# castacks/mvs_gi

Measured on AMD Instinct MI355X. Metric: stereo frames/sec/GPU (G16V, 3-cam, D=16) + inv-dist L1 vs reference, higher is better.
Workload: dtype f16x3 (split-fp16 MFMA operands: 11 + 11 significant bits, f32 accumulate/activations)

## Files before the change

include/mvsgi.h:

```cpp
#ifndef MVSGI_H
#define MVSGI_H

#include <stddef.h>
#include <stdint.h>

#ifdef __cplusplus
extern "C" {
#endif

#define MVSGI_ABI_VERSION 8

typedef void* mvsgi_stream_t;

#define MVSGI_CONV_AUTO   0
#define MVSGI_CONV_DIRECT 1
#define MVSGI_CONV_MFMA   2
#define MVSGI_CONV_BF16X3 3
#define MVSGI_CONV_BF16X3_C16 4
#define MVSGI_CONV_BF16X3_V32 5
#define MVSGI_CONV_BF16X3_D32 6

#define MVSGI_CONV_F16 0x100

#define MVSGI_SPLIT_F16 1

int         mvsgi_abi_version(void);
const char* mvsgi_last_error(void);

#define MVSGI_SAT_SWEEP 1u
#define MVSGI_SAT_SPLIT 2u
#define MVSGI_SAT_WINO  4u
int mvsgi_saturation_flags(int clear, unsigned* flags);
int mvsgi_saturation_words(unsigned* words8);

int mvsgi_sweep_max_cams(void);
int mvsgi_sweep_std_f32(const float* feats, const float* grids, const void* grid_masks,
                        int grid_mask_is_f32, const float* masks, float* vol,
                        int B, int N, int C, int Hi, int Wi, int Hm, int Wm,
                        int D, int Ho, int Wo, mvsgi_stream_t stream);

int mvsgi_sweep_cat_f32(const float* feats, const float* grids, float* vol,
                        int B, int N, int C, int Hi, int Wi,
                        int D, int Ho, int Wo, mvsgi_stream_t stream);

int mvsgi_sweep_std_nhwc_f32(const float* feats, const float* grids, const void* grid_masks,
                             int grid_mask_is_f32, const float* masks, float* vol,
                             int B, int N, int C, int Hi, int Wi, int Hm, int Wm,
                             int D, int Ho, int Wo, mvsgi_stream_t stream);
int mvsgi_sweep_cat_nhwc_f32(const float* feats, const float* grids, float* vol,
                             int B, int N, int C, int Hi, int Wi,
                             int D, int Ho, int Wo, mvsgi_stream_t stream);

int mvsgi_sweep_validity_u8(const float* grids, const void* grid_masks, int grid_mask_is_f32,
                            const float* masks, unsigned char* vmask,
                            int B, int N, int Hm, int Wm, int D, int Ho, int Wo, mvsgi_stream_t stream);
int mvsgi_sweep_std_nhwc_valid_f32(const float* feats, const float* grids, const unsigned char* vmask,
                                   float* vol, int B, int N, int C, int Hi, int Wi,
                                   int D, int Ho, int Wo, mvsgi_stream_t stream);
int mvsgi_sweep_std_nhwc_valid_rig_f32(const float* feats, const float* grids, const unsigned char* vmask,
                                       float* vol, int B, int N, int C, int Hi, int Wi, int D, int Ho, int Wo,
                                       mvsgi_stream_t stream);

size_t mvsgi_conv3d_packed_weight_floats(int Cout, int Cin);
int mvsgi_conv3d_pack_weights_f32(const float* w_oidhw, float* w_packed, int Cout, int Cin,
                                  mvsgi_stream_t stream);
size_t mvsgi_conv3d_packed_weight_bytes_bf16x3(int Cout, int Cin);
int mvsgi_conv3d_pack_weights_bf16x3(const float* w_oidhw, void* w_packed, int Cout, int Cin,
                                     mvsgi_stream_t stream);
int mvsgi_conv3d_pack_weights_split(const float* w_oidhw, void* w_packed, int Cout, int Cin, int layout, mvsgi_stream_t stream);
int mvsgi_conv3d_f32(const float* x, const float* w_oidhw, const float* w_packed,
                     const float* scale, const float* shift, const float* res, float* y,
                     int B, int Cin, int Din, int Hin, int Win, int Cout,
                     int stride, float neg_slope, int impl, mvsgi_stream_t stream);
const char* mvsgi_conv3d_variant_f32(int B, int Cin, int Din, int Hin, int Win, int Cout,
                                     int stride, int impl);

int mvsgi_conv3d_up2_f32(const float* x, const void* w_packed, int w_layout ,
                         const float* scale, const float* shift, const float* res, float* y,
                         int B, int Cin, int Dl, int Hl, int Wl, int Cout, float neg_slope, mvsgi_stream_t stream);
const char* mvsgi_conv3d_up2_variant_f32(int B, int Cin, int Dl, int Hl, int Wl, int Cout, int w_layout);
int mvsgi_conv3d_v32_applies(int B, int Cin, int Din, int Hin, int Win, int Cout, int stride);
int mvsgi_conv3d_d32_applies(int B, int Cin, int Din, int Hin, int Win, int Cout, int stride);
int mvsgi_conv3d_up2_d32_applies(int B, int Cin, int Dl, int Hl, int Wl, int Cout);
size_t mvsgi_conv3d_packed_weight_bytes_bf16x3_v32(int Cout, int Cin);
int mvsgi_conv3d_pack_weights_bf16x3_v32(const float* w_oidhw, void* w_packed, int Cout, int Cin, mvsgi_stream_t stream);
size_t mvsgi_conv3d_packed_weight_bytes_bf16x3_c16(int Cin);
int mvsgi_conv3d_pack_weights_bf16x3_c16(const float* w_oidhw, void* w_packed, int Cin, mvsgi_stream_t stream);

size_t mvsgi_conv2d_packed_weight_floats(int Cout, int Cin);
int mvsgi_conv2d_pack_weights_f32(const float* w_oihw, float* w_packed, int Cout, int Cin,
                                  mvsgi_stream_t stream);
size_t mvsgi_conv2d_stem_packed_weight_bytes(void);
int mvsgi_conv2d_stem_pack_weights(const float* w_oihw, void* w_packed, mvsgi_stream_t stream);
size_t mvsgi_conv2d_packed_weight_bytes_bf16x3(int Cout, int Cin);
int mvsgi_conv2d_pack_weights_bf16x3(const float* w_oihw, void* w_packed, int Cout, int Cin,
                                     mvsgi_stream_t stream);
int mvsgi_conv2d_f32(const float* x, const float* w_oihw, const void* w_packed,
                     const float* scale, const float* shift, const float* res, float* y,
                     int B, int Cin, int Hin, int Win, int Cout, int ksize, int stride,
                     float neg_slope, int impl, int in_nchw, mvsgi_stream_t stream);
const char* mvsgi_conv2d_variant_f32(int Cin, int Cout, int ksize, int stride, int impl, int in_nchw);

int mvsgi_resize_trilinear_f32(const float* x, float* y, int B, int C,
                               int Di, int Hi, int Wi, int Do, int Ho, int Wo,
                               mvsgi_stream_t stream);

int mvsgi_softargmin_f32(const float* costs, const float* inv_idx, float* inv_dist,
                         float* norm_costs, int B, int D, int H, int W, int scale,
                         mvsgi_stream_t stream);

int mvsgi_softargmin_div_f32(const float* costs, const float* inv_idx, float* inv_dist,
                             float* norm_costs, int B, int D, int H, int W, int scale,
                             float post_div, mvsgi_stream_t stream);

#define MVSGI_SA_AUTO  0
#define MVSGI_SA_PIXEL 1
#define MVSGI_SA_BAND  2
int mvsgi_softargmin_scaled_f32(const float* costs, const float* inv_idx, float* inv_dist,
                                float* norm_costs, int B, int D, int H, int W, double scale,
                                int OH, int OW, float post_div, int variant, mvsgi_stream_t stream);

int mvsgi_ncv_to_nvc_f32(const float* x, float* y, int B, int C, long long V, mvsgi_stream_t stream);
int mvsgi_nvc_to_ncv_f32(const float* x, float* y, int B, int C, long long V, mvsgi_stream_t stream);

int mvsgi_resblock2d_f32(const float* x, const void* w_packed1, const float* scale1, const float* shift1,
                         const void* w_packed2, const float* scale2, const float* shift2, float* y,
                         int N, int H, int W, float neg_slope, mvsgi_stream_t stream);

size_t mvsgi_split2d_bytes(int N, int H, int W);
int mvsgi_f32_to_split2d(const float* x, void* y_split, int N, int H, int W, mvsgi_stream_t stream);
int mvsgi_split2d_to_f32(const void* x_split, float* y, int N, int H, int W, mvsgi_stream_t stream);
size_t mvsgi_resblock2d_split_packed_weight_bytes(void);
int mvsgi_resblock2d_split_pack_weights(const float* w_oihw, const float* scale, void* w_packed, mvsgi_stream_t stream);
int mvsgi_resblock2d_split(const void* x_split, const void* w_packed1, const float* shift1,
                           const void* w_packed2, const float* shift2, void* y, int y_is_split,
                           int N, int H, int W, float neg_slope, mvsgi_stream_t stream);
int mvsgi_conv2d_s2_split(const void* x_split, const void* w_packed, const float* shift, void* y_split,
                          int N, int H, int W, float neg_slope, mvsgi_stream_t stream);
int mvsgi_conv2d_f32_out_split2d(const float* x, const float* w_oihw, const void* w_packed,
                                 const float* scale, const float* shift, const float* res, void* y_split,
                                 int B, int Cin, int Hin, int Win, int Cout, int ksize, int stride,
                                 float neg_slope, int impl, int in_nchw, mvsgi_stream_t stream);

int mvsgi_rays_panorama_f32(const float* dist, float* rays, int N, int H, int W,
                            float lat0, float lat1, float lon0, float lon1, mvsgi_stream_t stream);
int mvsgi_transform_points_f32(const float* T , const float* points, float* out,
                               int B, long long M, mvsgi_stream_t stream);
int mvsgi_grid_double_sphere_f32(const float* points, float* grid, unsigned char* mask, int B, long long M,
                                 float xi, float alpha, float fx, float fy, float cx, float cy,
                                 int calib_h, int calib_w, float w2, mvsgi_stream_t stream);
int mvsgi_grid_equirect_f32(const float* points, float* grid, int B, long long M, mvsgi_stream_t stream);
int mvsgi_rays_equirect_surrogate_f32(float* rays, int H, int W, mvsgi_stream_t stream);

int mvsgi_resample_bilinear_u8_f32(const unsigned char* imgs, const float* grid, const unsigned char* valid, float* out,
                                   long long M, int T, int Hr, int Wr, int H, int W, float invalid_value, mvsgi_stream_t stream);
int mvsgi_resample_bilinear_f32(const float* imgs, const float* grid, const unsigned char* valid, float* out, long long M, int T,
                                int C, int Hr, int Wr, int H, int W, float invalid_value, mvsgi_stream_t stream);
int mvsgi_resample_validity_u8(const float* grid, const unsigned char* ds_mask, unsigned char* valid, long long n,
                               mvsgi_stream_t stream);
int mvsgi_resample_u8_table_f32(float* table256);

int mvsgi_reproject_f32(const float* inv, const float* rays, const void* imgs, int img_kind, const float* T_host,
                        const float* cams_host, float* xyz, float* warped, unsigned char* valid, float* grid,
                        long long B, int N, int C, int Hr, int Wr, int H, int W, float bf, float invalid_value,
                        mvsgi_stream_t stream);

int mvsgi_deform_conv2d_pack_weights_f32(const float* w_oihw, float* w_packed, int Cout, int Cin, int Kh, int Kw,
                                         mvsgi_stream_t stream);
int mvsgi_deform_conv2d_f32(const float* x, const float* offset, int offset_per_image, const float* w_packed,
                            const float* scale, const float* shift, const float* res, float* y,
                            int N, int Cin, int H, int W, int Cout, int Kh, int Kw, int stride_h, int stride_w,
                            int pad_h, int pad_w, int dil_h, int dil_w, float neg_slope, mvsgi_stream_t stream);

int mvsgi_sweep_std_nhwc_valid_split(const float* feats, const float* grids, const unsigned char* vmask,
                                     void* vol_split, int B, int N, int C, int Hi, int Wi, int D, int Ho, int Wo,
                                     int rig_batch, mvsgi_stream_t stream);

int mvsgi_conv3d_f32_out_split(const float* x, const float* w_packed_b3, const float* scale, const float* shift,
                               const float* res, void* y_split, int B, int Cin, int Din, int Hin, int Win, int Cout,
                               int stride, float neg_slope, mvsgi_stream_t stream);
int mvsgi_conv3d_rs16_split(const void* x_split, const void* w_packed_rs, const float* scale, const float* shift, float* y,
                            int B, int D, int H, int W, float neg_slope, mvsgi_stream_t stream);
int mvsgi_conv3d_rs16_split_out_split(const void* x_split, const void* w_packed_rs, const float* scale, const float* shift,
                                      void* y_split, int B, int D, int H, int W, float neg_slope, mvsgi_stream_t stream);
size_t mvsgi_conv3d_s2rs_packed_weight_bytes(void);
int mvsgi_conv3d_s2rs_pack_weights(const float* w_oidhw, const float* scale, void* w_packed, mvsgi_stream_t stream);
int mvsgi_conv3d_s2rs(const void* x_split, const void* w_packed, const float* shift, void* y_split,
                      int B, int D, int H, int W, float neg_slope, mvsgi_stream_t stream);
size_t mvsgi_conv3d_rs_packed_weight_bytes(int Cout, int Cin);
int mvsgi_conv3d_rs_pack_weights(const float* w_oidhw, void* w_packed, int Cout, int Cin, mvsgi_stream_t stream);
size_t mvsgi_act_split_bytes(int B, int C, int D, int H, int W);
int mvsgi_act_f32_to_split(const float* x, void* y_split, int B, int C, int D, int H, int W, mvsgi_stream_t stream);
int mvsgi_act_split_to_f32(const void* x_split, float* y, int B, int C, int D, int H, int W, mvsgi_stream_t stream);
int mvsgi_conv3d_rs_split(const void* x_split, const void* w_packed_rs, const float* scale, const float* shift,
                          const void* res_split, void* y, int y_is_f32, int B, int Cin, int D, int H, int W, int Cout,
                          float neg_slope, mvsgi_stream_t stream);

int mvsgi_conv3d_up2_f32_out_split(const float* x, const void* w_packed, int w_layout, const float* scale, const float* shift,
                                   const float* res, void* y_split, int B, int Cin, int Dl, int Hl, int Wl, int Cout,
                                   float neg_slope, mvsgi_stream_t stream);
int mvsgi_conv3d_up2_poly_split(const void* x_split, const void* plan_dev, const float* scale, const float* shift, void* y_split,
                                int B, int D, int H, int W, float neg_slope, mvsgi_stream_t stream);
size_t mvsgi_conv3d_head_split_packed_weight_bytes(int Cin);
int mvsgi_conv3d_head_split_pack_weights(const float* w_oidhw, void* w_packed, int Cin, mvsgi_stream_t stream);
int mvsgi_conv3d_head_split(const void* x_split, const void* w_packed, float scale, float shift, float* y, int B, int Cin,
                            int D, int H, int W, float neg_slope, mvsgi_stream_t stream);
int mvsgi_conv3d_head_split_pack_weights_f16(const float* w_oidhw, void* w_packed, int Cin, mvsgi_stream_t stream);
int mvsgi_conv3d_head_split_f16(const void* x_split, const void* w_packed, float scale, float shift, float* y, int B, int Cin,
                            int D, int H, int W, float neg_slope, mvsgi_stream_t stream);
size_t mvsgi_conv3d_up2_poly_plan_bytes(int D, int H, int W);
int mvsgi_conv3d_up2_poly_plan(const float* w_oidhw_host, void* plan_host, int D, int H, int W);
int mvsgi_conv3d_up2_poly_f32(const void* x_split, const void* plan_dev, const float* scale, const float* shift, float* y,
                              int B, int D, int H, int W, float neg_slope, mvsgi_stream_t stream);

int mvsgi_act_f32_to_split_fmt(const float* x, void* y_split, int B, int C, int D, int H, int W, int fmt, mvsgi_stream_t stream);
int mvsgi_act_split_to_f32_fmt(const void* x_split, float* y, int B, int C, int D, int H, int W, int fmt, mvsgi_stream_t stream);
int mvsgi_sweep_std_nhwc_valid_split_fmt(const float* feats, const float* grids, const unsigned char* vmask, void* vol_split,
                                         int B, int N, int C, int Hi, int Wi, int D, int Ho, int Wo, int rig_batch, int fmt,
                                         mvsgi_stream_t stream);
int mvsgi_conv3d_f32_out_split_fmt(const float* x, const float* w_packed_b3, const float* scale, const float* shift,
                                   const float* res, void* y_split, int B, int Cin, int Din, int Hin, int Win, int Cout,
                                   int stride, float neg_slope, int fmt, mvsgi_stream_t stream);
int mvsgi_conv3d_rs_pack_weights_fmt(const float* w_oidhw, void* w_packed, int Cout, int Cin, int fmt, mvsgi_stream_t stream);
int mvsgi_conv3d_rs_split_fmt(const void* x_split, const void* w_packed_rs, const float* scale, const float* shift,
                              const void* res_split, void* y, int y_is_f32, int B, int Cin, int D, int H, int W, int Cout,
                              float neg_slope, int fmt, mvsgi_stream_t stream);
int mvsgi_conv3d_rs16_split_fmt(const void* x_split, const void* w_packed_rs, const float* scale, const float* shift, void* y,
                                int y_is_split, int B, int D, int H, int W, float neg_slope, int fmt, mvsgi_stream_t stream);
int mvsgi_conv3d_s2rs_pack_weights_fmt(const float* w_oidhw, const float* scale, void* w_packed, int fmt, mvsgi_stream_t stream);
int mvsgi_conv3d_s2rs_fmt(const void* x_split, const void* w_packed, const float* shift, void* y_split, int B, int D, int H, int W,
                          float neg_slope, float unscale, int fmt, mvsgi_stream_t stream);
int mvsgi_conv3d_s2rs_out_fmt(const void* x_split, const void* w_packed, const float* shift, void* y_split, int B, int D, int H, int W,
                              float neg_slope, float unscale, int fmt, int y_f32p, mvsgi_stream_t stream);
int mvsgi_conv3d_up2_poly_plan_fmt(const float* w_oidhw_host, void* plan_host, int D, int H, int W, int fmt);
int mvsgi_conv3d_up2_poly_fmt(const void* x_split, const void* plan_dev, const float* scale, const float* shift, void* y,
                              int y_is_split, int B, int D, int H, int W, float neg_slope, int fmt, mvsgi_stream_t stream);
int mvsgi_conv3d_up2_poly_wino_pays(int B, int D, int H, int W);

size_t mvsgi_conv3d_wino32_packed_weight_bytes(void);
int mvsgi_conv3d_wino32_applies(int Cin, int Cout, int D, int H, int W, int stride, float neg_slope);
int mvsgi_conv3d_wino32_pack_weights(const float* w_oidhw, void* w_packed, float* unscale, mvsgi_stream_t stream);
int mvsgi_conv3d_wino32_f16(const void* x_split, const void* w_packed, const float* scale, const float* shift, const void* res_split,
                            void* y, int y_is_f32, int act_f32p, int B, int D, int H, int W, float neg_slope, mvsgi_stream_t stream);

size_t mvsgi_instance_norm_ws_bytes(int B, int S, int C);
int mvsgi_instance_norm_f32(const float* x, const float* res, const float* gamma, const float* beta, float* y, float* ws,
                            int B, int S, int C, float eps, float neg_slope, mvsgi_stream_t stream);

#ifdef __cplusplus
}
#endif
#endif
```

mvs_gi_amd/_lib.py:

```python
from __future__ import annotations

import ctypes
import os
from ctypes import c_char_p, c_double, c_float, c_int, c_longlong, c_size_t, c_void_p

_HERE = os.path.dirname(os.path.abspath(__file__))
LIB_PATH = os.environ.get("MVSGI_LIB", os.path.join(_HERE, "libmvsgi_hip.so"))

ABI_VERSION = 8


class MvsgiLibraryMissing(RuntimeError):
    pass


_P = c_void_p
SIGNATURES = {
    "mvsgi_abi_version": (c_int, []),
    "mvsgi_last_error": (c_char_p, []),
    "mvsgi_saturation_flags": (c_int, [c_int, _P]),
    "mvsgi_saturation_words": (c_int, [_P]),
    "mvsgi_sweep_max_cams": (c_int, []),
    "mvsgi_sweep_std_f32": (c_int, [_P, _P, _P, c_int, _P, _P] + [c_int] * 10 + [_P]),
    "mvsgi_sweep_cat_f32": (c_int, [_P, _P, _P] + [c_int] * 8 + [_P]),
    "mvsgi_sweep_std_nhwc_f32": (c_int, [_P, _P, _P, c_int, _P, _P] + [c_int] * 10 + [_P]),
    "mvsgi_sweep_cat_nhwc_f32": (c_int, [_P, _P, _P] + [c_int] * 8 + [_P]),
    "mvsgi_sweep_validity_u8": (c_int, [_P, _P, c_int, _P, _P] + [c_int] * 7 + [_P]),
    "mvsgi_sweep_std_nhwc_valid_f32": (c_int, [_P, _P, _P, _P] + [c_int] * 8 + [_P]),
    "mvsgi_sweep_std_nhwc_valid_split": (c_int, [_P, _P, _P, _P] + [c_int] * 9 + [_P]),
    "mvsgi_sweep_std_nhwc_valid_rig_f32": (c_int, [_P, _P, _P, _P] + [c_int] * 8 + [_P]),
    "mvsgi_conv3d_packed_weight_floats": (c_size_t, [c_int, c_int]),
    "mvsgi_conv3d_pack_weights_f32": (c_int, [_P, _P, c_int, c_int, _P]),
    "mvsgi_conv3d_packed_weight_bytes_bf16x3": (c_size_t, [c_int, c_int]),
    "mvsgi_conv3d_pack_weights_bf16x3": (c_int, [_P, _P, c_int, c_int, _P]),
    "mvsgi_conv3d_pack_weights_split": (c_int, [_P, _P, c_int, c_int, c_int, _P]),
    "mvsgi_conv3d_f32": (c_int, [_P] * 7 + [c_int] * 7 + [c_float, c_int, _P]),
    "mvsgi_conv3d_variant_f32": (c_char_p, [c_int] * 8),
    "mvsgi_conv3d_up2_f32": (c_int, [_P, _P, c_int] + [_P] * 4 + [c_int] * 6 + [c_float, _P]),
    "mvsgi_conv3d_up2_variant_f32": (c_char_p, [c_int] * 7),
    "mvsgi_conv3d_v32_applies": (c_int, [c_int] * 7),
    "mvsgi_conv3d_d32_applies": (c_int, [c_int] * 7),
    "mvsgi_conv3d_up2_d32_applies": (c_int, [c_int] * 6),
    "mvsgi_conv3d_packed_weight_bytes_bf16x3_v32": (c_size_t, [c_int, c_int]),
    "mvsgi_conv3d_pack_weights_bf16x3_v32": (c_int, [_P, _P, c_int, c_int, _P]),
    "mvsgi_conv3d_packed_weight_bytes_bf16x3_c16": (c_size_t, [c_int]),
    "mvsgi_conv3d_pack_weights_bf16x3_c16": (c_int, [_P, _P, c_int, _P]),
    "mvsgi_conv2d_stem_packed_weight_bytes": (c_size_t, []),
    "mvsgi_conv2d_stem_pack_weights": (c_int, [_P, _P, _P]),
    "mvsgi_conv2d_packed_weight_floats": (c_size_t, [c_int, c_int]),
    "mvsgi_conv2d_pack_weights_f32": (c_int, [_P, _P, c_int, c_int, _P]),
    "mvsgi_conv2d_packed_weight_bytes_bf16x3": (c_size_t, [c_int, c_int]),
    "mvsgi_conv2d_pack_weights_bf16x3": (c_int, [_P, _P, c_int, c_int, _P]),
    "mvsgi_conv2d_f32": (c_int, [_P] * 7 + [c_int] * 7 + [c_float, c_int, c_int, _P]),
    "mvsgi_conv2d_variant_f32": (c_char_p, [c_int] * 6),
    "mvsgi_resblock2d_f32": (c_int, [_P] * 8 + [c_int] * 3 + [c_float, _P]),
    "mvsgi_split2d_bytes": (c_size_t, [c_int] * 3),
    "mvsgi_f32_to_split2d": (c_int, [_P, _P] + [c_int] * 3 + [_P]),
    "mvsgi_split2d_to_f32": (c_int, [_P, _P] + [c_int] * 3 + [_P]),
    "mvsgi_resblock2d_split_packed_weight_bytes": (c_size_t, []),
    "mvsgi_resblock2d_split_pack_weights": (c_int, [_P, _P, _P, _P]),
    "mvsgi_resblock2d_split": (c_int, [_P] * 6 + [c_int] * 4 + [c_float, _P]),
    "mvsgi_conv2d_s2_split": (c_int, [_P] * 4 + [c_int] * 3 + [c_float, _P]),
    "mvsgi_conv2d_f32_out_split2d": (c_int, [_P] * 7 + [c_int] * 7 + [c_float, c_int, c_int, _P]),
    "mvsgi_resize_trilinear_f32": (c_int, [_P, _P] + [c_int] * 8 + [_P]),
    "mvsgi_softargmin_f32": (c_int, [_P, _P, _P, _P] + [c_int] * 5 + [_P]),
    "mvsgi_softargmin_div_f32": (c_int, [_P, _P, _P, _P] + [c_int] * 5 + [c_float, _P]),
    "mvsgi_softargmin_scaled_f32": (c_int, [_P, _P, _P, _P] + [c_int] * 4 + [c_double, c_int, c_int, c_float, c_int, _P]),
    "mvsgi_rays_panorama_f32": (c_int, [_P, _P, c_int, c_int, c_int] + [c_float] * 4 + [_P]),
    "mvsgi_transform_points_f32": (c_int, [_P, _P, _P, c_int, c_longlong, _P]),
    "mvsgi_grid_double_sphere_f32": (c_int, [_P, _P, _P, c_int, c_longlong] + [c_float] * 6 + [c_int, c_int, c_float, _P]),
    "mvsgi_grid_equirect_f32": (c_int, [_P, _P, c_int, c_longlong, _P]),
    "mvsgi_rays_equirect_surrogate_f32": (c_int, [_P, c_int, c_int, _P]),
    "mvsgi_resample_bilinear_u8_f32": (c_int, [_P, _P, _P, _P, c_longlong] + [c_int] * 5 + [c_float, _P]),
    "mvsgi_resample_bilinear_f32": (c_int, [_P, _P, _P, _P, c_longlong] + [c_int] * 6 + [c_float, _P]),
    "mvsgi_resample_validity_u8": (c_int, [_P, _P, _P, c_longlong, _P]),
    "mvsgi_resample_u8_table_f32": (c_int, [_P]),
    "mvsgi_reproject_f32": (c_int, [_P, _P, _P, c_int] + [_P] * 6 + [c_longlong] + [c_int] * 6 + [c_float, c_float, _P]),
    "mvsgi_deform_conv2d_pack_weights_f32": (c_int, [_P, _P] + [c_int] * 4 + [_P]),
    "mvsgi_deform_conv2d_f32": (c_int, [_P, _P, c_int] + [_P] * 5 + [c_int] * 13 + [c_float, _P]),
    "mvsgi_act_split_bytes": (c_size_t, [c_int] * 5),
    "mvsgi_act_f32_to_split": (c_int, [_P, _P] + [c_int] * 5 + [_P]),
    "mvsgi_act_split_to_f32": (c_int, [_P, _P] + [c_int] * 5 + [_P]),
    "mvsgi_conv3d_f32_out_split": (c_int, [_P] * 6 + [c_int] * 7 + [c_float, _P]),
    "mvsgi_conv3d_rs16_split": (c_int, [_P] * 5 + [c_int] * 4 + [c_float, _P]),
    "mvsgi_conv3d_rs16_split_out_split": (c_int, [_P] * 5 + [c_int] * 4 + [c_float, _P]),
    "mvsgi_conv3d_s2rs_packed_weight_bytes": (c_size_t, []),
    "mvsgi_conv3d_s2rs_pack_weights": (c_int, [_P, _P, _P, _P]),
    "mvsgi_conv3d_s2rs": (c_int, [_P] * 4 + [c_int] * 4 + [c_float, _P]),
    "mvsgi_conv3d_rs_packed_weight_bytes": (c_size_t, [c_int, c_int]),
    "mvsgi_conv3d_rs_pack_weights": (c_int, [_P, _P, c_int, c_int, _P]),
    "mvsgi_conv3d_rs_split": (c_int, [_P] * 6 + [c_int] * 7 + [c_float, _P]),
    "mvsgi_conv3d_up2_f32_out_split": (c_int, [_P, _P, c_int] + [_P] * 4 + [c_int] * 6 + [c_float, _P]),
    "mvsgi_conv3d_up2_poly_split": (c_int, [_P] * 5 + [c_int] * 4 + [c_float, _P]),
    "mvsgi_conv3d_head_split_packed_weight_bytes": (c_size_t, [c_int]),
    "mvsgi_conv3d_head_split_pack_weights": (c_int, [_P, _P, c_int, _P]),
    "mvsgi_conv3d_head_split": (c_int, [_P, _P, c_float, c_float, _P] + [c_int] * 5 + [c_float, _P]),
    "mvsgi_conv3d_head_split_pack_weights_f16": (c_int, [_P, _P, c_int, _P]),
    "mvsgi_conv3d_head_split_f16": (c_int, [_P, _P, c_float, c_float, _P] + [c_int] * 5 + [c_float, _P]),
    "mvsgi_conv3d_up2_poly_plan_bytes": (c_size_t, [c_int] * 3),
    "mvsgi_conv3d_up2_poly_plan": (c_int, [_P, _P] + [c_int] * 3),
    "mvsgi_conv3d_up2_poly_f32": (c_int, [_P] * 5 + [c_int] * 4 + [c_float, _P]),
    "mvsgi_act_f32_to_split_fmt": (c_int, [_P, _P] + [c_int] * 6 + [_P]),
    "mvsgi_act_split_to_f32_fmt": (c_int, [_P, _P] + [c_int] * 6 + [_P]),
    "mvsgi_sweep_std_nhwc_valid_split_fmt": (c_int, [_P, _P, _P, _P] + [c_int] * 10 + [_P]),
    "mvsgi_conv3d_f32_out_split_fmt": (c_int, [_P] * 6 + [c_int] * 7 + [c_float, c_int, _P]),
    "mvsgi_conv3d_rs_pack_weights_fmt": (c_int, [_P, _P, c_int, c_int, c_int, _P]),
    "mvsgi_conv3d_rs_split_fmt": (c_int, [_P] * 6 + [c_int] * 7 + [c_float, c_int, _P]),
    "mvsgi_conv3d_rs16_split_fmt": (c_int, [_P] * 5 + [c_int] * 5 + [c_float, c_int, _P]),
    "mvsgi_conv3d_s2rs_pack_weights_fmt": (c_int, [_P, _P, _P, c_int, _P]),
    "mvsgi_conv3d_s2rs_fmt": (c_int, [_P] * 4 + [c_int] * 4 + [c_float, c_float, c_int, _P]),
    "mvsgi_conv3d_s2rs_out_fmt": (c_int, [_P] * 4 + [c_int] * 4 + [c_float, c_float, c_int, c_int, _P]),
    "mvsgi_conv3d_up2_poly_plan_fmt": (c_int, [_P, _P] + [c_int] * 4),
    "mvsgi_conv3d_wino32_packed_weight_bytes": (c_size_t, []),
    "mvsgi_conv3d_wino32_applies": (c_int, [c_int] * 6 + [c_float]),
    "mvsgi_conv3d_wino32_pack_weights": (c_int, [_P] * 4),
    "mvsgi_conv3d_wino32_f16": (c_int, [_P] * 6 + [c_int] * 6 + [c_float, _P]),
    "mvsgi_conv3d_up2_poly_fmt": (c_int, [_P] * 5 + [c_int] * 5 + [c_float, c_int, _P]),
    "mvsgi_conv3d_up2_poly_wino_pays": (c_int, [c_int] * 4),
    "mvsgi_ncv_to_nvc_f32": (c_int, [_P, _P, c_int, c_int, c_longlong, _P]),
    "mvsgi_nvc_to_ncv_f32": (c_int, [_P, _P, c_int, c_int, c_longlong, _P]),
    "mvsgi_instance_norm_ws_bytes": (c_size_t, [c_int] * 3),
    "mvsgi_instance_norm_f32": (c_int, [_P] * 6 + [c_int] * 3 + [c_float, c_float, _P]),
}

_lib = None


def load() -> ctypes.CDLL:
    global _lib
    if _lib is not None:
        return _lib
    if not os.path.isfile(LIB_PATH):
        raise MvsgiLibraryMissing(
            f"{LIB_PATH} not found: build the HIP library first (__graft_entry__.build()). "
            "mvs_gi_amd has no CPU fallback.")
    import torch
    lib = ctypes.CDLL(LIB_PATH)
    try:
        lib.mvsgi_abi_version.restype = c_int
        lib.mvsgi_abi_version.argtypes = []
        got = lib.mvsgi_abi_version()
    except AttributeError as e:
        raise MvsgiLibraryMissing(f"{LIB_PATH}: not a libmvsgi_hip ({e}); rebuild it (__graft_entry__.build())") from None
    if got != ABI_VERSION:
        raise MvsgiLibraryMissing(f"{LIB_PATH}: ABI version {got}, expected {ABI_VERSION}; rebuild it (__graft_entry__.build())")
    for name, (res, args) in SIGNATURES.items():
        try:
            fn = getattr(lib, name)
        except AttributeError:
            raise MvsgiLibraryMissing(f"{LIB_PATH}: symbol {name} missing although the ABI version matches; rebuild it "
                                      "(__graft_entry__.build())") from None
        fn.restype = res
        fn.argtypes = args
    lib.mvsgi_saturation_flags(0, None)
    _lib = lib
    return lib


def check(status: int, what: str) -> None:
    if status != 0:
        msg = load().mvsgi_last_error()
        raise RuntimeError(f"{what}: {msg.decode() if msg else 'unknown error'}")
```

mvs_gi_amd/csrc/common.hpp:

```cpp
#pragma once
#include <hip/hip_runtime.h>

#include <cstdarg>
#include <cstdio>
#include <cstdlib>
#include <cstring>
#include <string>

#include "../../include/mvsgi.h"

namespace mvsgi {

std::string& last_error_ref();

inline int fail(const char* fmt, ...) {
    char buf[512];
    va_list ap;
    va_start(ap, fmt);
    vsnprintf(buf, sizeof(buf), fmt, ap);
    va_end(ap);
    last_error_ref() = buf;
    return 1;
}

inline int check_launch(const char* what) {
    hipError_t e = hipGetLastError();
    if (e != hipSuccess) return fail("%s: launch failed: %s", what, hipGetErrorString(e));
    return 0;
}

#define MVSGI_REQUIRE(cond, ...)                      \
    do {                                              \
        if (!(cond)) return ::mvsgi::fail(__VA_ARGS__); \
    } while (0)

constexpr int kSatWords = 8;
unsigned* sat_words();
#define MVSGI_SAT_WORDS(VAR)                                                            \
    unsigned* VAR = ::mvsgi::sat_words();                                               \
    MVSGI_REQUIRE(VAR != nullptr, "cannot allocate the range report's pinned host words")

inline hipStream_t as_stream(mvsgi_stream_t s) { return reinterpret_cast<hipStream_t>(s); }

inline long long cdiv(long long a, long long b) { return (a + b - 1) / b; }

constexpr int kMaxCams = 8;

constexpr int kMaxDevices = 32;
struct PersistentGeom {
    int wgs_per_cu;
    int cus;
};
template <class K>
inline int persistent_geometry(K kern, int threads, size_t lds_bytes, int max_wgs_per_cu,
                               PersistentGeom (&cache)[kMaxDevices], const char* what, PersistentGeom& out) {
    int dev = 0;
    hipError_t e = hipGetDevice(&dev);
    if (e != hipSuccess) return fail("%s: hipGetDevice: %s", what, hipGetErrorString(e));
    if (dev < 0 || dev >= kMaxDevices) return fail("%s: device ordinal %d not supported (max %d)", what, dev, kMaxDevices);
    PersistentGeom g = cache[dev];
    if (!g.wgs_per_cu) {
        e = hipFuncSetAttribute(reinterpret_cast<const void*>(kern), hipFuncAttributeMaxDynamicSharedMemorySize,
                                (int)lds_bytes);
        if (e != hipSuccess) return fail("%s: hipFuncSetAttribute: %s", what, hipGetErrorString(e));
        int occ = 0;
        e = hipOccupancyMaxActiveBlocksPerMultiprocessor(&occ, kern, threads, lds_bytes);
        if (e != hipSuccess || occ < 1) occ = 1;
        int cus = 0;
        e = hipDeviceGetAttribute(&cus, hipDeviceAttributeMultiprocessorCount, dev);
        if (e != hipSuccess || cus < 1) return fail("%s: cannot read the device's CU count", what);
        g.wgs_per_cu = occ > max_wgs_per_cu ? max_wgs_per_cu : occ;
        g.cus = cus;
        cache[dev] = g;
    }
    out = g;
    return 0;
}

inline int device_cus() {
    static int cache[kMaxDevices] = {};
    int dev = 0;
    if (hipGetDevice(&dev) != hipSuccess || dev < 0 || dev >= kMaxDevices) return 256;
    if (!cache[dev]) {
        int cus = 0;
        if (hipDeviceGetAttribute(&cus, hipDeviceAttributeMultiprocessorCount, dev) != hipSuccess || cus < 1) cus = 256;
        cache[dev] = cus;
    }
    return cache[dev];
}

constexpr size_t kRs32PackedBytes = (size_t)2 * 2 * 14 * 2 * 64 * 16;
void rs32_pack_weights_host(const float* w_oidhw_32x32x27, void* packed, bool f16);
int rs32_up2_launch(const void* x_split, const void* w_sets, const float* scale32, const float* shift32, void* y, int y_is_split,
                    int B, int D, int H, int W, float neg_slope, bool f16, hipStream_t st);

constexpr size_t kWinoUp2RoleBytes = (size_t)4 * 4 * 3 * 2 * 2 * 64 * 16;
void wino_up2_pack_role(const float* w32_oidhw, unsigned short* wp, float* unscale32);
bool wino_up2_applies(int D, int H, int W);
int wino_up2_launch(const void* x_split, const void* w_roles, const float* unw, const float* scale16, const float* shift16, void* y_split,
                    int B, int D, int H, int W, float neg_slope, hipStream_t st);

}
```

mvs_gi_amd/csrc/conv3d_headsplit.hip:

```cpp
#include "common.hpp"

namespace {

typedef float f32x4 __attribute__((ext_vector_type(4)));
typedef unsigned u32x4 __attribute__((ext_vector_type(4)));
typedef __bf16 bf16x8 __attribute__((ext_vector_type(8)));
typedef _Float16 f16x8 __attribute__((ext_vector_type(8)));
typedef unsigned short u16x8 __attribute__((ext_vector_type(8)));

struct HeadArgs {
    const unsigned char* x;
    const bf16x8* wp;
    float* y;
    float scale, shift;
    float neg_slope;
    int B, Cin, D, H, W;
    int tiles_h, tiles_w;
};

__device__ __forceinline__ int hs_xcd_remap(int bid, int n) {
    const int q = n >> 3, r = n & 7, x = bid & 7, i = bid >> 3;
    return (x < r ? x * (q + 1) : r * (q + 1) + (x - r) * q) + i;
}

__global__ void head_split_pack_kernel(const float* __restrict__ w, bf16x8* __restrict__ wp, int Cin, bool f16) {
    const int idx = blockIdx.x * 256 + threadIdx.x;
    const int total = (Cin / 16) * 2 * 64;
    if (idx >= total) return;
    const int lane = idx & 63, tt = (idx >> 6) & 1, cs = idx >> 7;
    const int kg = lane >> 4, tap = tt * 16 + (lane & 15);
    u16x8 a1, a2;
    for (int j = 0; j < 8; ++j) {
        const float v = tap < 27 ? w[(cs * 16 + 8 * (kg & 1) + j) * 27 + tap] : 0.f;
        unsigned short h, l;
        if (f16) {
            const _Float16 hh = (_Float16)v;
            h = __builtin_bit_cast(unsigned short, hh);
            l = __builtin_bit_cast(unsigned short, (_Float16)(v - (float)hh));
        } else {
            const __bf16 hh = (__bf16)v;
            h = __builtin_bit_cast(unsigned short, hh);
            l = __builtin_bit_cast(unsigned short, (__bf16)(v - (float)hh));
        }
        a1[j] = h;
        a2[j] = kg < 2 ? l : (unsigned short)0;
    }
    wp[((cs * 2 + tt) * 2) * 64 + lane] = __builtin_bit_cast(bf16x8, a1);
    wp[((cs * 2 + tt) * 2 + 1) * 64 + lane] = __builtin_bit_cast(bf16x8, a2);
}

template <bool F16>
__global__ __launch_bounds__(256) void conv3d_head_split_kernel(HeadArgs a, int dchunk, int nd) {
    constexpr int TH = 8, TW = 32, ITH = TH + 2, ITW = TW + 2, PV = ITH * ITW;
    constexpr int NT = (PV + 15) / 16;
    constexpr int TPW = (NT + 3) / 4;
    constexpr int PSTR = 360;
    static_assert(NT * 16 <= PSTR, "P row too short");
    extern __shared__ __attribute__((aligned(16))) float hs_pbuf[];
    const int tid = threadIdx.x, lane = tid & 63;
    const int wave = __builtin_amdgcn_readfirstlane(tid >> 6);
    const int col = lane & 15, kg = lane >> 4;
    int t = hs_xcd_remap((int)blockIdx.x, (int)gridDim.x);
    const int tw_i = t % a.tiles_w;
    t /= a.tiles_w;
    const int th_i = t % a.tiles_h;
    t /= a.tiles_h;
    const int dc = t % nd;
    const int b = t / nd;
    const int oh0 = th_i * TH, ow0 = tw_i * TW;
    const int od_begin = dc * dchunk;
    const int od_end = od_begin + dchunk < a.D ? od_begin + dchunk : a.D;
    const int p0 = od_begin > 0 ? od_begin - 1 : 0;
    const int p1 = od_end < a.D - 1 ? od_end : a.D - 1;
    const int nchunks = a.Cin / 16;
    const int U = (p1 - p0 + 1) * nchunks;
    const int Hp = a.H + 2, Wp = a.W + 2, rec = a.Cin * 4;
    const long long plane_bytes = (long long)Hp * Wp * rec;

    unsigned goff[TPW];
#pragma unroll
    for (int k = 0; k < TPW; ++k) {
        const int T = wave + 4 * k, v = T * 16 + col;
        const int ih = v / ITW, iw = v - ih * ITW;
        const bool ok = T < NT && v < PV && oh0 + ih < Hp && ow0 + iw < Wp;
        goff[k] = ok ? (unsigned)(((oh0 + ih) * Wp + ow0 + iw) * rec + kg * 16) : 0xffffff00u;
    }
    const unsigned char* xb = a.x + (long long)b * (a.D + 2) * plane_bytes;
    bf16x8 wa[2][2];
    u32x4 xr[TPW];
#define HS_FETCH(P, CS)                                                                                             \
    {                                                                                                               \
        const __amdgpu_buffer_rsrc_t d_ = __builtin_amdgcn_make_buffer_rsrc(                                        \
            const_cast<unsigned char*>(xb) + (long long)((P) + 1) * plane_bytes, 0, (int)plane_bytes, 0x00020000); \
        _Pragma("unroll") for (int k = 0; k < TPW; ++k)                                                             \
            xr[k] = __builtin_amdgcn_raw_buffer_load_b128(d_, goff[k] + (unsigned)((CS) * 64), 0, 0);               \
        _Pragma("unroll") for (int tt = 0; tt < 2; ++tt) {                                                          \
            wa[tt][0] = a.wp[(((CS) * 2 + tt) * 2) * 64 + lane];                                                    \
            wa[tt][1] = a.wp[(((CS) * 2 + tt) * 2 + 1) * 64 + lane];                                                \
        }                                                                                                           \
    }
    HS_FETCH(p0, 0)

    const int h_ = tid / TW, w_ = tid % TW;
    const int oh = oh0 + h_, ow = ow0 + w_;
    const bool inside = oh < a.H && ow < a.W;
    float run[3] = {0.f, 0.f, 0.f};
    f32x4 acc[TPW][2];
#pragma unroll
    for (int k = 0; k < TPW; ++k) acc[k][0] = acc[k][1] = f32x4{0.f, 0.f, 0.f, 0.f};

    int p = p0, cs = 0;
    float pend = 0.f;
    long long pend_vox = -1;
    for (int u = 0; u < U; ++u) {
        int ncs = cs + 1, np = p;
        if (ncs == nchunks) { ncs = 0; np = p + 1; }
        bf16x8 cx[TPW], cw[2][2];
#pragma unroll
        for (int k = 0; k < TPW; ++k) cx[k] = __builtin_bit_cast(bf16x8, xr[k]);
#pragma unroll
        for (int tt = 0; tt < 2; ++tt) { cw[tt][0] = wa[tt][0]; cw[tt][1] = wa[tt][1]; }
        if (pend_vox >= 0) {
            a.y[pend_vox] = pend;
            pend_vox = -1;
        }
        {
            const int fp = u + 1 < U ? np : p, fcs = u + 1 < U ? ncs : cs;
            HS_FETCH(fp, fcs)
        }
#pragma unroll
        for (int k = 0; k < TPW; ++k) {
            if (wave + 4 * k < NT) {
#pragma unroll
                for (int tt = 0; tt < 2; ++tt) {
                    if constexpr (F16) {
                        acc[k][tt] = __builtin_amdgcn_mfma_f32_16x16x32_f16(__builtin_bit_cast(f16x8, cw[tt][1]), __builtin_bit_cast(f16x8, cx[k]), acc[k][tt], 0, 0, 0);
                        acc[k][tt] = __builtin_amdgcn_mfma_f32_16x16x32_f16(__builtin_bit_cast(f16x8, cw[tt][0]), __builtin_bit_cast(f16x8, cx[k]), acc[k][tt], 0, 0, 0);
                    } else {
                        acc[k][tt] = __builtin_amdgcn_mfma_f32_16x16x32_bf16(cw[tt][1], cx[k], acc[k][tt], 0, 0, 0);
                        acc[k][tt] = __builtin_amdgcn_mfma_f32_16x16x32_bf16(cw[tt][0], cx[k], acc[k][tt], 0, 0, 0);
                    }
                }
            }
        }
        if (ncs == 0) {
#pragma unroll
            for (int k = 0; k < TPW; ++k) {
                if (wave + 4 * k < NT) {
                    const int v = (wave + 4 * k) * 16 + col;
#pragma unroll
                    for (int tt = 0; tt < 2; ++tt)
#pragma unroll
                        for (int r = 0; r < 4; ++r) {
                            const int row = tt * 16 + 4 * kg + r;
                            if (row < 27) hs_pbuf[row * PSTR + v] = acc[k][tt][r];
                        }
                    acc[k][0] = acc[k][1] = f32x4{0.f, 0.f, 0.f, 0.f};
                }
            }
            __syncthreads();
#pragma unroll
            for (int k2 = 0; k2 < 9; ++k2) {
                const int vv = (h_ + k2 / 3) * ITW + (w_ + k2 % 3);
                run[0] += hs_pbuf[(18 + k2) * PSTR + vv];
                run[1] += hs_pbuf[(9 + k2) * PSTR + vv];
                run[2] += hs_pbuf[k2 * PSTR + vv];
            }
            const int od = p - 1;
            if (od >= od_begin && inside) {
                const long long vox = (((long long)b * a.D + od) * a.H + oh) * a.W + ow;
                const float r = run[0] * a.scale + a.shift;
                pend = r > 0.f ? r : r * a.neg_slope;
                pend_vox = vox;
            }
            run[0] = run[1];
            run[1] = run[2];
            run[2] = 0.f;
            __syncthreads();
        }
        p = np;
        cs = ncs;
    }
    if (pend_vox >= 0) a.y[pend_vox] = pend;
    if (p1 < od_end && inside) {
        const long long vox = (((long long)b * a.D + p1) * a.H + oh) * a.W + ow;
        const float r = run[0] * a.scale + a.shift;
        a.y[vox] = r > 0.f ? r : r * a.neg_slope;
    }
#undef HS_FETCH
}

}

extern "C" size_t mvsgi_conv3d_head_split_packed_weight_bytes(int Cin) {
    return Cin > 0 && Cin % 16 == 0 ? (size_t)(Cin / 16) * 2 * 2 * 64 * 16 : 0;
}

namespace {
int head_pack(const float* w_oidhw, void* w_packed, int Cin, bool f16, mvsgi_stream_t stream, const char* who) {
    MVSGI_REQUIRE(w_oidhw && w_packed, "%s: null pointer", who);
    MVSGI_REQUIRE(Cin > 0 && Cin % 16 == 0, "%s: Cin=%d must be a positive multiple of 16", who, Cin);
    const int total = (Cin / 16) * 2 * 64;
    hipLaunchKernelGGL(head_split_pack_kernel, dim3((unsigned)mvsgi::cdiv(total, 256)), dim3(256), 0, mvsgi::as_stream(stream), w_oidhw,
                       static_cast<bf16x8*>(w_packed), Cin, f16);
    return mvsgi::check_launch(who);
}

int head_launch(const void* x_split, const void* w_packed, float scale, float shift, float* y, int B, int Cin, int D, int H, int W,
                float neg_slope, bool f16, mvsgi_stream_t stream, const char* who) {
    MVSGI_REQUIRE(x_split && w_packed && y, "%s: null pointer", who);
    MVSGI_REQUIRE(B > 0 && D > 0 && H > 0 && W > 0 && Cin > 0 && Cin % 16 == 0, "%s: bad dims (Cin %% 16 == 0)", who);
    MVSGI_REQUIRE((long long)(H + 2) * (W + 2) * Cin * 4 < (1ll << 31), "%s: plane too large for 32-bit offsets", who);
    HeadArgs a{};
    a.x = static_cast<const unsigned char*>(x_split);
    a.wp = static_cast<const bf16x8*>(w_packed);
    a.y = y;
    a.scale = scale; a.shift = shift; a.neg_slope = neg_slope;
    a.B = B; a.Cin = Cin; a.D = D; a.H = H; a.W = W;
    a.tiles_h = (int)mvsgi::cdiv(H, 8);
    a.tiles_w = (int)mvsgi::cdiv(W, 32);
    const long long windows = (long long)B * a.tiles_h * a.tiles_w;
    long long nd = windows >= 1024 ? 1 : mvsgi::cdiv(1024, windows);
    if (nd > mvsgi::cdiv(D, 2)) nd = mvsgi::cdiv(D, 2);
    const int dchunk = (int)mvsgi::cdiv(D, nd);
    nd = mvsgi::cdiv(D, dchunk);
    const long long nt = windows * nd;
    MVSGI_REQUIRE(nt < (1ll << 31), "%s: too many tiles", who);
    constexpr size_t lds_bytes = (size_t)27 * 360 * sizeof(float);
    if (f16)
        hipLaunchKernelGGL(conv3d_head_split_kernel<true>, dim3((unsigned)nt), dim3(256), lds_bytes, mvsgi::as_stream(stream), a, dchunk, (int)nd);
    else
        hipLaunchKernelGGL(conv3d_head_split_kernel<false>, dim3((unsigned)nt), dim3(256), lds_bytes, mvsgi::as_stream(stream), a, dchunk, (int)nd);
    return mvsgi::check_launch(who);
}
}

extern "C" int mvsgi_conv3d_head_split_pack_weights(const float* w_oidhw, void* w_packed, int Cin, mvsgi_stream_t stream) {
    return head_pack(w_oidhw, w_packed, Cin, false, stream, "mvsgi_conv3d_head_split_pack_weights");
}
extern "C" int mvsgi_conv3d_head_split_pack_weights_f16(const float* w_oidhw, void* w_packed, int Cin, mvsgi_stream_t stream) {
    return head_pack(w_oidhw, w_packed, Cin, true, stream, "mvsgi_conv3d_head_split_pack_weights_f16");
}

extern "C" int mvsgi_conv3d_head_split(const void* x_split, const void* w_packed, float scale, float shift, float* y, int B, int Cin,
                                       int D, int H, int W, float neg_slope, mvsgi_stream_t stream) {
    return head_launch(x_split, w_packed, scale, shift, y, B, Cin, D, H, W, neg_slope, false, stream, "mvsgi_conv3d_head_split");
}
extern "C" int mvsgi_conv3d_head_split_f16(const void* x_split, const void* w_packed, float scale, float shift, float* y, int B, int Cin,
                                           int D, int H, int W, float neg_slope, mvsgi_stream_t stream) {
    return head_launch(x_split, w_packed, scale, shift, y, B, Cin, D, H, W, neg_slope, true, stream, "mvsgi_conv3d_head_split_f16");
}
```

mvs_gi_amd/csrc/conv3d_up2poly.hip:

```cpp
#include "common.hpp"

#include <cstring>
#include <vector>

namespace {

typedef float f32x4 __attribute__((ext_vector_type(4)));
typedef unsigned u32x4 __attribute__((ext_vector_type(4)));
typedef __bf16 bf16x8 __attribute__((ext_vector_type(8)));
#include "split_fmt.hpp"

enum { FIRST = 0, INT = 1, LAST = 2, ONLY = 3 };

struct M3 {
    double m[3][3];
};

M3 axis_matrix(int p, int i, int n) {
    M3 M{};
    for (int k = 0; k < 3; ++k) {
        const int v = 2 * i + p + k - 1;
        if (v < 0 || v >= 2 * n) continue;
        const int m = v >> 1, q = v & 1;
        const int src[2] = {q == 0 ? m - 1 : m, q == 0 ? m : m + 1};
        const double wgt[2] = {q == 0 ? 0.25 : 0.75, q == 0 ? 0.75 : 0.25};
        for (int e = 0; e < 2; ++e) {
            int s_ = src[e] < 0 ? 0 : (src[e] > n - 1 ? n - 1 : src[e]);
            M.m[s_ - i + 1][k] += wgt[e];
        }
    }
    return M;
}
M3 class_matrix(int p, int cls) {
    const int n = cls == ONLY ? 1 : 4;
    const int i = cls == FIRST || cls == ONLY ? 0 : (cls == INT ? 1 : n - 1);
    return axis_matrix(p, i, n);
}
M3 face_delta(int p, int cls) {
    const M3 a = class_matrix(p, cls), b = class_matrix(p, INT);
    M3 d{};
    for (int k = 0; k < 3; ++k) d.m[1][k] = a.m[1][k] - b.m[1][k];
    return d;
}
void fold(const M3& Md, const M3& Mh, const M3& Mw, const float* w, float* out) {
    for (int oi = 0; oi < 16 * 32; ++oi) {
        const float* ws = w + (size_t)oi * 27;
        double t1[27], t2[27], t3[27];
        for (int a = 0; a < 3; ++a)
            for (int l = 0; l < 3; ++l)
                for (int m = 0; m < 3; ++m) {
                    double s = 0;
                    for (int k = 0; k < 3; ++k) s += Md.m[a][k] * ws[k * 9 + l * 3 + m];
                    t1[a * 9 + l * 3 + m] = s;
                }
        for (int a = 0; a < 3; ++a)
            for (int b = 0; b < 3; ++b)
                for (int m = 0; m < 3; ++m) {
                    double s = 0;
                    for (int l = 0; l < 3; ++l) s += Mh.m[b][l] * t1[a * 9 + l * 3 + m];
                    t2[a * 9 + b * 3 + m] = s;
                }
        for (int a = 0; a < 3; ++a)
            for (int b = 0; b < 3; ++b)
                for (int c = 0; c < 3; ++c) {
                    double s = 0;
                    for (int m = 0; m < 3; ++m) s += Mw.m[c][m] * t2[a * 9 + b * 3 + m];
                    t3[a * 9 + b * 3 + c] = s;
                }
        for (int q = 0; q < 27; ++q) out[(size_t)oi * 27 + q] = (float)t3[q];
    }
}

struct Group {
    int cls, first, count;
};
std::vector<Group> groups_of(int n) {
    if (n == 1) return {{ONLY, 0, 1}};
    if (n == 2) return {{FIRST, 0, 1}, {LAST, 1, 1}};
    return {{FIRST, 0, 1}, {INT, 1, n - 2}, {LAST, n - 1, 1}};
}
struct Face {
    int idx, cls;
};
std::vector<Face> faces_of(int n) {
    if (n == 1) return {{0, ONLY}};
    return {{0, FIRST}, {n - 1, LAST}};
}

constexpr int kMagic = 0x50325032;
constexpr int kRoleInts = 32;
enum { R_WOFF = 0, R_NTAPS, R_TAP0, R_XBASE = 11, R_XS0, R_XSRUN, R_N0, R_NRUN, R_YS0, R_YSRUN, R_MFIRST, R_MLAST, R_YBASE0 = 20 };
enum { ST_WRITE = 0, ST_RMW = 1, ST_SKIP = 2 };
constexpr size_t kFaceRoleWBytes = (size_t)9 * 8 * 2 * 64 * 16;
constexpr size_t kEdgeSetFloats = (size_t)9 * 32 * 16;

struct PolyHeader {
    int magic, D, H, W;
    int n_roles, n_edge_cells, n_groups, max_tpf;
    long long off_main, off_facew, off_roles, off_edgew, off_edgecells, total;
    int sum_tpf;
    int pad0;
    long long off_roles_split;
    long long off_wino;
    long long off_wino_unscale;
    int pad[4];
};
static_assert(sizeof(PolyHeader) == 128, "header");

inline size_t align256(size_t v) { return (v + 255) & ~(size_t)255; }

PolyHeader layout(int D, int H, int W) {
    PolyHeader h{};
    h.magic = kMagic;
    h.D = D; h.H = H; h.W = W;
    const int ng = (int)groups_of(D).size(), nfh = (int)faces_of(H).size(), nfw = (int)faces_of(W).size();
    h.n_groups = ng;
    h.n_roles = (nfh + nfw) * ng;
    h.n_edge_cells = nfh * nfw;
    size_t o = sizeof(PolyHeader);
    h.off_main = (long long)(o = align256(o));
    o += 16 * mvsgi::kRs32PackedBytes;
    h.off_facew = (long long)(o = align256(o));
    o += (size_t)h.n_roles * kFaceRoleWBytes;
    h.off_roles = (long long)(o = align256(o));
    o += (size_t)h.n_roles * kRoleInts * 4;
    h.off_roles_split = (long long)(o = align256(o));
    o += (size_t)h.n_roles * kRoleInts * 4;
    h.off_edgew = (long long)(o = align256(o));
    o += (size_t)ng * h.n_edge_cells * 8 * kEdgeSetFloats * 4;
    h.off_edgecells = (long long)(o = align256(o));
    o += (size_t)h.n_edge_cells * 4 * 4;
    if (mvsgi::wino_up2_applies(D, H, W)) {
        h.off_wino = (long long)(o = align256(o));
        o += 2 * mvsgi::kWinoUp2RoleBytes;
        h.off_wino_unscale = (long long)(o = align256(o));
        o += 2 * 32 * 4;
    }
    h.total = (long long)align256(o);
    int tpf = 0, sum = 0;
    for (const Group& g : groups_of(D)) {
        const int a = g.count * (int)mvsgi::cdiv(W, 16), b = g.count * (int)mvsgi::cdiv(H, 16);
        tpf = a > tpf ? a : tpf;
        tpf = b > tpf ? b : tpf;
        sum += nfh * a + nfw * b;
    }
    h.max_tpf = tpf;
    h.sum_tpf = sum;
    return h;
}

void pack_face_weights(const float* wsrc, const int* taps, unsigned short* out, bool f16) {
    for (int t = 0; t < 9; ++t)
        for (int ph = 0; ph < 8; ++ph)
            for (int lane = 0; lane < 64; ++lane) {
                const int kg = lane >> 4, co = lane & 15;
                const size_t o = (((size_t)(t * 8 + ph) * 2) * 64 + lane) * 8;
                for (int e = 0; e < 8; ++e) {
                    const float v = wsrc[(((size_t)ph * 16 + co) * 32 + kg * 8 + e) * 27 + taps[t]];
                    sf_split_weight(v, f16, out[o + e], out[o + 64 * 8 + e]);
                }
            }
}

struct FaceGrid {
    int n_roles;
    int first[13];
};
template <bool F16>
__global__ __launch_bounds__(512, 2) void up2_face_kernel(const unsigned char* __restrict__ x, const unsigned char* __restrict__ plan,
                                                          unsigned char* __restrict__ y, int B, long long x_frame, long long y_frame,
                                                          long long off_facew, long long off_roles, FaceGrid fg) {
    extern __shared__ __attribute__((aligned(16))) unsigned char fw_lds[];
    int role = 0;
#pragma unroll
    for (int r = 1; r < 12; ++r) role += (r < fg.n_roles && (int)blockIdx.x >= fg.first[r]) ? 1 : 0;
    const int chunk = (int)blockIdx.x - fg.first[role], chunks = fg.first[role + 1] - fg.first[role];
    const int* R = reinterpret_cast<const int*>(plan + off_roles) + role * kRoleInts;
    const int n0 = R[R_N0], nrun = R[R_NRUN];
    const int tiles_run = (nrun + 15) >> 4, tpf = n0 * tiles_run;
    const int tid = threadIdx.x, lane = tid & 63, wave = __builtin_amdgcn_readfirstlane(tid >> 6);
    const int col = lane & 15, kg = lane >> 4;
    {
        const u32x4* src = reinterpret_cast<const u32x4*>(plan + off_facew) + (long long)R[R_WOFF];
        for (int i = tid; i < (int)(kFaceRoleWBytes / 16); i += 512) reinterpret_cast<u32x4*>(fw_lds)[i] = src[i];
    }
    __syncthreads();
    int tap[9], yb[8];
#pragma unroll
    for (int t = 0; t < 9; ++t) tap[t] = R[R_TAP0 + t];
#pragma unroll
    for (int p = 0; p < 8; ++p) yb[p] = R[R_YBASE0 + p];
    const int x_base = R[R_XBASE], x_s0 = R[R_XS0], x_srun = R[R_XSRUN];
    const int y_s0 = R[R_YS0], y_srun = R[R_YSRUN];
    const int m_first = R[R_MFIRST], m_last = R[R_MLAST];
    const int lane_x = (kg >> 1) * 64 + (kg & 1) * 16;
    const int total = B * tpf, stride = chunks * 8;
    for (int t = chunk * 8 + wave; t < total; t += stride) {
        const int rt = t % tiles_run;
        int q = t / tiles_run;
        const int o0 = q % n0, b = q / n0;
        const int run = rt * 16 + col;
        const bool ok = run < nrun;
        const __amdgpu_buffer_rsrc_t dx = __builtin_amdgcn_make_buffer_rsrc(const_cast<unsigned char*>(x) + (long long)b * x_frame, 0,
                                                                            (int)x_frame, 0x00020000);
        const unsigned xo = ok ? (unsigned)(x_base + o0 * x_s0 + run * x_srun + lane_x) : 0xffffff00u;
        u32x4 fh[9], fl[9];
#pragma unroll
        for (int k = 0; k < 9; ++k) {
            fh[k] = __builtin_amdgcn_raw_buffer_load_b128(dx, xo + (unsigned)tap[k], 0, 0);
            fl[k] = __builtin_amdgcn_raw_buffer_load_b128(dx, xo + (unsigned)tap[k] + 32u, 0, 0);
        }
        f32x4 acc[8];
#pragma unroll
        for (int p = 0; p < 8; ++p) acc[p] = f32x4{0.f, 0.f, 0.f, 0.f};
        int woff = lane * 16;
        asm volatile("" : "+v"(woff));
        bf16x8 wb[2][16];
#pragma unroll
        for (int i = 0; i < 16; ++i) wb[0][i] = *reinterpret_cast<const bf16x8*>(fw_lds + woff + i * 1024);
#pragma unroll
        for (int k = 0; k < 9; ++k) {
            if (k + 1 < 9) {
#pragma unroll
                for (int i = 0; i < 16; ++i) wb[(k + 1) & 1][i] = *reinterpret_cast<const bf16x8*>(fw_lds + woff + ((k + 1) * 16 + i) * 1024);
            }
            const bf16x8 xh = __builtin_bit_cast(bf16x8, fh[k]), xl = __builtin_bit_cast(bf16x8, fl[k]);
#pragma unroll
            for (int p = 0; p < 8; ++p) acc[p] = sf_mfma16<F16>(wb[k & 1][2 * p + 1], xh, acc[p]);
#pragma unroll
            for (int p = 0; p < 8; ++p) acc[p] = sf_mfma16<F16>(wb[k & 1][2 * p], xl, acc[p]);
#pragma unroll
            for (int p = 0; p < 8; ++p) acc[p] = sf_mfma16<F16>(wb[k & 1][2 * p], xh, acc[p]);
        }
        const int mode = run == 0 ? m_first : (run == nrun - 1 ? m_last : ST_WRITE);
        if (ok && mode != ST_SKIP) {
            unsigned char* yf = y + (long long)b * y_frame + (long long)o0 * y_s0 + (long long)run * y_srun + kg * 16;
#pragma unroll
            for (int p = 0; p < 8; ++p) {
                f32x4* dst = reinterpret_cast<f32x4*>(yf + yb[p]);
                *dst = mode == ST_RMW ? *dst + acc[p] : acc[p];
            }
        }
    }
}

template <bool F16>
__global__ __launch_bounds__(256) void up2_edge_kernel(const unsigned char* __restrict__ x, const unsigned char* __restrict__ plan,
                                                       float* __restrict__ y, int B, int D, int H, int W, int n_cells, int n_groups,
                                                       long long off_edgew, long long off_edgecells, int ob) {
    const long long idx = (long long)blockIdx.x * 256 + threadIdx.x;
    const long long n = (long long)B * D * n_cells * 128;
    if (idx >= n) return;
    const int co = (int)(idx & 15), phase = (int)((idx >> 4) & 7);
    long long q = idx >> 7;
    const int e = (int)(q % n_cells);
    q /= n_cells;
    const int i_d = (int)(q % D), b = (int)(q / D);
    const int* cell = reinterpret_cast<const int*>(plan + off_edgecells) + e * 4;
    const int i_h = cell[0], i_w = cell[1];
    const int g = n_groups == 1 ? 0 : (i_d == 0 ? 0 : (i_d == D - 1 ? n_groups - 1 : 1));
    const float* wt = reinterpret_cast<const float*>(plan + off_edgew) + ((size_t)(g * n_cells + e) * 8 + phase) * kEdgeSetFloats + co;
    const int Hp = H + 2, Wp = W + 2;
    const unsigned char* xb = x + ((((long long)b * (D + 2) + i_d + 1) * Hp + i_h + 1) * Wp + i_w + 1) * 128;
    float s = 0.f;
    for (int td = 0; td < 3; ++td)
        for (int th = 0; th < 3; ++th) {
            const unsigned char* xv = xb + ((long long)(td - 1) * Hp + (th - 1)) * Wp * 128;
            const float* wk = wt + (size_t)(td * 3 + th) * 32 * 16;
#pragma unroll
            for (int sl = 0; sl < 2; ++sl) {
                const unsigned* rec = reinterpret_cast<const unsigned*>(xv + sl * 64);
#pragma unroll
                for (int p = 0; p < 8; ++p) {
                    const unsigned hi = rec[p], lo = rec[p + 8];
                    const float a0 = sf_widen_lo<F16>(hi) + sf_widen_lo<F16>(lo);
                    const float a1 = sf_widen_hi<F16>(hi) + sf_widen_hi<F16>(lo);
                    s = fmaf(a0, wk[(sl * 16 + 2 * p) * 16], s);
                    s = fmaf(a1, wk[(sl * 16 + 2 * p + 1) * 16], s);
                }
            }
        }
    const int pd = phase >> 2, ph = (phase >> 1) & 1, pw = phase & 1;
    y[((((long long)b * (2 * D + 2 * ob) + 2 * i_d + pd + ob) * (2 * H + 2 * ob) + 2 * i_h + ph + ob) * (2 * W + 2 * ob) + 2 * i_w + pw + ob) * 16 + co] = s;
}

}

extern "C" size_t mvsgi_conv3d_up2_poly_plan_bytes(int D, int H, int W) {
    if (D < 1 || H < 1 || W < 1) return 0;
    return (size_t)layout(D, H, W).total;
}

extern "C" int mvsgi_conv3d_up2_poly_plan_fmt(const float* w_oidhw_host, void* plan_host, int D, int H, int W, int fmt) {
    MVSGI_REQUIRE(w_oidhw_host && plan_host, "mvsgi_conv3d_up2_poly_plan: null pointer");
    MVSGI_REQUIRE(fmt == 0 || fmt == MVSGI_SPLIT_F16, "mvsgi_conv3d_up2_poly_plan: fmt %d not in {0, MVSGI_SPLIT_F16}", fmt);
    const bool f16 = fmt != 0;
    MVSGI_REQUIRE(D > 0 && H > 0 && W > 0, "mvsgi_conv3d_up2_poly_plan: bad dims");
    MVSGI_REQUIRE((long long)(D + 2) * (H + 2) * (W + 2) * 128 < (1ll << 31) && (long long)D * H * W * 512 < (1ll << 31),
                  "mvsgi_conv3d_up2_poly_plan: frame too large for 32-bit offsets");
    const PolyHeader h = layout(D, H, W);
    unsigned char* P = static_cast<unsigned char*>(plan_host);
    memset(P, 0, (size_t)h.total);
    memcpy(P, &h, sizeof(h));
    const float* w = w_oidhw_host;
    std::vector<float> f0(16 * 32 * 27), w32(32 * 32 * 27);
    for (int pd = 0; pd < 2; ++pd)
        for (int cls = 0; cls < 4; ++cls)
            for (int ph = 0; ph < 2; ++ph) {
                for (int pw = 0; pw < 2; ++pw) {
                    fold(class_matrix(pd, cls), class_matrix(ph, INT), class_matrix(pw, INT), w, f0.data());
                    memcpy(w32.data() + (size_t)pw * 16 * 32 * 27, f0.data(), f0.size() * 4);
                }
                mvsgi::rs32_pack_weights_host(w32.data(), P + h.off_main + (size_t)((pd * 4 + cls) * 2 + ph) * mvsgi::kRs32PackedBytes, f16);
            }
    if (f16 && h.off_wino) {
        M3 ident{};
        for (int t = 0; t < 3; ++t) ident.m[t][t] = 1.0;
        for (int ph = 0; ph < 2; ++ph) {
            for (int pw = 0; pw < 2; ++pw) {
                fold(ident, class_matrix(ph, INT), class_matrix(pw, INT), w, f0.data());
                memcpy(w32.data() + (size_t)pw * 16 * 32 * 27, f0.data(), f0.size() * 4);
            }
            mvsgi::wino_up2_pack_role(w32.data(), reinterpret_cast<unsigned short*>(P + h.off_wino + (size_t)ph * mvsgi::kWinoUp2RoleBytes),
                                      reinterpret_cast<float*>(P + h.off_wino_unscale) + ph * 32);
        }
    }
    const int Hp = H + 2, Wp = W + 2, Hh = 2 * H, Wh = 2 * W;
    const std::vector<Group> gs = groups_of(D);
    const std::vector<Face> fhs = faces_of(H), fws = faces_of(W);
    int* roles = reinterpret_cast<int*>(P + h.off_roles);
    int r = 0;
    std::vector<float> w8(8 * 16 * 32 * 27);
    int* roles_split = reinterpret_cast<int*>(P + h.off_roles_split);
    auto emit = [&](const int* taps27, const int* tap_off, int x_base, int x_s0, int x_srun, int n0, int nrun, const int (*yb)[8],
                    const int* y_s0, const int* y_srun, int m_first, int m_last) {
        pack_face_weights(w8.data(), taps27, reinterpret_cast<unsigned short*>(P + h.off_facew + (size_t)r * kFaceRoleWBytes), f16);
        for (int geo = 0; geo < 2; ++geo) {
            int* R = (geo ? roles_split : roles) + (size_t)r * kRoleInts;
            R[R_WOFF] = (int)((size_t)r * kFaceRoleWBytes / 16);
            R[R_NTAPS] = 9;
            for (int t = 0; t < 9; ++t) R[R_TAP0 + t] = tap_off[t];
            R[R_XBASE] = x_base; R[R_XS0] = x_s0; R[R_XSRUN] = x_srun; R[R_N0] = n0; R[R_NRUN] = nrun;
            for (int p = 0; p < 8; ++p) R[R_YBASE0 + p] = yb[geo][p];
            R[R_YS0] = y_s0[geo]; R[R_YSRUN] = y_srun[geo]; R[R_MFIRST] = m_first; R[R_MLAST] = m_last;
        }
        ++r;
    };
    const int Hq[2] = {Hh, Hh + 2}, Wq[2] = {Wh, Wh + 2};
    for (const Group& g : gs) {
        for (const Face& fh : fhs) {
            int yb[2][8], ys0[2], ysr[2];
            for (int p = 0; p < 8; ++p) {
                const int pd = p >> 2, ph = (p >> 1) & 1, pw = p & 1;
                fold(class_matrix(pd, g.cls), face_delta(ph, fh.cls), class_matrix(pw, INT), w, w8.data() + (size_t)p * 16 * 32 * 27);
                for (int geo = 0; geo < 2; ++geo)
                    yb[geo][p] = (((2 * g.first + pd + geo) * Hq[geo] + 2 * fh.idx + ph + geo) * Wq[geo] + geo) * 64 + pw * 64;
            }
            for (int geo = 0; geo < 2; ++geo) { ys0[geo] = 2 * Hq[geo] * Wq[geo] * 64; ysr[geo] = 128; }
            int taps27[9], tap_off[9];
            for (int td = 0; td < 3; ++td)
                for (int tw = 0; tw < 3; ++tw) {
                    taps27[td * 3 + tw] = td * 9 + 3 + tw;
                    tap_off[td * 3 + tw] = ((td - 1) * Hp * Wp + (tw - 1)) * 128;
                }
            emit(taps27, tap_off, (((g.first + 1) * Hp + fh.idx + 1) * Wp + 1) * 128, Hp * Wp * 128, 128, g.count, W, yb, ys0, ysr,
                 ST_RMW, ST_RMW);
        }
        for (const Face& fw : fws) {
            int yb[2][8], ys0[2], ysr[2];
            for (int p = 0; p < 8; ++p) {
                const int pd = p >> 2, ph = (p >> 1) & 1, pw = p & 1;
                fold(class_matrix(pd, g.cls), class_matrix(ph, INT), face_delta(pw, fw.cls), w, w8.data() + (size_t)p * 16 * 32 * 27);
                for (int geo = 0; geo < 2; ++geo)
                    yb[geo][p] = (((2 * g.first + pd + geo) * Hq[geo] + ph + geo) * Wq[geo] + 2 * fw.idx + pw + geo) * 64;
            }
            for (int geo = 0; geo < 2; ++geo) { ys0[geo] = 2 * Hq[geo] * Wq[geo] * 64; ysr[geo] = 2 * Wq[geo] * 64; }
            int taps27[9], tap_off[9];
            for (int td = 0; td < 3; ++td)
                for (int th = 0; th < 3; ++th) {
                    taps27[td * 3 + th] = td * 9 + th * 3 + 1;
                    tap_off[td * 3 + th] = ((td - 1) * Hp + (th - 1)) * Wp * 128;
                }
            emit(taps27, tap_off, (((g.first + 1) * Hp + 1) * Wp + fw.idx + 1) * 128, Hp * Wp * 128, Wp * 128, g.count, H, yb, ys0, ysr,
                 ST_SKIP, ST_SKIP);
        }
    }
    MVSGI_REQUIRE(r == h.n_roles, "mvsgi_conv3d_up2_poly_plan: internal role count mismatch");
    int* cells = reinterpret_cast<int*>(P + h.off_edgecells);
    float* ew = reinterpret_cast<float*>(P + h.off_edgew);
    int e = 0;
    for (const Face& fh : fhs)
        for (const Face& fw : fws) {
            cells[e * 4] = fh.idx;
            cells[e * 4 + 1] = fw.idx;
            for (size_t gi = 0; gi < gs.size(); ++gi)
                for (int phase = 0; phase < 8; ++phase) {
                    const int pd = phase >> 2, ph = (phase >> 1) & 1, pw = phase & 1;
                    fold(class_matrix(pd, gs[gi].cls), class_matrix(ph, fh.cls), face_delta(pw, fw.cls), w, f0.data());
                    float* dst = ew + ((gi * h.n_edge_cells + e) * 8 + phase) * kEdgeSetFloats;
                    for (int td = 0; td < 3; ++td)
                        for (int th = 0; th < 3; ++th)
                            for (int ci = 0; ci < 32; ++ci)
                                for (int co = 0; co < 16; ++co)
                                    dst[((size_t)(td * 3 + th) * 32 + ci) * 16 + co] = f0[((size_t)co * 32 + ci) * 27 + td * 9 + th * 3 + 1];
                }
            ++e;
        }
    return 0;
}
extern "C" int mvsgi_conv3d_up2_poly_plan(const float* w_oidhw_host, void* plan_host, int D, int H, int W) {
    return mvsgi_conv3d_up2_poly_plan_fmt(w_oidhw_host, plan_host, D, H, W, 0);
}

namespace {

int poly_launch(const void* x_split, const void* plan_dev, const float* scale, const float* shift, void* y, int ob, int B, int D, int H,
                int W, float neg_slope, int fmt, hipStream_t st, int form = 0) {
    MVSGI_REQUIRE(x_split && plan_dev && scale && shift && y, "mvsgi_conv3d_up2_poly: null pointer");
    MVSGI_REQUIRE(fmt == 0 || fmt == MVSGI_SPLIT_F16, "mvsgi_conv3d_up2_poly: fmt %d not in {0, MVSGI_SPLIT_F16}", fmt);
    MVSGI_REQUIRE(B > 0 && D > 0 && H > 0 && W > 0, "mvsgi_conv3d_up2_poly: bad dims");
    MVSGI_REQUIRE(neg_slope >= 0.f && neg_slope <= 1.f, "mvsgi_conv3d_up2_poly: neg_slope %g not in [0, 1]", (double)neg_slope);
    MVSGI_REQUIRE((long long)(D + 2) * (H + 2) * (W + 2) * 128 < (1ll << 31) &&
                      (long long)(2 * D + 2) * (2 * H + 2) * (2 * W + 2) * 64 < (1ll << 31),
                  "mvsgi_conv3d_up2_poly: frame too large for 32-bit offsets");
    const PolyHeader h = layout(D, H, W);
    const unsigned char* P = static_cast<const unsigned char*>(plan_dev);
    const long long x_frame = (long long)(D + 2) * (H + 2) * (W + 2) * 128;
    const long long y_frame = (long long)(2 * D + 2 * ob) * (2 * H + 2 * ob) * (2 * W + 2 * ob) * 64;
    const long long n = (long long)B * D * h.n_edge_cells * 128;
    MVSGI_REQUIRE(mvsgi::cdiv(n, 256) < (1ll << 31), "mvsgi_conv3d_up2_poly: too many edge threads");
    if (fmt)
        hipLaunchKernelGGL(up2_edge_kernel<true>, dim3((unsigned)mvsgi::cdiv(n, 256)), dim3(256), 0, st, static_cast<const unsigned char*>(x_split), P,
                           static_cast<float*>(y), B, D, H, W, h.n_edge_cells, h.n_groups, h.off_edgew, h.off_edgecells, ob);
    else
        hipLaunchKernelGGL(up2_edge_kernel<false>, dim3((unsigned)mvsgi::cdiv(n, 256)), dim3(256), 0, st, static_cast<const unsigned char*>(x_split), P,
                           static_cast<float*>(y), B, D, H, W, h.n_edge_cells, h.n_groups, h.off_edgew, h.off_edgecells, ob);
    if (mvsgi::check_launch("mvsgi_conv3d_up2_poly(edges)")) return 1;
    int dev = 0, cus = 256;
    if (hipGetDevice(&dev) == hipSuccess) (void)hipDeviceGetAttribute(&cus, hipDeviceAttributeMultiprocessorCount, dev);
    static bool attr_set[mvsgi::kMaxDevices] = {};
    if (dev >= 0 && dev < mvsgi::kMaxDevices && !attr_set[dev]) {
        hipError_t e = hipFuncSetAttribute(reinterpret_cast<const void*>(up2_face_kernel<false>), hipFuncAttributeMaxDynamicSharedMemorySize,
                                           (int)kFaceRoleWBytes);
        if (e == hipSuccess)
            e = hipFuncSetAttribute(reinterpret_cast<const void*>(up2_face_kernel<true>), hipFuncAttributeMaxDynamicSharedMemorySize,
                                    (int)kFaceRoleWBytes);
        MVSGI_REQUIRE(e == hipSuccess, "mvsgi_conv3d_up2_poly: hipFuncSetAttribute: %s", hipGetErrorString(e));
        attr_set[dev] = true;
    }
    MVSGI_REQUIRE(h.n_roles <= 12, "mvsgi_conv3d_up2_poly: internal: %d face roles", h.n_roles);
    long long slots = (long long)cus - h.n_roles;
    if (slots < 8) slots = 8;
    long long tpw = mvsgi::cdiv((long long)B * h.sum_tpf, slots);
    if (tpw < 8) tpw = 8;
    FaceGrid fg{};
    fg.n_roles = h.n_roles;
    {
        int r = 0, acc = 0;
        for (const Group& g : groups_of(D)) {
            const int nfh = (int)faces_of(H).size(), nfw = (int)faces_of(W).size();
            for (int f = 0; f < nfh + nfw; ++f) {
                const long long tpf = (long long)g.count * mvsgi::cdiv(f < nfh ? W : H, 16);
                fg.first[r++] = acc;
                acc += (int)mvsgi::cdiv((long long)B * tpf, tpw);
            }
        }
        fg.first[r] = acc;
    }
    if (fmt)
        hipLaunchKernelGGL(up2_face_kernel<true>, dim3((unsigned)fg.first[h.n_roles]), dim3(512), kFaceRoleWBytes, st,
                           static_cast<const unsigned char*>(x_split), P, static_cast<unsigned char*>(y), B, x_frame, y_frame, h.off_facew,
                           ob ? h.off_roles_split : h.off_roles, fg);
    else
        hipLaunchKernelGGL(up2_face_kernel<false>, dim3((unsigned)fg.first[h.n_roles]), dim3(512), kFaceRoleWBytes, st,
                           static_cast<const unsigned char*>(x_split), P, static_cast<unsigned char*>(y), B, x_frame, y_frame, h.off_facew,
                           ob ? h.off_roles_split : h.off_roles, fg);
    if (mvsgi::check_launch("mvsgi_conv3d_up2_poly(faces)")) return 1;
    MVSGI_REQUIRE(form != 2 || (fmt && ob && h.off_wino), "mvsgi_conv3d_up2_poly: the Winograd form needs the fp16 split, a split-padded output, "
                  "D == 8, H %% 2 == 0 and W %% 32 == 0 (got D, H, W = %d, %d, %d)", D, H, W);
    if (form == 2)
        return mvsgi::wino_up2_launch(x_split, P + h.off_wino, reinterpret_cast<const float*>(P + h.off_wino_unscale), scale, shift, y,
                                      B, D, H, W, neg_slope, st);
    if (fmt && ob && form == 0 && h.off_wino) {
        const long long units = (long long)B * (H / 2) * (W / 32);
        long long nwalk = cus / 16;
        if (nwalk > mvsgi::cdiv(units, 8)) nwalk = mvsgi::cdiv(units, 8);
        if (nwalk < 1) nwalk = 1;
        const long long rounds = mvsgi::cdiv(mvsgi::cdiv(units, 8), nwalk);
        if (10 * units >= 7 * rounds * 8 * nwalk)
            return mvsgi::wino_up2_launch(x_split, P + h.off_wino, reinterpret_cast<const float*>(P + h.off_wino_unscale), scale, shift, y,
                                          B, D, H, W, neg_slope, st);
    }
    return mvsgi::rs32_up2_launch(x_split, P + h.off_main, scale, shift, y, ob, B, D, H, W, neg_slope, fmt != 0, st);
}

}

extern "C" int mvsgi_conv3d_up2_poly_f32(const void* x_split, const void* plan_dev, const float* scale, const float* shift, float* y,
                                         int B, int D, int H, int W, float neg_slope, mvsgi_stream_t stream) {
    return poly_launch(x_split, plan_dev, scale, shift, y, 0, B, D, H, W, neg_slope, 0, mvsgi::as_stream(stream));
}

extern "C" int mvsgi_conv3d_up2_poly_split(const void* x_split, const void* plan_dev, const float* scale, const float* shift, void* y_split,
                                           int B, int D, int H, int W, float neg_slope, mvsgi_stream_t stream) {
    return poly_launch(x_split, plan_dev, scale, shift, y_split, 1, B, D, H, W, neg_slope, 0, mvsgi::as_stream(stream));
}

extern "C" int mvsgi_conv3d_up2_poly_fmt(const void* x_split, const void* plan_dev, const float* scale, const float* shift, void* y,
                                         int y_is_split, int B, int D, int H, int W, float neg_slope, int fmt, mvsgi_stream_t stream) {
    MVSGI_REQUIRE(y_is_split == 0 || y_is_split == 1 || y_is_split == 3 || y_is_split == 5, "mvsgi_conv3d_up2_poly: y_is_split %d not in {0, 1, 3, 5}",
                  y_is_split);
    return poly_launch(x_split, plan_dev, scale, shift, y, y_is_split ? 1 : 0, B, D, H, W, neg_slope, fmt, mvsgi::as_stream(stream),
                       y_is_split == 3 ? 1 : (y_is_split == 5 ? 2 : 0));
}

extern "C" int mvsgi_conv3d_up2_poly_wino_pays(int B, int D, int H, int W) {
    if (!mvsgi::wino_up2_applies(D, H, W) || B < 1) return 0;
    const int cus = mvsgi::device_cus();
    const long long units = (long long)B * (H / 2) * (W / 32);
    long long nwalk = cus / 16;
    if (nwalk > mvsgi::cdiv(units, 8)) nwalk = mvsgi::cdiv(units, 8);
    if (nwalk < 1) nwalk = 1;
    const long long rounds = mvsgi::cdiv(mvsgi::cdiv(units, 8), nwalk);
    return 10 * units >= 7 * rounds * 8 * nwalk ? 1 : 0;
}
```

mvs_gi_amd/csrc/conv3d_wino_up2.hip:

```cpp
#include "common.hpp"

#include <cmath>
#include <cstring>
#include <vector>

namespace {

typedef float f32x4 __attribute__((ext_vector_type(4)));
typedef float f32x2 __attribute__((ext_vector_type(2)));
typedef unsigned u32x2 __attribute__((ext_vector_type(2)));
typedef unsigned u32x4 __attribute__((ext_vector_type(4)));

#include "split_fmt.hpp"
#include "conv3d_wino_common.hpp"

struct WinoUp2Args {
    const unsigned char* x;
    unsigned char* y;
    const u32x4* wp;
    const float* unw;
    const float* scale;
    const float* shift;
    int B, D, H, W;
    float neg_slope;
    int tiles_h, groups_w, total_units;
    unsigned* sat;
};

namespace wu {
constexpr int HALF = 17, PITCH = 5, RPITCH = 9;
constexpr int NVOX = 4 * 2 * HALF;
constexpr int SUB = (NVOX * PITCH + 15) / 16 * 16;
constexpr int PLANE_SLOTS = 2 * SUB;
constexpr int NDMA = 22, DPW = 6;
constexpr int PLANE_LDS = NDMA * 1024;
constexpr int NBUF = 2;
constexpr int ZB = NBUF * PLANE_LDS;
constexpr int RB = ZB + 2 * 16384;
constexpr int RDPW = 3, RES_LDS = 4 * RDPW * 1024, NRES = 3;
constexpr int XB = RB + NRES * RES_LDS;
constexpr int DUMMY = XB + 32768;
constexpr int LDS_BYTES = DUMMY + 1024;
constexpr int DEPTH = 16;
static_assert(LDS_BYTES <= 160 * 1024, "LDS budget");
enum { PLAIN = 0, EVEN = 1, ODD = 2, COPY = 3 };
__host__ __device__ constexpr int step_type(int s) { return s == 15 ? PLAIN : (s == 14 ? COPY : ((s & 1) ? ODD : EVEN)); }
__host__ __device__ constexpr int step_request(int s) { return s == 0 ? 2 : (s == 1 ? 3 : (s == 3 ? 4 : (s == 5 ? 5 : (s == 7 ? 6 : (s == 9 ? 7 : (s == 11 ? 8 : (s == 13 ? 9 : -1))))))); }
__host__ __device__ constexpr int step_read(int s) { return s == 14 ? 8 : (s == 15 ? 9 : ((s & 1) && s <= 11 ? (s + 3) / 2 : -1)); }
}

__device__ __forceinline__ void split_pair_ovfl(float v0, float v1, unsigned& hi, unsigned& lo, float& satm) {
    satm = sf_sat_acc(satm, v0, v1);
    hi = sf_cvt_pk<true>(v0, v1);
    lo = sf_cvt_pk<true>(mix_sub_lo(v0, hi), mix_sub_hi(v1, hi));
}

__global__ __launch_bounds__(256, 1) void conv3d_wino_up2_kernel(WinoUp2Args a) {
    using namespace wu;
    extern __shared__ __attribute__((aligned(16))) unsigned char lds[];
    __builtin_amdgcn_s_setreg((1 - 1) << 11 | 23 << 6 | 1, 1u);
    const int tid = threadIdx.x, lane = tid & 63;
    const int wv = __builtin_amdgcn_readfirstlane(tid >> 6);
    const int n = lane & 15, kg = lane >> 4;
    const int Hp = a.H + 2, Wp = a.W + 2;
    const long long plane_bytes = (long long)Hp * Wp * 128;
    const long long frame_bytes = (a.D + 2) * plane_bytes;
    const long long total_bytes = frame_bytes * a.B;
    const int Hq = 2 * a.H + 2, Wq = 2 * a.W + 2;
    const long long oplane_bytes = (long long)Hq * Wq * 64;
    const long long oframe_bytes = (2 * a.D + 2) * oplane_bytes;
    const long long ototal_bytes = oframe_bytes * a.B;
    const int i0 = wv == 0 ? 0 : (wv == 2 ? 2 : 1);
    const int i1 = wv == 0 ? 2 : (wv == 1 ? 2 : (wv == 2 ? 1 : 3));
    const float sgn = __builtin_bit_cast(float, __builtin_amdgcn_readfirstlane(wv == 1 ? 0x3f800000 : 0xbf800000));
    const int pa = wv & 1, q = wv >> 1;
    const float osg = pa ? -1.f : 1.f;

    const int G = gridDim.x, xcd = (int)blockIdx.x & 7, iw = (int)blockIdx.x >> 3;
    const int ph = iw & 1, walker = iw >> 1, nwalk = G >> 4;
    const int T_ = a.total_units, q8 = T_ >> 3, r8 = T_ & 7;
    const int ulo = xcd < r8 ? xcd * (q8 + 1) : r8 * (q8 + 1) + (xcd - r8) * q8, ucnt = q8 + (xcd < r8 ? 1 : 0);
    const int ubase = ulo + walker, ustep = nwalk;
    const int nmine = walker < ucnt ? (ucnt - walker + nwalk - 1) / nwalk : 0;
    if (nmine == 0) return;

    u32x4 wh[4][3][2], wl[4][3][2];
#pragma unroll
    for (int b = 0; b < 4; ++b)
#pragma unroll
        for (int kd = 0; kd < 3; ++kd)
#pragma unroll
            for (int c = 0; c < 2; ++c) {
                const u32x4* p_ = a.wp + ((long long)(((((ph * 4 + wv) * 4 + b) * 3 + kd) * 2 + c) * 2)) * 64 + lane;
                wh[b][kd][c] = p_[0];
                wl[b][kd][c] = p_[64];
            }
#pragma unroll
    for (int b = 0; b < 4; ++b)
#pragma unroll
        for (int kd = 0; kd < 3; ++kd)
#pragma unroll
            for (int c = 0; c < 2; ++c) asm volatile("" : "+a"(wh[b][kd][c]), "+a"(wl[b][kd][c]));
    const f32x4 esc_ = *reinterpret_cast<const f32x4*>(a.scale + kg * 4), esh_ = *reinterpret_cast<const f32x4*>(a.shift + kg * 4);
    const f32x4 ema_[2] = {*reinterpret_cast<const f32x4*>(a.unw + (ph * 2 + 0) * 16 + kg * 4) * esc_,
                           *reinterpret_cast<const f32x4*>(a.unw + (ph * 2 + 1) * 16 + kg * 4) * esc_};
    __builtin_amdgcn_sched_barrier(0);

    const int lane_out = (2 * n) * 128 + (kg >> 1) * 16 + (kg & 1) * 8;
    const int rd0 = ((kg & 1) * SUB + (i0 * 2 * HALF + n) * PITCH + (kg >> 1) * 2) * 16;
    const int rd1 = ((kg & 1) * SUB + (i1 * 2 * HALF + n) * PITCH + (kg >> 1) * 2) * 16;
    constexpr int RD2 = 16;
    unsigned voff[DPW], rvoff[RDPW];
    int rrow[RDPW], rcol[RDPW];
#pragma unroll
    for (int k = 0; k < DPW; ++k) {
        const int m = wv + 4 * k;
        const int sl = m * 64 + lane;
        const int sub = sl >= SUB ? 1 : 0, rem = sl - sub * SUB;
        const int vox = rem / PITCH, c = rem - vox * PITCH;
        const int row = vox / (2 * HALF), rr = vox - row * (2 * HALF);
        const int par = rr / HALF, idx = rr - par * HALF;
        const int piece = c * 2 + sub;
        voff[k] = (m < NDMA && sl < PLANE_SLOTS && vox < NVOX && c < 4) ? (unsigned)((row * Wp + 2 * idx + par) * 128 + piece * 16)
                                                                        : 0xffffff00u;
    }
#pragma unroll
    for (int k = 0; k < RDPW; ++k) {
        const int sl = (wv + 4 * k) * 64 + lane;
        const int vox = sl / RPITCH, piece = sl - vox * RPITCH;
        rrow[k] = vox >> 5;
        rcol[k] = vox & 31;
        rvoff[k] = (vox < 64 && piece < 8) ? (unsigned)((vox >> 5) * 2 * Wq * 64 + (vox & 31) * 128 + piece * 16) : 0xffffff00u;
    }
    const int rrd = ((pa * 32 + 2 * n + q) * RPITCH + kg) * 16;
    const int xoff = XB + tid * 8;

    f32x4 Y[3][4][2];
    u32x4 vh[2][4], vl[2][4];
    u32x4 raw[2][4][2];
    float T[2][4];
    f32x2 Xc[4][4];
    f32x2 Pq[4];
    float satm = 0.f;

#define KU_DESC(U, LIVE)                                                                                    \
    ({                                                                                                      \
        const int c_ = (U) % a.groups_w, t_ = (U) / a.groups_w;                                             \
        const int r_ = t_ % a.tiles_h, b_ = t_ / a.tiles_h;                                                 \
        const long long off_ = (LIVE) ? b_ * frame_bytes + ((long long)(2 * r_) * Wp + 32 * c_) * 128 : 0;  \
        const long long left_ = total_bytes - off_;                                                         \
        __builtin_amdgcn_make_buffer_rsrc(const_cast<unsigned char*>(a.x) + off_, 0,                        \
                                          (LIVE) ? (left_ > 0x7fffff00ll ? 0x7fffff00 : (int)left_) : 0, 0x00020000); \
    })
#define KU_DMA_ISSUE(Q, K0, K1)                                                                             \
    _Pragma("unroll") for (int k_ = (K0); k_ < (K1); ++k_)                                                  \
        __builtin_amdgcn_raw_ptr_buffer_load_lds((Q) < 8 ? dsc : dsc_next,                                  \
                                                 (__attribute__((address_space(3))) void*)(lds + (wv + 4 * k_ < NDMA ? ((Q) & 1) * PLANE_LDS + (wv + 4 * k_) * 1024 : DUMMY)), \
                                                 16, voff[k_], (unsigned)(((Q) % 8 + 1) * plane_bytes), 0, 0);
#define KU_RES_DMA(IMG, O)                                                                                  \
    {                                                                                                       \
        const unsigned so_ = (unsigned)(((O) + 1) * oplane_bytes);                                          \
        _Pragma("unroll") for (int k_ = 0; k_ < RDPW; ++k_)                                                 \
            __builtin_amdgcn_raw_ptr_buffer_load_lds(rdsc, (__attribute__((address_space(3))) void*)(lds + RB + (IMG) * RES_LDS + (wv + 4 * k_) * 1024), \
                                                     16, rvu[k_], so_, 0, 0);                               \
    }
#define KU_READ(BUF_)                                                                                       \
    {                                                                                                       \
        const unsigned char* im_ = lds + (BUF_) * PLANE_LDS;                                                \
        _Pragma("unroll") for (int j_ = 0; j_ < 4; ++j_) {                                                  \
            const int o_ = (((j_ & 1) * HALF + (j_ >> 1)) * PITCH) * 16;                                    \
            raw[0][j_][0] = *reinterpret_cast<const u32x4*>(im_ + rd0 + o_);                                \
            raw[0][j_][1] = *reinterpret_cast<const u32x4*>(im_ + rd0 + o_ + RD2);                          \
            raw[1][j_][0] = *reinterpret_cast<const u32x4*>(im_ + rd1 + o_);                                \
            raw[1][j_][1] = *reinterpret_cast<const u32x4*>(im_ + rd1 + o_ + RD2);                          \
        }                                                                                                   \
    }
#define KU_TPIECE(M, VN, TY)                                                                                \
    {                                                                                                       \
        constexpr int d_ = (M) / 18, r_ = (M) % 18;                                                         \
        if constexpr (r_ < 8) {                                                                             \
            constexpr int j_ = r_ >> 1;                                                                     \
            if constexpr ((TY) != PLAIN && r_ < 4)                                                          \
                Pq[r_] = *reinterpret_cast<const f32x2*>(lds + xoff + (r_ * 4 + d_) * 2048);                \
            if constexpr ((TY) == PLAIN || (TY) == EVEN) {                                                  \
                       \
                if constexpr ((r_ & 1) == 0) {                                                              \
                    asm("v_fma_mix_f32 %0, %1, 1.0, %2 op_sel:[0,0,0] op_sel_hi:[1,0,1]\n\t"                \
                        "v_fma_mix_f32 %0, %3, %5, %0 op_sel:[0,0,0] op_sel_hi:[1,0,0]\n\t"                 \
                        "v_fma_mix_f32 %0, %4, %5, %0 op_sel:[0,0,0] op_sel_hi:[1,0,0]"                      \
                        : "=&v"(T[0][j_]) : "v"(raw[0][j_][0][d_]), "v"(raw[0][j_][1][d_]), "v"(raw[1][j_][0][d_]), "v"(raw[1][j_][1][d_]), "s"(sgn)); \
                } else {                                                                                    \
                    asm("v_fma_mix_f32 %0, %1, 1.0, %2 op_sel:[1,0,1] op_sel_hi:[1,0,1]\n\t"                \
                        "v_fma_mix_f32 %0, %3, %5, %0 op_sel:[1,0,0] op_sel_hi:[1,0,0]\n\t"                 \
                        "v_fma_mix_f32 %0, %4, %5, %0 op_sel:[1,0,0] op_sel_hi:[1,0,0]"                      \
                        : "=&v"(T[1][j_]) : "v"(raw[0][j_][0][d_]), "v"(raw[0][j_][1][d_]), "v"(raw[1][j_][0][d_]), "v"(raw[1][j_][1][d_]), "s"(sgn)); \
                }                                                                                           \
            }                                                                                               \
        } else if constexpr (r_ < 16) {                                                                     \
            constexpr int b_ = (r_ - 8) >> 1;                                                               \
            constexpr int x_ = b_ == 0 ? 0 : (b_ == 2 ? 2 : 1), y_ = b_ == 0 ? 2 : (b_ == 1 ? 2 : (b_ == 2 ? 1 : 3)); \
            if constexpr (((r_ - 8) & 1) == 0) {                                                            \
                if constexpr ((TY) == PLAIN || (TY) == EVEN) {                                              \
                    X0 = b_ == 1 ? T[0][x_] + T[0][y_] : T[0][x_] - T[0][y_];                               \
                    X1 = b_ == 1 ? T[1][x_] + T[1][y_] : T[1][x_] - T[1][y_];                               \
                }                                                                                           \
                if constexpr ((TY) == PLAIN) {             \
                    *reinterpret_cast<f32x2*>(lds + xoff + (b_ * 4 + d_) * 2048) = f32x2{X0, X1};           \
                } else if constexpr ((TY) == EVEN) {                             \
                    Xc[b_][d_] = f32x2{X0, X1};                                                             \
                    X0 = __builtin_fmaf(X0 - Pq[b_][0], 0.25f, Pq[b_][0]);                                  \
                    X1 = __builtin_fmaf(X1 - Pq[b_][1], 0.25f, Pq[b_][1]);                                  \
                } else if constexpr ((TY) == ODD) {        \
                    X0 = __builtin_fmaf(Xc[b_][d_][0] - Pq[b_][0], 0.75f, Pq[b_][0]);                       \
                    X1 = __builtin_fmaf(Xc[b_][d_][1] - Pq[b_][1], 0.75f, Pq[b_][1]);                       \
                    *reinterpret_cast<f32x2*>(lds + xoff + (b_ * 4 + d_) * 2048) = Xc[b_][d_];              \
                } else {                                                      \
                    X0 = Pq[b_][0];                                                                         \
                    X1 = Pq[b_][1];                                                                         \
                }                                                                                           \
                satm = sf_sat_acc(satm, X0, X1);           \
                if constexpr (b_ > 0) vl[VN][b_ - 1][d_] = sf_cvt_pk<true>(L0, L1);      \
            } else {                                                                                        \
                const unsigned h_ = sf_cvt_pk<true>(X0, X1);                                                \
                vh[VN][b_][d_] = h_;                                                                        \
                asm("v_fma_mix_f32 %0, %2, -1.0, %3 op_sel:[0,0,0] op_sel_hi:[1,0,0]\n\t"                   \
                    "v_fma_mix_f32 %1, %2, -1.0, %4 op_sel:[1,0,0] op_sel_hi:[1,0,0]"                        \
                    : "=&v"(L0), "=&v"(L1) : "v"(h_), "v"(X0), "v"(X1));                                    \
            }                                                                                               \
        } else if constexpr (r_ == 16) {                                                                    \
            vl[VN][3][d_] = sf_cvt_pk<true>(L0, L1);                                                        \
        }                                                                                                   \
    }
#define KU_DPIECE(M, S)                                                                                     \
    if constexpr (step_request(S) >= 0 && (M) >= 1 && (M) <= 3) { KU_DMA_ISSUE(step_request(S), 2 * ((M) - 1), 2 * (M)) } \
    else if constexpr ((M) == 17) { KU_RES_DMA(ri, S) }
#define KU_OUT_WRITE(SF, ZIMG)                                                                              \
    _Pragma("unroll") for (int c_ = 0; c_ < 2; ++c_) {                                                      \
        f32x4 y0_ = Y[SF][0][c_], y1_ = Y[SF][1][c_], y2_ = Y[SF][2][c_], y3_ = Y[SF][3][c_];               \
        if constexpr ((SF) >= 1) {       \
            asm volatile("" : "+v"(y0_), "+v"(y1_), "+v"(y2_), "+v"(y3_));                                  \
        }                                                                                                   \
        const f32x4 z0_ = (y0_ + y1_) + y2_;                                                                \
        const f32x4 z1_ = (y1_ - y2_) - y3_;                                                                \
        *reinterpret_cast<f32x4*>(lds + ZB + (ZIMG) * 16384 + ((wv * 2 + 0) * 2 + c_) * 1024 + lane * 16) = z0_; \
        *reinterpret_cast<f32x4*>(lds + ZB + (ZIMG) * 16384 + ((wv * 2 + 1) * 2 + c_) * 1024 + lane * 16) = z1_; \
    }
#define KU_EPI_READS(ZIMG)                                                                                  \
    f32x4 zz_[2][3], rf_[2];                                                                                \
    _Pragma("unroll") for (int c_ = 0; c_ < 2; ++c_)                                                        \
        _Pragma("unroll") for (int k_ = 0; k_ < 3; ++k_)                                                    \
            zz_[c_][k_] = *reinterpret_cast<const f32x4*>(lds + ZB + (ZIMG) * 16384 + (((pa + k_) * 2 + q) * 2 + c_) * 1024 + lane * 16); \
    _Pragma("unroll") for (int c_ = 0; c_ < 2; ++c_) rf_[c_] = *reinterpret_cast<const f32x4*>(rim_ + rrd + c_ * 64);
#define KU_EPILOGUE(O)                                                                                      \
    _Pragma("unroll") for (int c_ = 0; c_ < 2; ++c_) {                                                      \
        f32x4 t_ = zz_[c_][0] + osg * (zz_[c_][1] + zz_[c_][2]);                                            \
        _Pragma("unroll") for (int e_ = 0; e_ < 4; ++e_)                                                    \
            t_[e_] = __builtin_fmaf(t_[e_], ema_[c_][e_], __builtin_fmaf(rf_[c_][e_], esc_[e_], esh_[e_])); \
        _Pragma("unroll") for (int e_ = 0; e_ < 4; ++e_) t_[e_] = __builtin_fmaxf(t_[e_], t_[e_] * a.neg_slope); \
        unsigned h0_, l0_, h1_, l1_;                                                                        \
        split_pair_ovfl(t_[0], t_[1], h0_, l0_, satm);                                                      \
        split_pair_ovfl(t_[2], t_[3], h1_, l1_, satm);                                                      \
        unsigned char* q_ = yb + (long long)((O) + 1) * oplane_bytes + lane_out + c_ * 64;                  \
        *reinterpret_cast<u32x2*>(q_) = u32x2{h0_, h1_};                                                    \
        *reinterpret_cast<u32x2*>(q_ + 32) = u32x2{l0_, l1_};                                               \
    }
#define KU_SLOT(M, S, SI, SM, SF, VB)                                                                       \
    {                                                                                                       \
        constexpr int g_ = (M) / 24, w_ = (M) % 24, tm_ = w_ / 8, b_ = (w_ % 8) / 2, c_ = w_ % 2;           \
        constexpr int kd_ = 2 - g_, s_ = g_ == 0 ? (SF) : (g_ == 1 ? (SM) : (SI));                          \
        constexpr bool live_ = !(g_ == 0 && (S) == 0) && !(g_ == 2 && (S) == DEPTH - 1);                    \
        constexpr bool first_ = tm_ == 0 && (g_ == 2 || (g_ == 1 && (S) == 0));                             \
        if constexpr (live_) {                                                                              \
            if constexpr (s_ >= 1) {                                                                        \
                if constexpr (first_) { WN_MFA0(Y[s_][b_][c_], wl[b_][kd_][c_], vh[VB][b_]) }               \
                else if constexpr (tm_ == 0) { WN_MFA(Y[s_][b_][c_], wl[b_][kd_][c_], vh[VB][b_]) }         \
                else if constexpr (tm_ == 1) { WN_MFA(Y[s_][b_][c_], wh[b_][kd_][c_], vl[VB][b_]) }         \
                else { WN_MFA(Y[s_][b_][c_], wh[b_][kd_][c_], vh[VB][b_]) }                                 \
            } else {                                                                                        \
                if constexpr (first_) { WN_MF0(Y[s_][b_][c_], wl[b_][kd_][c_], vh[VB][b_]) }                \
                else if constexpr (tm_ == 0) { WN_MF(Y[s_][b_][c_], wl[b_][kd_][c_], vh[VB][b_]) }          \
                else if constexpr (tm_ == 1) { WN_MF(Y[s_][b_][c_], wh[b_][kd_][c_], vl[VB][b_]) }          \
                else { WN_MF(Y[s_][b_][c_], wh[b_][kd_][c_], vh[VB][b_]) }                                  \
            }                                                                                               \
        }                                                                                                   \
        KU_TPIECE(M, (VB) ^ 1, step_type(S))                                                                \
        KU_DPIECE(M, S)                                                                                     \
        __builtin_amdgcn_sched_barrier(0);                                                                  \
    }
#define KU_S8(M, S, SI, SM, SF, VB)                                                                         \
    KU_SLOT(M, S, SI, SM, SF, VB) KU_SLOT(M + 1, S, SI, SM, SF, VB) KU_SLOT(M + 2, S, SI, SM, SF, VB) KU_SLOT(M + 3, S, SI, SM, SF, VB) \
    KU_SLOT(M + 4, S, SI, SM, SF, VB) KU_SLOT(M + 5, S, SI, SM, SF, VB) KU_SLOT(M + 6, S, SI, SM, SF, VB) KU_SLOT(M + 7, S, SI, SM, SF, VB)

#define KU_STEP(S, SI, SM, SF, VB)                                                                          \
    {                                                                                                       \
        unsigned char* rim_ = lds + RB + rprev * RES_LDS;                                                   \
        asm volatile("s_nop 1");                                                                            \
        {                                                                                                   \
            float X0 = 0.f, X1 = 0.f, L0 = 0.f, L1 = 0.f;                                                   \
            KU_S8(0, S, SI, SM, SF, VB) KU_S8(8, S, SI, SM, SF, VB) KU_S8(16, S, SI, SM, SF, VB)            \
            KU_S8(24, S, SI, SM, SF, VB) KU_S8(32, S, SI, SM, SF, VB) KU_S8(40, S, SI, SM, SF, VB)          \
            KU_S8(48, S, SI, SM, SF, VB) KU_S8(56, S, SI, SM, SF, VB) KU_S8(64, S, SI, SM, SF, VB)          \
        }                                                                                                   \
        WN_PAD()                                                                                            \
        if constexpr ((S) > 0) { KU_OUT_WRITE(SF, ((S) - 1) & 1) }                                          \
         \
        if constexpr (step_request(S) >= 0) asm volatile("s_waitcnt vmcnt(9) lgkmcnt(0)" ::: "memory");     \
        else asm volatile("s_waitcnt vmcnt(3) lgkmcnt(0)" ::: "memory");                                    \
        __builtin_amdgcn_s_barrier();                                                                       \
        if constexpr ((S) > 0) {                                                                            \
            KU_EPI_READS(((S) - 1) & 1)                                                                     \
            KU_EPILOGUE((S) - 1)                                                                            \
        }                                                                                                   \
        __builtin_amdgcn_sched_barrier(0);                                                                  \
        if constexpr (step_read(S) >= 0) { KU_READ(step_read(S) & 1) }                                      \
        rprev = ri;                                                                                         \
        ri = ri == NRES - 1 ? 0 : ri + 1;                                                                   \
    }
#define KU_FINISH(SF)                                                                                       \
    {                                                                                                       \
        unsigned char* rim_ = lds + RB + rprev * RES_LDS;                                                   \
        KU_OUT_WRITE(SF, (DEPTH - 1) & 1)                                                                   \
        asm volatile("s_waitcnt vmcnt(4) lgkmcnt(0)" ::: "memory");                                         \
        __builtin_amdgcn_s_barrier();                                                                       \
        KU_EPI_READS((DEPTH - 1) & 1)                                                                       \
        KU_EPILOGUE(DEPTH - 1)                                                                              \
    }
#define KU_T8(M, TY) KU_TPIECE(M, 0, TY) KU_TPIECE(M + 1, 0, TY) KU_TPIECE(M + 2, 0, TY) KU_TPIECE(M + 3, 0, TY) KU_TPIECE(M + 4, 0, TY) KU_TPIECE(M + 5, 0, TY) KU_TPIECE(M + 6, 0, TY) KU_TPIECE(M + 7, 0, TY)

    int ri = 0, rprev = 0;
    auto dsc = KU_DESC(ubase, true);
    auto dsc_next = dsc;
    KU_DMA_ISSUE(0, 0, DPW)
    KU_DMA_ISSUE(1, 0, DPW)
    asm volatile("s_waitcnt vmcnt(0) lgkmcnt(0)" ::: "memory");
    __builtin_amdgcn_s_barrier();
    KU_READ(0)
    {
        float X0 = 0.f, X1 = 0.f, L0 = 0.f, L1 = 0.f;
        KU_T8(0, PLAIN) KU_T8(8, PLAIN) KU_T8(16, PLAIN) KU_T8(24, PLAIN) KU_T8(32, PLAIN) KU_T8(40, PLAIN) KU_T8(48, PLAIN) KU_T8(56, PLAIN) KU_T8(64, PLAIN)
    }
    KU_READ(1)
    __builtin_amdgcn_s_barrier();
    for (int k = 0; k < nmine; ++k) {
        const int u = ubase + k * ustep;
        const int c = u % a.groups_w;
        const int t = u / a.groups_w;
        const int r = t % a.tiles_h;
        const int b = t / a.tiles_h;
        unsigned char* yb = a.y + b * oframe_bytes + ((long long)(2 * (2 * r + pa) + ph + 1) * Wq + 2 * (32 * c + q) + 1) * 64;
        const long long roff = b * oframe_bytes + ((long long)(2 * (2 * r) + ph + 1) * Wq + 2 * (32 * c) + 1) * 64;
        const long long rleft = ototal_bytes - roff;
        const auto rdsc = __builtin_amdgcn_make_buffer_rsrc(a.y + roff, 0, rleft > 0x7fffff00ll ? 0x7fffff00 : (int)rleft, 0x00020000);
        unsigned rvu[RDPW];
#pragma unroll
        for (int k_ = 0; k_ < RDPW; ++k_) {
            const int ih_ = 2 * r + rrow[k_], iw_ = 32 * c + rcol[k_];
            const bool face_ = ih_ == 0 || ih_ == a.H - 1 || iw_ == 0 || iw_ == a.W - 1;
            rvu[k_] = face_ ? rvoff[k_] : 0xffffff00u;
        }
        dsc_next = KU_DESC(u + ustep, k + 1 < nmine);
#define KU_STEPP(S) KU_STEP(S, ((S) + 1) % 3, (S) % 3, ((S) + 2) % 3, (S) & 1)
        KU_STEPP(0) KU_STEPP(1) KU_STEPP(2) KU_STEPP(3) KU_STEPP(4) KU_STEPP(5) KU_STEPP(6) KU_STEPP(7)
        KU_STEPP(8) KU_STEPP(9) KU_STEPP(10) KU_STEPP(11) KU_STEPP(12) KU_STEPP(13) KU_STEPP(14) KU_STEPP(15)
        KU_FINISH((DEPTH - 1) % 3)
        dsc = dsc_next;
    }
    sf_sat_report(a.sat, kSatSplit, satm, kF16Max);
}

}

namespace mvsgi {

void wino_up2_pack_role(const float* w32, unsigned short* wp, float* unscale) {
    static const double Gm[4][3] = {{1., 0., 0.}, {0.5, 0.5, 0.5}, {0.5, -0.5, 0.5}, {0., 0., 1.}};
    for (int co = 0; co < 32; ++co) {
        double amax = 0.;
        std::vector<double> Uc((size_t)32 * 48);
        for (int ci = 0; ci < 32; ++ci) {
            const float* g = w32 + ((size_t)co * 32 + ci) * 27;
            for (int ab = 0; ab < 16; ++ab)
                for (int kd = 0; kd < 3; ++kd) {
                    double acc = 0.;
                    for (int kh = 0; kh < 3; ++kh)
                        for (int kw = 0; kw < 3; ++kw) acc += Gm[ab >> 2][kh] * Gm[ab & 3][kw] * (double)g[kd * 9 + kh * 3 + kw];
                    Uc[(size_t)ci * 48 + ab * 3 + kd] = acc;
                    amax = std::fmax(amax, std::fabs(acc));
                }
        }
        int k = 0;
        if (amax > 0.) {
            int e;
            const double m = std::frexp(amax, &e);
            k = m == 0.5 ? 11 - e : 10 - e;
            k = k < -100 ? -100 : (k > 100 ? 100 : k);
        }
        const double up = std::ldexp(1., k);
        unscale[co] = (float)std::ldexp(1., -k);
        for (int ci = 0; ci < 32; ++ci)
            for (int ab = 0; ab < 16; ++ab)
                for (int kd = 0; kd < 3; ++kd) {
                    unsigned short hi, lo;
                    sf_split_weight((float)(Uc[(size_t)ci * 48 + ab * 3 + kd] * up), true, hi, lo);
                    const size_t frag = (((size_t)ab * 3 + kd) * 2 + (co >> 4)) * 2;
                    const int lane = (ci >> 3) * 16 + (co & 15);
                    wp[((frag + 0) * 64 + lane) * 8 + (ci & 7)] = hi;
                    wp[((frag + 1) * 64 + lane) * 8 + (ci & 7)] = lo;
                }
    }
}

bool wino_up2_applies(int D, int H, int W) {
    return D == 8 && H > 0 && W > 0 && H % 2 == 0 && W % 32 == 0 && (long long)(D + 2) * (H + 2) * (W + 2) * 128 < (1ll << 31) &&
           (long long)(2 * D + 2) * (2 * H + 2) * (2 * W + 2) * 64 < (1ll << 31);
}

int wino_up2_launch(const void* x_split, const void* w_roles, const float* unw, const float* scale16, const float* shift16, void* y_split,
                    int B, int D, int H, int W, float neg_slope, hipStream_t st) {
    MVSGI_REQUIRE(wino_up2_applies(D, H, W), "mvsgi_conv3d_up2_poly(winograd): needs D == 8, H %% 2 == 0, W %% 32 == 0 (got %d, %d, %d)", D, H, W);
    WinoUp2Args a;
    memset(&a, 0, sizeof(a));
    a.x = static_cast<const unsigned char*>(x_split);
    a.y = static_cast<unsigned char*>(y_split);
    a.wp = static_cast<const u32x4*>(w_roles);
    a.unw = unw;
    a.scale = scale16;
    a.shift = shift16;
    a.B = B; a.D = D; a.H = H; a.W = W;
    a.neg_slope = neg_slope;
    a.tiles_h = H / 2;
    a.groups_w = W / 32;
    const long long units = (long long)B * a.tiles_h * a.groups_w;
    MVSGI_REQUIRE(units < (1ll << 30), "mvsgi_conv3d_up2_poly(winograd): too many units");
    a.total_units = (int)units;
    MVSGI_SAT_WORDS(sat_words_);
    a.sat = sat_words_;
    static PersistentGeom geo_cache[kMaxDevices] = {};
    PersistentGeom geo;
    if (persistent_geometry(conv3d_wino_up2_kernel, 256, wu::LDS_BYTES, 1, geo_cache, "conv3d(winograd up2)", geo)) return 1;
    long long nwalk = geo.cus / 16;
    const long long most = cdiv(units, 8);
    if (nwalk > most) nwalk = most;
    if (nwalk < 1) nwalk = 1;
    hipLaunchKernelGGL(conv3d_wino_up2_kernel, dim3((unsigned)(16 * nwalk)), dim3(256), wu::LDS_BYTES, st, a);
    return check_launch("mvsgi_conv3d_up2_poly(winograd main)");
}

}
```

mvs_gi_amd/dropin/cost_volume_regulator.py:

```python
from __future__ import annotations

import copy
import os
from typing import Sequence

from torch import nn, Tensor

from .. import hip_ops as H
from . import common_modules as cm
from .common_modules import NORM3D_TYPE, RELU_TYPE


class UNetDownBlk(nn.Module):
    def __init__(self, in_chs: int, out_chs: int, kernel_size: int, width: int,
                 activation: nn.Module = cm.NoOp(), norm_layer: nn.Module = cm.NoOp()):
        super().__init__()
        self.k_sz = kernel_size
        self.first = cm.BaseConvBlk3d(in_chs, out_chs, kernel_size, stride=2,
                                      activation=copy.deepcopy(activation), norm_layer=copy.deepcopy(norm_layer))
        self.blks = nn.Sequential(*[
            cm.ResConvBlk3d(out_chs, out_chs, kernel_size, activation=copy.deepcopy(activation),
                            norm_layer=copy.deepcopy(norm_layer)) for _ in range(width - 1)])

    __getstate__ = cm.module_getstate

    def forward(self, x: Tensor) -> Tensor:
        return cm._to_ncdhw_view(down_block_ndhwc(self, H.as_ndhwc(x)))


_USE_RS = True
_USE_WINO = os.environ.get("MVSGI_WINO", "1") != "0"
_WINO_A32 = True


def _rs_chain(blk, x: Tensor):
    if not (_USE_RS and H.split_mode() and len(blk.blks) > 0):
        return None
    L0 = cm.lower_conv_block(blk.first)
    if L0.cin % 16 or L0.cout != 32 or L0.inorm is not None:
        return None
    B, D, Hh, W, _ = x.shape
    s = L0.stride
    Do, Ho, Wo = (D - 1) // s + 1, (Hh - 1) // s + 1, (W - 1) // s + 1
    chain = []
    for rb in blk.blks:
        if not cm._is_identity(rb.one_by_one) or getattr(rb, "out_pad", 0) != 0:
            return None
        L1, L2 = cm.lower_conv_block(rb.blk1), cm.lower_conv_block(rb.blk2)
        if not (L1.rs_ok() and L2.rs_ok()):
            return None
        chain.append((L1, L2))
    return L0, chain, (B, Do, Ho, Wo)


_CUS = {}


def _cu_count(device) -> int:
    import torch
    key = str(device)
    if key not in _CUS:
        _CUS[key] = torch.cuda.get_device_properties(device).multi_processor_count
    return _CUS[key]


def _wino_pays(B: int, Ho: int, Wo: int, device) -> bool:
    units = B * (Ho // 2) * (Wo // 32)
    cus = _cu_count(device)
    rounds = -(-units // cus)
    return units >= 0.7 * rounds * cus


def _down_block_rs(blk, x: Tensor, L0, chain, dims) -> Tensor:
    B, Do, Ho, Wo = dims
    b = cm._owned_split_buffer(blk, "_mvsgi_rs_bufs", (B, Do, Ho, Wo, x.device),
                               lambda: [H.SplitAct(B, Do, Ho, Wo, 32, x.device) for _ in range(3)])
    fmt = H.mode_fmt()
    wino = fmt == "f16" and _USE_WINO and _wino_pays(B, Ho, Wo, x.device) and \
        all(L1.wino_ok(Do, Ho, Wo) and L2.wino_ok(Do, Ho, Wo) for L1, L2 in chain)
    if isinstance(x, H.SplitAct):
        if x.fmt != fmt:
            raise RuntimeError(f"split-padded cost volume holds {x.fmt} pieces, the library's mode writes {fmt}")
        p0 = L0._s2(fmt)
        H.conv3d_s2rs(x, p0.wp, p0.shift, out=b[0], neg_slope=L0.neg_slope, unscale=p0.unscale, out_f32p=wino and _WINO_A32)
    else:
        p0 = L0._stream_packed(H.CONV_BF16X3, fmt)
        H.conv3d_out_split(x, p0.wp, p0.scale, L0.shift, out=b[0], stride=L0.stride, neg_slope=L0.neg_slope, fmt=fmt)
    conv = H.conv3d_wino if wino else H.conv3d_rs
    cur, out = 0, None
    for i, (L1, L2) in enumerate(chain):
        r, y = (cur + 1) % 3, (cur + 2) % 3
        p1 = L1._wino() if wino else L1._rs(fmt)
        p2 = L2._wino() if wino else L2._rs(fmt)
        conv(b[cur], p1.wp, p1.scale, L1.shift, neg_slope=L1.neg_slope, out=b[r])
        if i == len(chain) - 1:
            out = conv(b[r], p2.wp, p2.scale, L2.shift, res=b[cur], neg_slope=L2.neg_slope, out_f32=True)
        else:
            conv(b[r], p2.wp, p2.scale, L2.shift, res=b[cur], neg_slope=L2.neg_slope, out=b[y])
            cur = y
    return out


_USE_S2RS = os.environ.get("MVSGI_S2RS", "1") != "0"


class _Shape:
    __slots__ = ("shape",)

    def __init__(self, shape):
        self.shape = tuple(shape)


def regulator_takes_split(self, shape) -> bool:
    if not (_USE_S2RS and H.split_mode() and len(self.down_blks) > 0 and len(shape) == 5 and shape[4] == 16):
        return False
    blk = self.down_blks[0]
    return cm.lower_conv_block(blk.first).s2rs_ok() and _rs_chain(blk, _Shape(shape)) is not None


def regulator_forward_split_in(self, xs) -> Tensor:
    if not regulator_takes_split(self, xs.shape):
        raise RuntimeError(f"this regulator does not take a split-padded volume of geometry {xs.shape}: call forward() with the fp32 tensor")
    return cm._to_ncdhw_view(regulator_forward_ndhwc(self, xs))


def down_block_ndhwc(blk, x) -> Tensor:
    rs = _rs_chain(blk, x)
    if rs is not None:
        return _down_block_rs(blk, x, *rs)
    if isinstance(x, H.SplitAct):
        raise RuntimeError("split-padded input needs the register-stationary level-0 chain (regulator_takes_split)")
    x = cm.lower_conv_block(blk.first).run(x)
    for rb in blk.blks:
        x = cm.res_block_ndhwc(rb, x)
    return x


_USE_POLY = os.environ.get("MVSGI_POLY", "1") != "0"
_HEAD_SPLIT = os.environ.get("MVSGI_HEAD_SPLIT", "1") != "0"
_POLY_MIN_UNITS = 1600


def _poly_tail(self, x: Tensor, skip: Tensor):
    if not (_USE_POLY and len(self.upBlks) > 0):
        return None
    up, oc = self.upBlks[len(self.upBlks) - 1], self.out_costs[0]
    Lu, Lo = cm.lower_conv_block(up.conv), cm.lower_conv_block(oc.conv)
    if not (Lo.poly_ok() and Lu.can_fuse_up2() and Lu.inorm is None and Lu.cout == 32 and oc.scale == 2 and oc.out_pad == 0 and up.scale == 2 and up.out_pad == 0):
        return None
    B, Dl, Hl, Wl, _ = x.shape
    if tuple(skip.shape[1:4]) != (2 * Dl, 2 * Hl, 2 * Wl):
        return None
    if B * ((2 * Dl + 1) // 2) * ((2 * Hl + 3) // 4) * ((2 * Wl + 15) // 16) < _POLY_MIN_UNITS:
        return None
    xs = Lu.run_up2_split(x, skip, cm._owned_split_buffer(self, "_mvsgi_poly_bufs", (B, 2 * Dl, 2 * Hl, 2 * Wl, x.device),
                                                          lambda: H.SplitAct(B, 2 * Dl, 2 * Hl, 2 * Wl, 32, x.device)))
    Lh = cm.lower_conv_block(self.out_costs[1])
    if _HEAD_SPLIT and Lh.head_split_ok() and Lh.cin == 16:
        hi = cm._owned_split_buffer(self, "_mvsgi_poly_bufs", (B, 4 * Dl, 4 * Hl, 4 * Wl, "hi", x.device),
                                    lambda: H.SplitAct(B, 4 * Dl, 4 * Hl, 4 * Wl, 16, x.device))
        return Lh.run_head_split(Lo.run_up2_poly_split(xs, hi))
    return Lh.run(Lo.run_up2_poly(xs))


def regulator_forward_ndhwc(self, x: Tensor) -> Tensor:
    skips = []
    n_down = len(self.down_blks)
    for i, blk in enumerate(self.down_blks):
        x = down_block_ndhwc(blk, x)
        if i != n_down - 1:
            skips.append(x)
    skips.reverse()
    n_up = len(self.upBlks)
    for i, up in enumerate(self.upBlks):
        if i == n_up - 1:
            y = _poly_tail(self, x, skips[i])
            if y is not None:
                return y
        x = cm.resize_conv_ndhwc(up, x, res=skips[i])
    y = _split_head_tail(self, x)
    if y is not None:
        return y
    x = cm.resize_conv_ndhwc(self.out_costs[0], x)
    return cm.lower_conv_block(self.out_costs[1]).run(x)


def _split_head_tail(self, x: Tensor):
    oc = self.out_costs[0]
    Lo, Lh = cm.lower_conv_block(oc.conv), cm.lower_conv_block(self.out_costs[1])
    if not (_HEAD_SPLIT and Lh.head_split_ok() and Lo.can_fuse_up2() and Lo.inorm is None and oc.scale == 2 and oc.out_pad == 0 and Lh.cin == Lo.cout):
        return None
    B, Dl, Hl, Wl, _ = x.shape
    if (2 * Dl + 2) * (2 * Hl + 4) * (2 * Wl + 4) * Lo.cout * 4 >= 2 ** 31:
        return None
    return Lh.run_head_split(Lo.run_up2_split(x, None, cm._owned_head_buffer(self, B, 2 * Dl, 2 * Hl, 2 * Wl, Lo.cout, x.device)))


def regulator_forward(self, x: Tensor) -> Tensor:
    H.check_range("cv_regulator: an earlier call")
    return cm._to_ncdhw_view(regulator_forward_ndhwc(self, H.as_ndhwc(x)))


class UNetCostVolumeRegulatorBase(nn.Module):
    def __init__(self, in_chs: int = 16, f_int_chs: int = 32, final_chs: int = 1, u_depth: int = 3,
                 blk_width: int = 4, stage_factor: int = 2, cost_k_sz: int = 3, keep_last_chs: Sequence[int] = [],
                 deconv_k_sz: int = 3, norm_type: str = "batch", relu_type: str = "leaky"):
        super().__init__()
        self.in_chs, self.f_int_chs, self.final_chs = in_chs, f_int_chs, final_chs
        self.u_depth, self.blkWidth, self.stage_factor = u_depth, blk_width, stage_factor
        self.k_sz, self.keep_last_chs, self.deconv_k_sz = cost_k_sz, keep_last_chs, deconv_k_sz
        self.norm_type = NORM3D_TYPE[norm_type]
        self.relu_type = RELU_TYPE[relu_type]

        self._int_chs = []
        downs = []
        cin, cout = in_chs, f_int_chs
        for lvl in range(u_depth):
            if lvl != 0 and lvl not in keep_last_chs:
                cout *= stage_factor
            downs.append(UNetDownBlk(cin, cout, cost_k_sz, blk_width, activation=self.relu_type(),
                                     norm_layer=self.norm_type(cout)))
            self._int_chs.append(cout)
            cin = cout
        self.down_blks = nn.ModuleList(downs)

        rev = self._int_chs[::-1]
        self.upBlks = nn.ModuleList([
            cm.ResizeConv3d(rev[i], rev[i + 1], deconv_k_sz, stride=2, activation=self.relu_type(),
                            norm_layer=self.norm_type(rev[i + 1])) for i in range(u_depth - 1)])
        self.out_costs = nn.Sequential(
            cm.ResizeConv3d(self._int_chs[0], in_chs, deconv_k_sz, stride=2, activation=self.relu_type(),
                            norm_layer=self.norm_type(in_chs)),
            cm.BaseConvBlk3d(in_chs, final_chs, deconv_k_sz, bias_on=True, activation=cm.NoOp(),
                             norm_layer=cm.NoOp()))

    forward = regulator_forward
    takes_split = regulator_takes_split
    forward_split_in = regulator_forward_split_in
    __getstate__ = cm.module_getstate


class UNetCostVolumeRegulator(nn.Module):
    def __init__(self, in_chs: int, final_chs: int, u_depth: int, blk_width: int, stage_factor: int,
                 cost_k_sz: int, keep_last_chs: Sequence[int], deconv_k_sz: int, sweep_fuse_ch_reduce: int = 2,
                 num_cams: int = 3, only_one_cam: bool = False, norm_type: str = "batch", relu_type: str = "leaky"):
        super().__init__()
        self.in_chs = in_chs if only_one_cam else (in_chs * num_cams) // sweep_fuse_ch_reduce
        self.final_chs, self.u_depth, self.blkWidth = final_chs, u_depth, blk_width
        self.stage_factor, self.k_sz = stage_factor, cost_k_sz
        self.keep_last_chs, self.deconv_k_sz = keep_last_chs, deconv_k_sz
        self.norm_type = NORM3D_TYPE[norm_type]
        self.relu_type = RELU_TYPE[relu_type]

        downs = []
        cin = cout = self.in_chs
        for lvl in range(u_depth):
            if lvl not in keep_last_chs:
                cout *= stage_factor
            downs.append(UNetDownBlk(cin, cout, cost_k_sz, blk_width, activation=self.relu_type(),
                                     norm_layer=self.norm_type(cout)))
            if lvl not in keep_last_chs:
                cin *= stage_factor
        self.down_blks = nn.ModuleList(downs)

        top = self.in_chs * stage_factor ** (u_depth - len(keep_last_chs))
        ups = []
        cin = cout = top
        for i in range(u_depth - 1):
            if i + 1 not in keep_last_chs:
                cout //= stage_factor
            ups.append(cm.ResizeConv3d(cin, cout, deconv_k_sz, stride=2, activation=self.relu_type(),
                                       norm_layer=self.norm_type(cout)))
            if i + 1 not in keep_last_chs:
                cin //= stage_factor
        self.upBlks = nn.ModuleList(ups)
        self.out_costs = nn.Sequential(
            cm.ResizeConv3d(2 * self.in_chs, self.in_chs, deconv_k_sz, stride=2, activation=self.relu_type(),
                            norm_layer=self.norm_type(self.in_chs)),
            cm.BaseConvBlk3d(self.in_chs, final_chs, deconv_k_sz, bias_on=True, activation=cm.NoOp(),
                             norm_layer=cm.NoOp()))

    forward = regulator_forward
    takes_split = regulator_takes_split
    forward_split_in = regulator_forward_split_in
    __getstate__ = cm.module_getstate
```

mvs_gi_amd/hip_ops.py:

```python
from __future__ import annotations

from typing import Optional

import torch

from . import _lib

import math
import os

CONV_AUTO, CONV_DIRECT, CONV_MFMA, CONV_BF16X3, CONV_BF16X3_C16, CONV_BF16X3_V32, CONV_BF16X3_D32 = 0, 1, 2, 3, 4, 5, 6
SPLIT_F16 = 1
CONV_F16 = 0x100

CONV_MODES = ("f32", "bf16x3", "f16x3")
_CONV_MODE = os.environ.get("MVSGI_CONV_MODE", "f16x3")
if _CONV_MODE not in CONV_MODES:
    raise ValueError(f"MVSGI_CONV_MODE={_CONV_MODE!r} not in {CONV_MODES}")




def set_conv_mode(mode: str) -> None:
    global _CONV_MODE
    if mode not in CONV_MODES:
        raise ValueError(f"conv mode {mode!r} not in {CONV_MODES}")
    _CONV_MODE = mode


def get_conv_mode() -> str:
    return _CONV_MODE


SAT_SWEEP, SAT_SPLIT, SAT_WINO = 1, 2, 4
_SAT_TEXT = {SAT_SWEEP: "the sweep's cost volume reached +-65504 (un-normalised features?)",
             SAT_SPLIT: "an activation written or staged in fp16 pieces reached +-65504",
             SAT_WINO: "an activation of the Winograd-form level reached its +-16376 range (or a transformed sum +-65504)"}
RANGE_CHECKS = ("raise", "warn", "off")
_RANGE_CHECK = os.environ.get("MVSGI_RANGE_CHECK", "raise")
if _RANGE_CHECK not in RANGE_CHECKS:
    raise ValueError(f"MVSGI_RANGE_CHECK={_RANGE_CHECK!r} not in {RANGE_CHECKS}")
_RANGE_WARNED = set()
_RANGE_SEEN = 0


class MvsgiRangeError(RuntimeError):
    """The fp16 split left its range: results since the last check are saturated, not the reference's."""


def set_range_check(policy: str) -> None:
    global _RANGE_CHECK
    if policy not in RANGE_CHECKS:
        raise ValueError(f"range check policy {policy!r} not in {RANGE_CHECKS}")
    _RANGE_CHECK = policy


def get_range_check() -> str:
    return _RANGE_CHECK


def saturation_flags(clear: bool = False) -> int:
    import ctypes
    out = ctypes.c_uint(0)
    if _lib.load().mvsgi_saturation_flags(1 if clear else 0, ctypes.byref(out)) != 0:
        return 0
    return int(out.value)


def saturation_words():
    import ctypes
    out = (ctypes.c_uint * 8)()
    if _lib.load().mvsgi_saturation_words(out) != 0:
        return [0] * 8
    return [int(v) for v in out]


def range_flags_seen() -> int:
    return _RANGE_SEEN


def check_range(where: str = "", sync_device=None) -> int:
    if _RANGE_CHECK == "off":
        return 0
    if sync_device is not None:
        torch.cuda.synchronize(sync_device)
    f = saturation_flags(clear=False)
    if not f:
        return 0
    words = saturation_words()
    saturation_flags(clear=True)
    global _RANGE_SEEN
    _RANGE_SEEN |= f
    what = "; ".join(t for b, t in _SAT_TEXT.items() if f & b)
    msg = (f"mvs_gi_amd{' (' + where + ')' if where else ''}: the fp16 split (MVSGI_CONV_MODE=f16x3, the default) left its range (flags 0x{f:x}, words {words[:4]}) -- {what}. "
           "Results computed since the last check are saturated, not the reference's fp32 results "
           "(dsta_mvs/model/common/common_modules.py:105-115 has no clamp). Re-run with MVSGI_CONV_MODE=bf16x3 "
           "(hip_ops.set_conv_mode('bf16x3'): fp32's range, ~8x the rounding error) or 'f32'; HotPath.precision_check(frames) measures "
           "which arithmetic a checkpoint needs. MVSGI_RANGE_CHECK=warn|off relaxes this check.")
    if _RANGE_CHECK == "raise":
        raise MvsgiRangeError(msg)
    if f not in _RANGE_WARNED:
        _RANGE_WARNED.add(f)
        import warnings
        warnings.warn(msg, RuntimeWarning, stacklevel=2)
    return f


def split_mode() -> bool:
    return _CONV_MODE in ("bf16x3", "f16x3")


def mode_fmt() -> str:
    return "f16" if _CONV_MODE == "f16x3" else "bf16"


def _fmt_code(fmt: str) -> int:
    if fmt not in ("bf16", "f16"):
        raise ValueError(f"split format {fmt!r} not in ('bf16', 'f16')")
    return SPLIT_F16 if fmt == "f16" else 0


def _pow2_unscale(amax: torch.Tensor):
    k = torch.where(amax > 0, torch.floor(torch.log2(1024.0 / amax.clamp_min(1e-37))), torch.zeros_like(amax)).clamp(-100.0, 100.0)
    return torch.exp2(k), torch.exp2(-k)


def _stream_ptr(t: torch.Tensor) -> int:
    return torch.cuda.current_stream(t.device).cuda_stream


def _dev(t: torch.Tensor, name: str, dtype=torch.float32) -> torch.Tensor:
    if not isinstance(t, torch.Tensor):
        raise TypeError(f"{name}: expected a torch.Tensor, got {type(t)}")
    if not t.is_cuda:
        raise RuntimeError(f"{name}: mvs_gi_amd runs on the GPU only (tensor is on {t.device}); "
                           "there is no CPU fallback")
    if t.dtype != dtype:
        raise TypeError(f"{name}: expected {dtype}, got {t.dtype}")
    if not t.is_contiguous():
        t = t.contiguous()
    if t.data_ptr() % 16:
        t = t.clone()
    return t


def _ptr(t: Optional[torch.Tensor]) -> Optional[int]:
    return None if t is None else t.data_ptr()


def _call(name: str, *args) -> None:
    _lib.check(getattr(_lib.load(), name)(*args), name)


def _feats_nhwc(feats):
    if feats.dim() != 5:
        raise AssertionError(f"feats must be [B, N, C, Hi, Wi], got {tuple(feats.shape)}")
    v = feats.permute(0, 1, 3, 4, 2)
    if v.is_contiguous() and v.data_ptr() % 16 == 0 and v.is_cuda and v.dtype == torch.float32:
        return v
    f = _dev(feats, "feats")
    B, N, C, Hi, Wi = f.shape
    y = torch.empty((B, N, Hi, Wi, C), device=f.device, dtype=torch.float32)
    _call("mvsgi_ncv_to_nvc_f32", f.data_ptr(), y.data_ptr(), B * N, C, Hi * Wi, _stream_ptr(f))
    return y


def nhwc_sweep_ok(feats) -> bool:
    return feats.dim() == 5 and feats.shape[2] % 4 == 0 and feats.shape[1] <= 4


def sweep_max_cams() -> int:
    return int(_lib.load().mvsgi_sweep_max_cams())


def valid_sweep_ok(feats) -> bool:
    return feats.dim() == 5 and feats.shape[2] % 4 == 0 and 1 <= feats.shape[1] <= sweep_max_cams()


def _rig_args(grids, grid_masks, masks, B: int, N: int):
    grids = _dev(grids, "grids")
    masks = _dev(masks, "masks")
    if grid_masks.dtype in (torch.bool, torch.uint8):
        gm, gm_f32 = _dev(grid_masks, "grid_masks", grid_masks.dtype), 0
    else:
        gm, gm_f32 = _dev(grid_masks.to(torch.float32) if grid_masks.dtype != torch.float32 else grid_masks, "grid_masks"), 1
    Bg, Ng, D, Ho, Wo, two = grids.shape
    if (Bg, Ng, two) != (B, N, 2):
        raise AssertionError(f"grids {tuple(grids.shape)} must be [{B}, {N}, D, Ho, Wo, 2]")
    if tuple(gm.shape[:5]) != (B, N, D, Ho, Wo) or gm.numel() != B * N * D * Ho * Wo:
        raise AssertionError(f"grid_masks {tuple(gm.shape)} do not match grids {tuple(grids.shape)}")
    if masks.shape[0] != B or masks.shape[1] != N or masks.numel() != B * N * masks.shape[-2] * masks.shape[-1]:
        raise AssertionError(f"masks {tuple(masks.shape)} do not match grids {tuple(grids.shape)}")
    return grids, gm, gm_f32, masks, (D, Ho, Wo) + tuple(masks.shape[-2:])


def sweep_validity(grids, grid_masks, masks) -> torch.Tensor:
    B, N = grids.shape[:2]
    if N > sweep_max_cams():
        raise AssertionError(f"grids must be [B, N<={sweep_max_cams()}, D, Ho, Wo, 2], got {tuple(grids.shape)}")
    grids, gm, gm_f32, masks, (D, Ho, Wo, Hm, Wm) = _rig_args(grids, grid_masks, masks, B, N)
    vmask = torch.empty((B, D, Ho, Wo), device=grids.device, dtype=torch.uint8)
    _call("mvsgi_sweep_validity_u8", grids.data_ptr(), gm.data_ptr(), gm_f32, masks.data_ptr(), vmask.data_ptr(),
          B, N, Hm, Wm, D, Ho, Wo, _stream_ptr(grids))
    return vmask


def sweep_std_valid(feats, grids, vmask) -> torch.Tensor:
    if not valid_sweep_ok(feats):
        raise AssertionError(f"sweep_std_valid needs C % 4 == 0 and num_cams in [1, {sweep_max_cams()}], got feats {tuple(feats.shape)}")
    B, N, C, Hi, Wi = feats.shape
    f = _feats_nhwc(feats)
    grids = _dev(grids, "grids")
    vmask = _dev(vmask, "vmask", torch.uint8)
    Bg, Ng, D, Ho, Wo, two = grids.shape
    if (Ng, two) != (N, 2) or Bg not in (1, B):
        raise AssertionError(f"grids {tuple(grids.shape)} do not match feats {tuple(feats.shape)}")
    if tuple(vmask.shape) != (Bg, D, Ho, Wo):
        raise AssertionError(f"vmask {tuple(vmask.shape)} does not match grids {tuple(grids.shape)}")
    vol = torch.empty((B, D, Ho, Wo, C), device=f.device, dtype=torch.float32)
    _call("mvsgi_sweep_std_nhwc_valid_rig_f32" if (Bg == 1 and B > 1) else "mvsgi_sweep_std_nhwc_valid_f32",
          f.data_ptr(), grids.data_ptr(), vmask.data_ptr(), vol.data_ptr(), B, N, C, Hi, Wi, D, Ho, Wo, _stream_ptr(f))
    return vol


def sweep_std_valid_split(feats, grids, vmask, out: "SplitAct", fmt: str = "bf16") -> "SplitAct":
    if not valid_sweep_ok(feats):
        raise AssertionError(f"sweep_std_valid_split needs C == 16 and num_cams in [1, {sweep_max_cams()}], got feats {tuple(feats.shape)}")
    B, N, C, Hi, Wi = feats.shape
    f = _feats_nhwc(feats)
    grids = _dev(grids, "grids")
    vmask = _dev(vmask, "vmask", torch.uint8)
    Bg, Ng, D, Ho, Wo, two = grids.shape
    if (Ng, two) != (N, 2) or Bg not in (1, B) or tuple(vmask.shape) != (Bg, D, Ho, Wo) or C != 16:
        raise AssertionError(f"grids {tuple(grids.shape)} / vmask {tuple(vmask.shape)} do not match feats {tuple(feats.shape)}")
    if out.shape != (B, D, Ho, Wo, C):
        raise AssertionError(f"split output {out.shape} does not match {(B, D, Ho, Wo, C)}")
    _call("mvsgi_sweep_std_nhwc_valid_split_fmt", f.data_ptr(), grids.data_ptr(), vmask.data_ptr(), out.buf.data_ptr(), B, N, C, Hi, Wi, D, Ho, Wo,
          Bg, _fmt_code(fmt), _stream_ptr(f))
    out.fmt = fmt
    return out


def sweep_std(feats, grids, grid_masks, masks, layout: str = "auto") -> torch.Tensor:
    if feats.dim() != 5:
        raise AssertionError(f"feats must be [B, N, C, Hi, Wi], got {tuple(feats.shape)}")
    if not 1 <= feats.shape[1] <= sweep_max_cams():
        raise AssertionError(f"sweep_std: num_cams {feats.shape[1]} not in [1, {sweep_max_cams()}]")
    nhwc = layout == "auto" and nhwc_sweep_ok(feats)
    if layout == "auto" and not nhwc and valid_sweep_ok(feats):
        if tuple(grids.shape[:2]) != tuple(feats.shape[:2]):
            raise AssertionError(f"grids {tuple(grids.shape)} must be [{feats.shape[0]}, {feats.shape[1]}, D, Ho, Wo, 2]")
        return sweep_std_valid(feats, grids, sweep_validity(grids, grid_masks, masks))
    B, N, C, Hi, Wi = feats.shape
    f = _feats_nhwc(feats) if nhwc else _dev(feats, "feats")
    grids, gm, gm_f32, masks, (D, Ho, Wo, Hm, Wm) = _rig_args(grids, grid_masks, masks, B, N)
    vol = torch.empty((B, D, Ho, Wo, C), device=f.device, dtype=torch.float32)
    _call("mvsgi_sweep_std_nhwc_f32" if nhwc else "mvsgi_sweep_std_f32", f.data_ptr(), grids.data_ptr(), gm.data_ptr(), gm_f32,
          masks.data_ptr(), vol.data_ptr(), B, N, C, Hi, Wi, Hm, Wm, D, Ho, Wo, _stream_ptr(f))
    return vol


def sweep_cat(feats, grids, layout: str = "auto") -> torch.Tensor:
    nhwc = layout == "auto" and feats.dim() == 5 and feats.shape[2] % 4 == 0
    f = _feats_nhwc(feats) if nhwc else _dev(feats, "feats")
    B, N, C, Hi, Wi = feats.shape
    grids = _dev(grids, "grids")
    Bg, Ng, D, Ho, Wo, two = grids.shape
    if (Bg, Ng, two) != (B, N, 2):
        raise AssertionError(f"grids {tuple(grids.shape)} do not match feats {tuple(feats.shape)}")
    vol = torch.empty((B, D, Ho, Wo, N * C), device=f.device, dtype=torch.float32)
    _call("mvsgi_sweep_cat_nhwc_f32" if nhwc else "mvsgi_sweep_cat_f32", f.data_ptr(), grids.data_ptr(), vol.data_ptr(), B, N, C, Hi, Wi,
          D, Ho, Wo, _stream_ptr(f))
    return vol


def pack_conv_weights(w_oidhw: torch.Tensor) -> Optional[torch.Tensor]:
    lib = _lib.load()
    w = _dev(w_oidhw, "conv weight")
    Cout, Cin = w.shape[:2]
    if tuple(w.shape[2:]) != (3, 3, 3):
        raise NotImplementedError(f"only 3x3x3 kernels are supported, got {tuple(w.shape[2:])}")
    if Cin % 16 or not (Cout % 16 == 0 or Cout == 1):
        return None
    wp = torch.empty(lib.mvsgi_conv3d_packed_weight_floats(Cout, Cin), device=w.device, dtype=torch.float32)
    _call("mvsgi_conv3d_pack_weights_f32", w.data_ptr(), wp.data_ptr(), Cout, Cin, _stream_ptr(w))
    return wp


def _pack_conv3d_split(w_oidhw: torch.Tensor, layout: int, fmt: str = "bf16"):
    lib = _lib.load()
    w = _dev(w_oidhw, "conv weight")
    Cout, Cin = w.shape[:2]
    if tuple(w.shape[2:]) != (3, 3, 3) or Cin % 16 or Cout % 16 or (layout == CONV_BF16X3_C16 and Cout != 16) or \
            (layout == CONV_BF16X3_V32 and Cout % 32) or (layout == CONV_BF16X3_D32 and Cin % 32):
        return None
    unscale = None
    if fmt == "f16":
        up, unscale = _pow2_unscale(w.abs().amax(dim=(1, 2, 3, 4)))
        w = (w * up.view(-1, 1, 1, 1, 1)).contiguous()
    n = {CONV_BF16X3: lambda: lib.mvsgi_conv3d_packed_weight_bytes_bf16x3(Cout, Cin),
         CONV_BF16X3_C16: lambda: lib.mvsgi_conv3d_packed_weight_bytes_bf16x3_c16(Cin),
         CONV_BF16X3_D32: lambda: lib.mvsgi_conv3d_packed_weight_bytes_bf16x3(Cout, Cin),
         CONV_BF16X3_V32: lambda: lib.mvsgi_conv3d_packed_weight_bytes_bf16x3_v32(Cout, Cin)}[layout]()
    wp = torch.empty(n, device=w.device, dtype=torch.uint8)
    _call("mvsgi_conv3d_pack_weights_split", w.data_ptr(), wp.data_ptr(), Cout, Cin, layout | (CONV_F16 if _fmt_code(fmt) else 0),
          _stream_ptr(w))
    return wp, (None if unscale is None else unscale.contiguous())


def _pack_bf16(w_oidhw: torch.Tensor, layout: int) -> Optional[torch.Tensor]:
    p = _pack_conv3d_split(w_oidhw, layout)
    return None if p is None else p[0]


def pack_conv_weights_bf16x3(w_oidhw: torch.Tensor) -> Optional[torch.Tensor]:
    return _pack_bf16(w_oidhw, CONV_BF16X3)


def pack_conv_weights_f16x3(w_oidhw: torch.Tensor, layout: int = CONV_BF16X3):
    return _pack_conv3d_split(w_oidhw, layout, "f16")


def pack_conv_weights_bf16x3_d32(w_oidhw: torch.Tensor) -> Optional[torch.Tensor]:
    return _pack_bf16(w_oidhw, CONV_BF16X3_D32)


def pack_conv_weights_bf16x3_v32(w_oidhw: torch.Tensor) -> Optional[torch.Tensor]:
    return _pack_bf16(w_oidhw, CONV_BF16X3_V32)


def pack_conv_weights_bf16x3_c16(w_oidhw: torch.Tensor) -> Optional[torch.Tensor]:
    return _pack_bf16(w_oidhw, CONV_BF16X3_C16)


def conv3d_d32_applies(B, Cin, Din, Hin, Win, Cout, stride=1) -> bool:
    return bool(_lib.load().mvsgi_conv3d_d32_applies(B, Cin, Din, Hin, Win, Cout, stride))


def conv3d_up2_d32_applies(B, Cin, Dl, Hl, Wl, Cout) -> bool:
    return bool(_lib.load().mvsgi_conv3d_up2_d32_applies(B, Cin, Dl, Hl, Wl, Cout))


def conv3d_v32_applies(B, Cin, Din, Hin, Win, Cout, stride=1) -> bool:
    return bool(_lib.load().mvsgi_conv3d_v32_applies(B, Cin, Din, Hin, Win, Cout, stride))


def conv3d(x, w_oidhw, w_packed, scale, shift, res=None, stride=1, neg_slope=0.01, impl=CONV_AUTO, out=None):
    x = _dev(x, "x")
    B, Din, Hin, Win, Cin = x.shape
    Cout = scale.numel()
    Do, Ho, Wo = (Din - 1) // stride + 1, (Hin - 1) // stride + 1, (Win - 1) // stride + 1
    if res is not None:
        res = _dev(res, "res")
        if tuple(res.shape) != (B, Do, Ho, Wo, Cout):
            raise AssertionError(f"residual {tuple(res.shape)} does not match output {(B, Do, Ho, Wo, Cout)}")
    y = out if out is not None else torch.empty((B, Do, Ho, Wo, Cout), device=x.device, dtype=torch.float32)
    _call("mvsgi_conv3d_f32", x.data_ptr(), _ptr(w_oidhw), _ptr(w_packed), scale.data_ptr(), shift.data_ptr(), _ptr(res), y.data_ptr(), B, Cin, Din,
          Hin, Win, Cout, stride, float(neg_slope), impl, _stream_ptr(x))
    return y


def conv3d_up2(x, w_packed_b3, scale, shift, res=None, neg_slope=0.01, out=None, w_layout=CONV_BF16X3):
    x = _dev(x, "x")
    B, Dl, Hl, Wl, Cin = x.shape
    Cout = scale.numel()
    shp = (B, 2 * Dl, 2 * Hl, 2 * Wl, Cout)
    if res is not None:
        res = _dev(res, "res")
        if tuple(res.shape) != shp:
            raise AssertionError(f"residual {tuple(res.shape)} does not match output {shp}")
    y = out if out is not None else torch.empty(shp, device=x.device, dtype=torch.float32)
    _call("mvsgi_conv3d_up2_f32", x.data_ptr(), _ptr(w_packed_b3), w_layout, scale.data_ptr(), shift.data_ptr(), _ptr(res), y.data_ptr(), B, Cin, Dl,
          Hl, Wl, Cout, float(neg_slope), _stream_ptr(x))
    return y


def conv3d_up2_out_split(x, w_packed_b3, scale, shift, out: "SplitAct", res=None, neg_slope=0.01, w_layout=CONV_BF16X3) -> "SplitAct":
    x = _dev(x, "x")
    B, Dl, Hl, Wl, Cin = x.shape
    Cout = scale.numel()
    if out.shape != (B, 2 * Dl, 2 * Hl, 2 * Wl, Cout):
        raise AssertionError(f"split output {out.shape} does not match {(B, 2 * Dl, 2 * Hl, 2 * Wl, Cout)}")
    if res is not None:
        res = _dev(res, "res")
        if tuple(res.shape) != out.shape:
            raise AssertionError(f"residual {tuple(res.shape)} does not match output {out.shape}")
    _call("mvsgi_conv3d_up2_f32_out_split", x.data_ptr(), _ptr(w_packed_b3), w_layout, scale.data_ptr(), shift.data_ptr(), _ptr(res),
          out.buf.data_ptr(), B, Cin, Dl, Hl, Wl, Cout, float(neg_slope), _stream_ptr(x))
    out.fmt = "f16" if w_layout & CONV_F16 else "bf16"
    return out


def conv3d_up2_poly_applies(cin: int, cout: int, neg_slope: float) -> bool:
    return cin == 32 and cout == 16 and 0.0 <= neg_slope <= 1.0


def conv3d_up2_poly_plan(w_oidhw: torch.Tensor, D: int, H: int, W: int, fmt: str = "bf16"):
    lib = _lib.load()
    if tuple(w_oidhw.shape) != (16, 32, 3, 3, 3):
        raise AssertionError(f"polyphase plan needs a [16, 32, 3, 3, 3] weight, got {tuple(w_oidhw.shape)}")
    n = lib.mvsgi_conv3d_up2_poly_plan_bytes(D, H, W)
    if not n:
        raise RuntimeError("mvsgi_conv3d_up2_poly_plan_bytes: bad dims")
    wh = w_oidhw.detach().to("cpu", torch.float32).contiguous()
    unscale = None
    if fmt == "f16":
        up, un = _pow2_unscale(wh.abs().amax(dim=(1, 2, 3, 4)))
        wh = (wh * up.view(-1, 1, 1, 1, 1)).contiguous()
        unscale = un.to(w_oidhw.device)
    plan = torch.empty(n, dtype=torch.uint8)
    _call("mvsgi_conv3d_up2_poly_plan_fmt", wh.data_ptr(), plan.data_ptr(), D, H, W, _fmt_code(fmt))
    plan = plan.to(w_oidhw.device)
    return (plan, unscale) if fmt == "f16" else plan


def conv3d_up2_poly(x: "SplitAct", plan: torch.Tensor, scale, shift, neg_slope=0.01, out=None) -> torch.Tensor:
    if x.C != 32 or scale.numel() != 16:
        raise AssertionError("conv3d_up2_poly is the 32 -> 16 kernel")
    shp = (x.B, 2 * x.D, 2 * x.H, 2 * x.W, 16)
    y = out if out is not None else torch.empty(shp, device=x.buf.device, dtype=torch.float32)
    if tuple(y.shape) != shp or not y.is_contiguous():
        raise AssertionError(f"output {tuple(y.shape)} does not match {shp}")
    _call("mvsgi_conv3d_up2_poly_fmt", x.buf.data_ptr(), plan.data_ptr(), scale.data_ptr(), shift.data_ptr(), y.data_ptr(), 0, x.B, x.D, x.H, x.W,
          float(neg_slope), _fmt_code(x.fmt), _stream_ptr(x.buf))
    return y


POLY_WINO = os.environ.get("MVSGI_POLY_WINO", "1") != "0"


def conv3d_up2_poly_wino_pays(B: int, D: int, Hh: int, W: int) -> bool:
    return POLY_WINO and bool(_lib.load().mvsgi_conv3d_up2_poly_wino_pays(int(B), int(D), int(Hh), int(W)))


def conv3d_up2_poly_split(x: "SplitAct", plan: torch.Tensor, scale, shift, out: "SplitAct", neg_slope=0.01, direct: bool = False,
                          wino: bool = False) -> "SplitAct":
    if x.C != 32 or scale.numel() != 16 or out.shape != (x.B, 2 * x.D, 2 * x.H, 2 * x.W, 16):
        raise AssertionError(f"conv3d_up2_poly_split: input {x.shape}, output {out.shape}")
    _call("mvsgi_conv3d_up2_poly_fmt", x.buf.data_ptr(), plan.data_ptr(), scale.data_ptr(), shift.data_ptr(), out.buf.data_ptr(),
          5 if wino else (3 if (direct or not POLY_WINO) else 1), x.B, x.D, x.H, x.W, float(neg_slope), _fmt_code(x.fmt), _stream_ptr(x.buf))
    out.fmt = x.fmt
    return out


def pack_head_split_weights(w_oidhw: torch.Tensor) -> Optional[torch.Tensor]:
    lib = _lib.load()
    w = _dev(w_oidhw, "conv weight")
    if w.shape[0] != 1 or tuple(w.shape[2:]) != (3, 3, 3) or w.shape[1] % 16:
        return None
    wp = torch.empty(lib.mvsgi_conv3d_head_split_packed_weight_bytes(int(w.shape[1])), device=w.device, dtype=torch.uint8)
    _call("mvsgi_conv3d_head_split_pack_weights", w.data_ptr(), wp.data_ptr(), int(w.shape[1]), _stream_ptr(w))
    return wp


def pack_head_split_weights_f16(w_oidhw: torch.Tensor):
    lib = _lib.load()
    w = _dev(w_oidhw, "conv weight")
    if w.shape[0] != 1 or tuple(w.shape[2:]) != (3, 3, 3) or w.shape[1] % 16:
        return None
    amax = float(w.abs().max())
    k = 0.0 if amax == 0.0 else float(torch.floor(torch.log2(torch.tensor(1024.0 / amax))))
    ws = (w * (2.0 ** k)).contiguous()
    wp = torch.empty(lib.mvsgi_conv3d_head_split_packed_weight_bytes(int(w.shape[1])), device=w.device, dtype=torch.uint8)
    _call("mvsgi_conv3d_head_split_pack_weights_f16", ws.data_ptr(), wp.data_ptr(), int(w.shape[1]), _stream_ptr(w))
    return wp, 2.0 ** -k


def conv3d_head_split(x: "SplitAct", w_packed, scale: float, shift: float, neg_slope=1.0, out=None, f16: bool = False) -> torch.Tensor:
    if x.fmt != ("f16" if f16 else "bf16"):
        raise AssertionError(f"conv3d_head_split(f16={f16}) on a split-padded buffer holding {x.fmt} pieces")
    y = out if out is not None else torch.empty((x.B, x.D, x.H, x.W, 1), device=x.buf.device, dtype=torch.float32)
    if tuple(y.shape) != (x.B, x.D, x.H, x.W, 1) or not y.is_contiguous():
        raise AssertionError(f"head output {tuple(y.shape)} does not match {(x.B, x.D, x.H, x.W, 1)}")
    _call("mvsgi_conv3d_head_split_f16" if f16 else "mvsgi_conv3d_head_split", x.buf.data_ptr(), w_packed.data_ptr(), float(scale),
          float(shift), y.data_ptr(), x.B, x.C, x.D, x.H, x.W, float(neg_slope), _stream_ptr(x.buf))
    return y


def conv3d_up2_variant(B, Cin, Dl, Hl, Wl, Cout, w_layout=CONV_BF16X3) -> str:
    lib = _lib.load()
    name = lib.mvsgi_conv3d_up2_variant_f32(B, Cin, Dl, Hl, Wl, Cout, w_layout)
    if name is None:
        raise RuntimeError("mvsgi_conv3d_up2_variant_f32: " + lib.mvsgi_last_error().decode())
    return name.decode()


def conv3d_variant(B, Cin, Din, Hin, Win, Cout, stride=1, impl=CONV_AUTO) -> str:
    lib = _lib.load()
    name = lib.mvsgi_conv3d_variant_f32(B, Cin, Din, Hin, Win, Cout, stride, impl)
    if name is None:
        raise RuntimeError("mvsgi_conv3d_variant_f32: " + lib.mvsgi_last_error().decode())
    return name.decode()


class SplitAct:
    __slots__ = ("buf", "B", "D", "H", "W", "C", "fmt")

    def __init__(self, B, D, H, W, C, device, buf=None):
        self.B, self.D, self.H, self.W, self.C = int(B), int(D), int(H), int(W), int(C)
        self.fmt = "bf16"
        if buf is None:
            buf = torch.zeros((self.B, self.D + 2, self.H + 2, self.W + 2, self.C), device=device, dtype=torch.int32)
        self.buf = buf

    @property
    def shape(self):
        return (self.B, self.D, self.H, self.W, self.C)

    @property
    def device(self):
        return self.buf.device


def act_to_split(x_ndhwc: torch.Tensor, out: Optional[SplitAct] = None, fmt: str = "bf16") -> SplitAct:
    x = _dev(x_ndhwc, "x")
    B, D, Hh, W, C = x.shape
    y = out if out is not None else SplitAct(B, D, Hh, W, C, x.device)
    if y.shape != (B, D, Hh, W, C):
        raise AssertionError(f"split buffer {y.shape} does not match {tuple(x.shape)}")
    _call("mvsgi_act_f32_to_split_fmt", x.data_ptr(), y.buf.data_ptr(), B, C, D, Hh, W, _fmt_code(fmt), _stream_ptr(x))
    y.fmt = fmt
    return y


def act_from_split(x: SplitAct, out: Optional[torch.Tensor] = None) -> torch.Tensor:
    y = out if out is not None else torch.empty(x.shape, device=x.buf.device, dtype=torch.float32)
    _call("mvsgi_act_split_to_f32_fmt", x.buf.data_ptr(), y.data_ptr(), x.B, x.C, x.D, x.H, x.W, _fmt_code(x.fmt), _stream_ptr(x.buf))
    return y


def pack_conv_weights_rs(w_oidhw: torch.Tensor, fmt: str = "bf16"):
    lib = _lib.load()
    w = _dev(w_oidhw, "conv weight")
    unscale = None
    if fmt == "f16":
        up, unscale = _pow2_unscale(w.abs().amax(dim=(1, 2, 3, 4)))
        w = (w * up.view(-1, 1, 1, 1, 1)).contiguous()
    Cout, Cin = w.shape[:2]
    nbytes = lib.mvsgi_conv3d_rs_packed_weight_bytes(Cout, Cin) if tuple(w.shape[2:]) == (3, 3, 3) else 0
    if not nbytes:
        return None
    wp = torch.empty(nbytes, device=w.device, dtype=torch.uint8)
    _call("mvsgi_conv3d_rs_pack_weights_fmt", w.data_ptr(), wp.data_ptr(), Cout, Cin, _fmt_code(fmt), _stream_ptr(w))
    return (wp, unscale.contiguous()) if fmt == "f16" else wp


def conv3d_rs(x: SplitAct, w_packed_rs, scale, shift, res: Optional[SplitAct] = None, neg_slope=0.01,
              out=None, out_f32: bool = False):
    Cout = scale.numel()
    if out_f32:
        y = out if out is not None else torch.empty((x.B, x.D, x.H, x.W, Cout), device=x.buf.device, dtype=torch.float32)
        yp = y.data_ptr()
        if tuple(y.shape) != (x.B, x.D, x.H, x.W, Cout) or not y.is_contiguous():
            raise AssertionError(f"fp32 output {tuple(y.shape)} does not match {(x.B, x.D, x.H, x.W, Cout)}")
    else:
        y = out if out is not None else SplitAct(x.B, x.D, x.H, x.W, Cout, x.buf.device)
        yp = y.buf.data_ptr()
        if y.shape != (x.B, x.D, x.H, x.W, Cout):
            raise AssertionError(f"split output {y.shape} does not match {(x.B, x.D, x.H, x.W, Cout)}")
    if res is not None and (res.shape != (x.B, x.D, x.H, x.W, Cout) or res.fmt != x.fmt):
        raise AssertionError(f"residual {res.shape} ({res.fmt}) does not match the output ({x.fmt})")
    _call("mvsgi_conv3d_rs_split_fmt", x.buf.data_ptr(), w_packed_rs.data_ptr(), scale.data_ptr(), shift.data_ptr(),
          None if res is None else res.buf.data_ptr(), yp, int(out_f32), x.B, x.C, x.D, x.H, x.W, Cout, float(neg_slope), _fmt_code(x.fmt),
          _stream_ptr(x.buf))
    if not out_f32:
        y.fmt = x.fmt
    return y


def conv3d_wino_applies(cin, cout, D, Hh, W, stride, neg_slope) -> bool:
    return bool(_lib.load().mvsgi_conv3d_wino32_applies(int(cin), int(cout), int(D), int(Hh), int(W), int(stride), float(neg_slope)))


def pack_conv_weights_wino(w_oidhw: torch.Tensor):
    lib = _lib.load()
    w = _dev(w_oidhw, "conv weight")
    if tuple(w.shape) != (32, 32, 3, 3, 3):
        return None
    wp = torch.empty(lib.mvsgi_conv3d_wino32_packed_weight_bytes(), device=w.device, dtype=torch.uint8)
    unscale = torch.empty(32, device=w.device, dtype=torch.float32)
    _call("mvsgi_conv3d_wino32_pack_weights", w.data_ptr(), wp.data_ptr(), unscale.data_ptr(), _stream_ptr(w))
    return wp, unscale


F32P_MAX = 16376.0


def act_to_f32p(x_ndhwc: torch.Tensor, out: Optional[SplitAct] = None) -> SplitAct:
    x = _dev(x_ndhwc, "x")
    B, D, Hh, W, C = x.shape
    y = out if out is not None else SplitAct(B, D, Hh, W, C, x.device)
    y.buf.view(torch.float32)[:, 1:-1, 1:-1, 1:-1, :] = x.clamp(-F32P_MAX, F32P_MAX)
    y.fmt = "f32p"
    return y


def act_from_f32p(x: SplitAct) -> torch.Tensor:
    if x.fmt != "f32p":
        raise AssertionError(f"buffer holds {x.fmt} records")
    return x.buf.view(torch.float32)[:, 1:-1, 1:-1, 1:-1, :].contiguous()


def conv3d_wino(x: SplitAct, w_packed, scale, shift, res: Optional[SplitAct] = None, neg_slope=0.01, out=None, out_f32: bool = False,
                ):
    lib = _lib.load()
    if x.fmt not in ("f16", "f32p") or x.C != 32:
        raise AssertionError(f"conv3d_wino: needs a 32-channel input in the fp16 split or fp32-padded (got {x.C}, {x.fmt})")
    if out_f32:
        y = out if out is not None else torch.empty(x.shape, device=x.buf.device, dtype=torch.float32)
        if tuple(y.shape) != x.shape or not y.is_contiguous() or y.dtype != torch.float32:
            raise AssertionError(f"fp32 output {tuple(y.shape)} does not match {x.shape}")
        yp = y.data_ptr()
    else:
        y = out if out is not None else SplitAct(x.B, x.D, x.H, x.W, 32, x.buf.device)
        if y.shape != x.shape:
            raise AssertionError(f"split output {y.shape} does not match {x.shape}")
        yp = y.buf.data_ptr()
    if res is not None and (res.shape != x.shape or res.fmt != x.fmt):
        raise AssertionError(f"residual {res.shape} ({res.fmt}) does not match the input ({x.fmt})")
    if w_packed.numel() != lib.mvsgi_conv3d_wino32_packed_weight_bytes():
        raise AssertionError("conv3d_wino: packed weights of the wrong size")
    _call("mvsgi_conv3d_wino32_f16", x.buf.data_ptr(), w_packed.data_ptr(), scale.data_ptr(), shift.data_ptr(),
          None if res is None else res.buf.data_ptr(), yp, int(out_f32), int(x.fmt == "f32p"), x.B, x.D, x.H, x.W, float(neg_slope),
          _stream_ptr(x.buf))
    if not out_f32:
        y.fmt = x.fmt
    return y


def conv3d_out_split(x, w_packed_b3, scale, shift, out: "SplitAct", res=None, stride=1, neg_slope=0.01, fmt: str = "bf16") -> "SplitAct":
    x = _dev(x, "x")
    B, Din, Hin, Win, Cin = x.shape
    Cout = scale.numel()
    Do, Ho, Wo = (Din - 1) // stride + 1, (Hin - 1) // stride + 1, (Win - 1) // stride + 1
    if out.shape != (B, Do, Ho, Wo, Cout):
        raise AssertionError(f"split output {out.shape} does not match {(B, Do, Ho, Wo, Cout)}")
    if res is not None:
        res = _dev(res, "res")
    _call("mvsgi_conv3d_f32_out_split_fmt", x.data_ptr(), w_packed_b3.data_ptr(), scale.data_ptr(), shift.data_ptr(), _ptr(res), out.buf.data_ptr(),
          B, Cin, Din, Hin, Win, Cout, stride, float(neg_slope), _fmt_code(fmt), _stream_ptr(x))
    out.fmt = fmt
    return out


def conv3d_rs16(x: "SplitAct", w_packed_rs, scale, shift, neg_slope=0.01, out=None, out_split: Optional["SplitAct"] = None):
    if x.C != 16 or scale.numel() != 16:
        raise AssertionError("conv3d_rs16 is the 16 -> 16 kernel")
    if out_split is not None:
        if out_split.shape != x.shape or out_split.buf.data_ptr() == x.buf.data_ptr():
            raise AssertionError(f"split output {out_split.shape} must match the input {x.shape} and be another buffer")
        _call("mvsgi_conv3d_rs16_split_fmt", x.buf.data_ptr(), w_packed_rs.data_ptr(), scale.data_ptr(), shift.data_ptr(), out_split.buf.data_ptr(),
              1, x.B, x.D, x.H, x.W, float(neg_slope), _fmt_code(x.fmt), _stream_ptr(x.buf))
        out_split.fmt = x.fmt
        return out_split
    y = out if out is not None else torch.empty((x.B, x.D, x.H, x.W, 16), device=x.buf.device, dtype=torch.float32)
    _call("mvsgi_conv3d_rs16_split_fmt", x.buf.data_ptr(), w_packed_rs.data_ptr(), scale.data_ptr(), shift.data_ptr(), y.data_ptr(), 0, x.B, x.D,
          x.H, x.W, float(neg_slope), _fmt_code(x.fmt), _stream_ptr(x.buf))
    return y


def conv3d_s2rs_applies(cin: int, cout: int, stride: int, neg_slope: float) -> bool:
    return cin == 16 and cout == 32 and stride == 2 and 0.0 <= neg_slope <= 1.0


def pack_conv_weights_s2rs(w_oidhw: torch.Tensor, scale: torch.Tensor, fmt: str = "bf16"):
    lib = _lib.load()
    w = _dev(w_oidhw, "w")
    scale = _dev(scale, "scale")
    if tuple(w.shape) != (32, 16, 3, 3, 3) or scale.numel() != 32:
        raise AssertionError(f"conv3d_s2rs is the 16 -> 32 channel stride-2 layer, got weights {tuple(w.shape)}")
    up = un = None
    if fmt == "f16":
        up_t, un_t = _pow2_unscale((w.abs().amax(dim=(1, 2, 3, 4)) * scale.abs()).max().reshape(1))
        up, un = float(up_t[0]), float(un_t[0])
        scale = (scale * up).contiguous()
    wp = torch.empty(lib.mvsgi_conv3d_s2rs_packed_weight_bytes(), device=w.device, dtype=torch.uint8)
    _call("mvsgi_conv3d_s2rs_pack_weights_fmt", w.data_ptr(), scale.data_ptr(), wp.data_ptr(), _fmt_code(fmt), _stream_ptr(w))
    return (wp, up, un) if fmt == "f16" else wp


def conv3d_s2rs(x: "SplitAct", w_packed, shift, out: "SplitAct", neg_slope=0.01, unscale: float = 1.0, out_f32p: bool = False) -> "SplitAct":
    Do, Ho, Wo = (x.D - 1) // 2 + 1, (x.H - 1) // 2 + 1, (x.W - 1) // 2 + 1
    if x.C != 16 or out.shape != (x.B, Do, Ho, Wo, 32) or shift.numel() != 32:
        raise AssertionError(f"conv3d_s2rs: input {x.shape} -> output {out.shape}, expected {(x.B, Do, Ho, Wo, 32)}")
    _call("mvsgi_conv3d_s2rs_out_fmt", x.buf.data_ptr(), w_packed.data_ptr(), shift.data_ptr(), out.buf.data_ptr(), x.B, x.D, x.H, x.W,
          float(neg_slope), float(unscale), _fmt_code(x.fmt), int(out_f32p), _stream_ptr(x.buf))
    out.fmt = "f32p" if out_f32p else x.fmt
    return out


def conv3d_rs_applies(cin: int, cout: int, stride: int, neg_slope: float) -> bool:
    return cin == 32 and cout == 32 and stride == 1 and 0.0 <= neg_slope <= 1.0


def pack_conv2d_weights_bf16x3(w_oihw: torch.Tensor) -> Optional[torch.Tensor]:
    lib = _lib.load()
    w = _dev(w_oihw, "conv weight")
    Cout, Cin = w.shape[:2]
    if tuple(w.shape[2:]) != (3, 3) or Cin % 16 or Cout % 16:
        return None
    wp = torch.empty(lib.mvsgi_conv2d_packed_weight_bytes_bf16x3(Cout, Cin), device=w.device, dtype=torch.uint8)
    _call("mvsgi_conv2d_pack_weights_bf16x3", w.data_ptr(), wp.data_ptr(), Cout, Cin, _stream_ptr(w))
    return wp


def pack_conv2d_stem_weights(w_oihw: torch.Tensor) -> Optional[torch.Tensor]:
    lib = _lib.load()
    w = _dev(w_oihw, "conv weight")
    if tuple(w.shape) != (16, 3, 5, 5):
        return None
    wp = torch.empty(lib.mvsgi_conv2d_stem_packed_weight_bytes(), device=w.device, dtype=torch.uint8)
    _call("mvsgi_conv2d_stem_pack_weights", w.data_ptr(), wp.data_ptr(), _stream_ptr(w))
    return wp


def pack_conv2d_weights_f32(w_oihw: torch.Tensor) -> Optional[torch.Tensor]:
    lib = _lib.load()
    w = _dev(w_oihw, "conv weight")
    Cout, Cin = w.shape[:2]
    if tuple(w.shape[2:]) != (3, 3) or Cin % 16 or Cout not in (16, 32):
        return None
    wp = torch.empty(lib.mvsgi_conv2d_packed_weight_floats(Cout, Cin), device=w.device, dtype=torch.float32)
    _call("mvsgi_conv2d_pack_weights_f32", w.data_ptr(), wp.data_ptr(), Cout, Cin, _stream_ptr(w))
    return wp


def conv2d(x, w_oihw, w_packed, scale, shift, res=None, stride=1, neg_slope=0.01, impl=CONV_AUTO, in_nchw=False, out_split=None):
    layout = int(bool(in_nchw))
    if x.dtype == torch.uint8:
        x = _dev(x, "imgs", torch.uint8)
        B, Hin, Win, Cin = x.shape
        layout = 2
    else:
        x = _dev(x, "x")
        if in_nchw:
            B, Cin, Hin, Win = x.shape
        else:
            B, Hin, Win, Cin = x.shape
    Cout, k = scale.numel(), int(w_oihw.shape[-1])
    pad = k // 2
    Ho, Wo = (Hin + 2 * pad - k) // stride + 1, (Win + 2 * pad - k) // stride + 1
    if res is not None:
        res = _dev(res, "res")
        if tuple(res.shape) != (B, Ho, Wo, Cout):
            raise AssertionError(f"residual {tuple(res.shape)} does not match output {(B, Ho, Wo, Cout)}")
    if out_split is not None:
        _check_split2d(out_split, B, Ho, Wo, x.device)
        _call("mvsgi_conv2d_f32_out_split2d", x.data_ptr(), _ptr(w_oihw), _ptr(w_packed), scale.data_ptr(), shift.data_ptr(), _ptr(res),
              out_split.data_ptr(), B, Cin, Hin, Win, Cout, k, stride, float(neg_slope), impl, layout, _stream_ptr(x))
        return out_split
    y = torch.empty((B, Ho, Wo, Cout), device=x.device, dtype=torch.float32)
    _call("mvsgi_conv2d_f32", x.data_ptr(), _ptr(w_oihw), _ptr(w_packed), scale.data_ptr(), shift.data_ptr(), _ptr(res), y.data_ptr(), B, Cin, Hin,
          Win, Cout, k, stride, float(neg_slope), impl, layout, _stream_ptr(x))
    return y


def conv2d_variant(Cin, Cout, k=3, stride=1, impl=CONV_AUTO, in_nchw=False) -> str:
    lib = _lib.load()
    name = lib.mvsgi_conv2d_variant_f32(Cin, Cout, k, stride, impl, int(bool(in_nchw)))
    if name is None:
        raise RuntimeError("mvsgi_conv2d_variant_f32: " + lib.mvsgi_last_error().decode())
    return name.decode()


def resize_trilinear(x, size) -> torch.Tensor:
    x = _dev(x, "x")
    B, Di, Hi, Wi, C = x.shape
    Do, Ho, Wo = (int(s) for s in size)
    y = torch.empty((B, Do, Ho, Wo, C), device=x.device, dtype=torch.float32)
    _call("mvsgi_resize_trilinear_f32", x.data_ptr(), y.data_ptr(), B, C, Di, Hi, Wi, Do, Ho, Wo, _stream_ptr(x))
    return y


def _images(imgs, m: str, count=None, device=None):
    if not isinstance(imgs, torch.Tensor) or imgs.dtype not in (torch.uint8, torch.float32):
        raise TypeError(f"imgs: expected a uint8 [{m}, Hr, Wr, 3] or fp32 [{m}, C, Hr, Wr] tensor, got {getattr(imgs, 'dtype', type(imgs))}")
    u8 = imgs.dtype == torch.uint8
    imgs = _dev(imgs, "imgs", imgs.dtype)
    if imgs.dim() != 4 or (u8 and imgs.shape[3] != 3) or (count is not None and imgs.shape[0] != count) or \
            (device is not None and imgs.device != device):
        lead = m if count is None else count
        where, got_where = ("", "") if device is None else (f" on {device}", f" on {imgs.device}")
        raise AssertionError(f"imgs must be uint8 [{lead}, Hr, Wr, 3] or fp32 [{lead}, C, Hr, Wr]{where}, got {imgs.dtype} "
                             f"{tuple(imgs.shape)}{got_where}")
    C, Hr, Wr = (imgs.shape[3], imgs.shape[1], imgs.shape[2]) if u8 else tuple(imgs.shape[1:])
    return imgs, u8, C, Hr, Wr


def resample_validity(grid, in_fov) -> torch.Tensor:
    if not isinstance(grid, torch.Tensor) or grid.dtype != torch.float32:
        raise TypeError(f"grid: expected a fp32 tensor, got {getattr(grid, 'dtype', type(grid))}")
    if not isinstance(in_fov, torch.Tensor) or in_fov.dtype not in (torch.bool, torch.uint8):
        raise TypeError(f"in_fov: expected a bool or uint8 tensor, got {getattr(in_fov, 'dtype', type(in_fov))}")
    if grid.dim() < 2 or grid.shape[-1] != 2 or tuple(in_fov.shape) != tuple(grid.shape[:-1]) or in_fov.device != grid.device:
        raise AssertionError(f"grid must be [..., 2] and in_fov its leading shape on one device, got {tuple(grid.shape)} on {grid.device}, "
                             f"{tuple(in_fov.shape)} on {in_fov.device}")
    grid, in_fov = _dev(grid, "grid"), _dev(in_fov, "in_fov", in_fov.dtype)
    valid = torch.empty(in_fov.shape, device=grid.device, dtype=torch.uint8)
    _call("mvsgi_resample_validity_u8", grid.data_ptr(), in_fov.data_ptr(), valid.data_ptr(), valid.numel(), _stream_ptr(grid))
    return valid


def resample_bilinear(imgs, grid, valid, invalid_value: float = 0.0, out=None) -> torch.Tensor:
    imgs, u8, C, Hr, Wr = _images(imgs, "M")
    M = imgs.shape[0]
    grid = _dev(grid, "grid")
    if not isinstance(valid, torch.Tensor) or valid.dtype not in (torch.bool, torch.uint8):
        raise TypeError(f"valid: expected a bool or uint8 tensor, got {getattr(valid, 'dtype', type(valid))}")
    valid = _dev(valid, "valid", valid.dtype)
    if grid.dim() != 4 or grid.shape[3] != 2 or tuple(valid.shape) != tuple(grid.shape[:3]):
        raise AssertionError(f"grid must be [T, H, W, 2] and valid [T, H, W], got {tuple(grid.shape)}, {tuple(valid.shape)}")
    T, Ho, Wo = valid.shape
    if out is None:
        out = torch.empty((M, C, Ho, Wo), device=imgs.device, dtype=torch.float32)
    elif tuple(out.shape) != (M, C, Ho, Wo) or out.dtype != torch.float32 or out.device != imgs.device or not out.is_contiguous() \
            or out.data_ptr() % 16:
        raise AssertionError(f"out must be a contiguous, 16-byte aligned fp32 [{M}, {C}, {Ho}, {Wo}] tensor on {imgs.device}")
    if u8:
        _call("mvsgi_resample_bilinear_u8_f32", imgs.data_ptr(), grid.data_ptr(), valid.data_ptr(), out.data_ptr(), M, T, Hr, Wr, Ho, Wo,
              float(invalid_value), _stream_ptr(imgs))
    else:
        _call("mvsgi_resample_bilinear_f32", imgs.data_ptr(), grid.data_ptr(), valid.data_ptr(), out.data_ptr(), M, T, C, Hr, Wr, Ho, Wo,
              float(invalid_value), _stream_ptr(imgs))
    return out


REPROJECT_CAM_FLOATS = 10


def reproject(inv, rays, T, cams, bf: float, imgs=None, invalid_value: float = 0.0, want=("xyz", "warped", "valid"), out=None) -> dict:
    inv = _dev(inv, "inv")
    rays = _dev(rays, "rays")
    if inv.dim() == 4 and inv.shape[1] == 1:
        inv = inv.squeeze(1)
    if inv.dim() != 3 or rays.dim() != 3 or rays.shape[0] != 3 or tuple(rays.shape[1:]) != tuple(inv.shape[1:]) or rays.device != inv.device:
        raise AssertionError(f"inv must be [B, H, W] and rays [3, H, W] on one device, got {tuple(inv.shape)}, {tuple(rays.shape)}")
    B, Ho, Wo = inv.shape
    T = torch.as_tensor(T)
    cams = torch.as_tensor(cams)
    if T.is_cuda or cams.is_cuda or T.dtype != torch.float32 or cams.dtype != torch.float32:
        raise TypeError("T and cams are fp32 host tensors (they travel in the kernel's arguments)")
    N = T.shape[0] if T.dim() == 3 else -1
    if tuple(T.shape) != (N, 4, 4) or tuple(cams.shape) != (N, REPROJECT_CAM_FLOATS):
        raise AssertionError(f"T must be [N, 4, 4] and cams [N, {REPROJECT_CAM_FLOATS}], got {tuple(T.shape)}, {tuple(cams.shape)}")
    if not 1 <= N <= sweep_max_cams():
        raise ValueError(f"reproject: {N} cameras (1 ... {sweep_max_cams()} are supported)")
    T, cams = T.contiguous(), cams.contiguous()
    want = tuple(want)
    if not want or set(want) - {"xyz", "warped", "valid", "grid"} or len(set(want)) != len(want):
        raise ValueError(f"want: a non-empty selection of 'xyz', 'warped', 'valid', 'grid', got {want}")
    kind, C, Hr, Wr = 0, 0, 0, 0
    if "warped" in want:
        imgs, u8, C, Hr, Wr = _images(imgs, "B*N", count=B * N, device=inv.device)
        kind = 0 if u8 else 1
    elif imgs is not None:
        raise ValueError("reproject: imgs given but 'warped' is not wanted")
    shapes = {"xyz": ((B, 3, Ho, Wo), torch.float32), "warped": ((B, N, C, Ho, Wo), torch.float32),
              "valid": ((B, N, Ho, Wo), torch.bool), "grid": ((B, N, Ho, Wo, 2), torch.float32)}
    res = {}
    for k in want:
        shape, dtype = shapes[k]
        t = None if out is None else out.get(k)
        if t is None:
            t = torch.empty(shape, device=inv.device, dtype=dtype)
        elif tuple(t.shape) != shape or t.dtype != dtype or t.device != inv.device or not t.is_contiguous() or t.data_ptr() % 16:
            raise AssertionError(f"out['{k}'] must be a contiguous, 16-byte aligned {dtype} {list(shape)} tensor on {inv.device}")
        res[k] = t
    _call("mvsgi_reproject_f32", inv.data_ptr(), rays.data_ptr(), _ptr(imgs) if "warped" in want else None, kind, T.data_ptr(),
          cams.data_ptr(), _ptr(res.get("xyz")), _ptr(res.get("warped")), _ptr(res.get("valid")), _ptr(res.get("grid")), B, N, C, Hr, Wr,
          Ho, Wo, float(bf), float(invalid_value), _stream_ptr(inv))
    return res


def instance_norm(x, res=None, gamma=None, beta=None, eps: float = 1e-5, neg_slope: float = 1.0, out=None) -> torch.Tensor:
    lib = _lib.load()
    x = _dev(x, "x")
    B, C = int(x.shape[0]), int(x.shape[-1])
    S = x.numel() // max(B * C, 1)
    if S < 2:
        raise ValueError(f"Expected more than 1 spatial element when training, got input size "
                         f"{[B, C] + list(x.shape[1:-1])}")
    if res is not None:
        res = _dev(res, "res")
        if tuple(res.shape) != tuple(x.shape):
            raise AssertionError(f"residual {tuple(res.shape)} does not match {tuple(x.shape)}")
    for t, name in ((gamma, "gamma"), (beta, "beta")):
        if t is not None and (t.numel() != C or not t.is_cuda or t.dtype != torch.float32 or not t.is_contiguous()):
            raise AssertionError(f"{name} must be a contiguous fp32 [{C}] device tensor")
    if out is None:
        out = torch.empty_like(x)
    elif out.data_ptr() != x.data_ptr():
        out = _dev(out, "out")
        if tuple(out.shape) != tuple(x.shape) or out.data_ptr() % 16:
            raise AssertionError(f"out {tuple(out.shape)} does not match {tuple(x.shape)}")
    nbytes = lib.mvsgi_instance_norm_ws_bytes(B, S, C)
    ws = torch.empty(max(int(nbytes), 16), device=x.device, dtype=torch.uint8)
    _call("mvsgi_instance_norm_f32", x.data_ptr(), _ptr(res), _ptr(gamma), _ptr(beta), out.data_ptr(), ws.data_ptr(), B, S, C, float(eps),
          float(neg_slope), _stream_ptr(x))
    return out


SA_AUTO, SA_PIXEL, SA_BAND = 0, 1, 2


def softargmin(costs_bdhw, inv_idx, scale: float, want_norm_costs: bool, post_div: float = 1.0, variant: int = SA_AUTO):
    c = _dev(costs_bdhw, "costs")
    inv_idx = _dev(inv_idx.reshape(-1), "inv_dist_idx")
    B, D, H, W = c.shape
    if inv_idx.numel() != D:
        raise AssertionError(f"{D} cost planes but {inv_idx.numel()} distance candidates")
    scale = float(scale)
    if not (math.isfinite(scale) and scale > 0):
        raise ValueError(f"softargmin: scale {scale} is not a finite positive factor")
    OH, OW = math.floor(H * scale), math.floor(W * scale)
    if OH < 1 or OW < 1:
        raise ValueError(f"softargmin: scale {scale} gives an empty {OH} x {OW} output for {H} x {W}")
    inv = torch.empty((B, 1, OH, OW), device=c.device, dtype=torch.float32)
    pr = torch.empty((B, D, OH, OW), device=c.device, dtype=torch.float32) if want_norm_costs else None
    if variant == SA_AUTO and scale in (1.0, 2.0):
        _call("mvsgi_softargmin_div_f32", c.data_ptr(), inv_idx.data_ptr(), inv.data_ptr(), _ptr(pr), B, D, H, W, int(scale), float(post_div),
              _stream_ptr(c))
    else:
        _call("mvsgi_softargmin_scaled_f32", c.data_ptr(), inv_idx.data_ptr(), inv.data_ptr(), _ptr(pr), B, D, H, W, scale, OH, OW, float(post_div),
              int(variant), _stream_ptr(c))
    return inv, pr


def ncdhw_to_ndhwc(x) -> torch.Tensor:
    x = _dev(x, "x")
    B, C, D, H, W = x.shape
    y = torch.empty((B, D, H, W, C), device=x.device, dtype=torch.float32)
    _call("mvsgi_ncv_to_nvc_f32", x.data_ptr(), y.data_ptr(), B, C, D * H * W, _stream_ptr(x))
    return y


def ndhwc_to_ncdhw(x) -> torch.Tensor:
    x = _dev(x, "x")
    B, D, H, W, C = x.shape
    y = torch.empty((B, C, D, H, W), device=x.device, dtype=torch.float32)
    _call("mvsgi_nvc_to_ncv_f32", x.data_ptr(), y.data_ptr(), B, C, D * H * W, _stream_ptr(x))
    return y


def as_ndhwc(vol: torch.Tensor) -> torch.Tensor:
    if vol.dim() != 5:
        raise AssertionError(f"expected a [B, C, D, H, W] volume, got {tuple(vol.shape)}")
    v = vol.permute(0, 2, 3, 4, 1)
    if v.is_contiguous():
        return v
    return ncdhw_to_ndhwc(vol.contiguous())


def pack_deform_conv2d_weights(w_oihw: torch.Tensor) -> torch.Tensor:
    w = _dev(w_oihw, "deform conv weight")
    Cout, Cin, Kh, Kw = w.shape
    wp = torch.empty((Kh * Kw, Cin, Cout), device=w.device, dtype=torch.float32)
    _call("mvsgi_deform_conv2d_pack_weights_f32", w.data_ptr(), wp.data_ptr(), Cout, Cin, Kh, Kw, _stream_ptr(w))
    return wp


def deform_conv2d(x_nhwc, offset, w_packed, scale, shift, kernel_size, stride=(1, 1), padding=(0, 0), dilation=(1, 1),
                  res=None, neg_slope=1.0) -> torch.Tensor:
    x = _dev(x_nhwc, "x")
    offset = _dev(offset, "offset")
    N, Hh, W, Cin = x.shape
    Kh, Kw = kernel_size
    Cout = scale.numel()
    Ho = (Hh + 2 * padding[0] - (dilation[0] * (Kh - 1) + 1)) // stride[0] + 1
    Wo = (W + 2 * padding[1] - (dilation[1] * (Kw - 1) + 1)) // stride[1] + 1
    if offset.dim() != 4 or tuple(offset.shape[1:]) != (2 * Kh * Kw, Ho, Wo) or offset.shape[0] not in (1, N):
        raise AssertionError(f"offset {tuple(offset.shape)} does not match [1|{N}, {2 * Kh * Kw}, {Ho}, {Wo}]")
    if tuple(w_packed.shape) != (Kh * Kw, Cin, Cout):
        raise AssertionError(f"w_packed {tuple(w_packed.shape)} does not match {(Kh * Kw, Cin, Cout)}")
    if res is not None:
        res = _dev(res, "res")
        if tuple(res.shape) != (N, Ho, Wo, Cout):
            raise AssertionError(f"residual {tuple(res.shape)} does not match output {(N, Ho, Wo, Cout)}")
    y = torch.empty((N, Ho, Wo, Cout), device=x.device, dtype=torch.float32)
    _call("mvsgi_deform_conv2d_f32", x.data_ptr(), offset.data_ptr(), int(offset.shape[0] == N and N > 1), w_packed.data_ptr(), scale.data_ptr(),
          shift.data_ptr(), _ptr(res), y.data_ptr(), N, Cin, Hh, W, Cout, Kh, Kw, stride[0], stride[1], padding[0], padding[1], dilation[0],
          dilation[1], float(neg_slope), _stream_ptr(x))
    return y


def split2d_buffer(N: int, H: int, W: int, device) -> torch.Tensor:
    return torch.zeros((N, H + 4, W + 4, 64), device=device, dtype=torch.uint8)


def _check_split2d(t: torch.Tensor, N: int, H: int, W: int, device) -> None:
    if t.dtype != torch.uint8 or tuple(t.shape) != (N, H + 4, W + 4, 64) or not t.is_contiguous() or t.device != device:
        raise AssertionError(f"split-padded 2-D buffer {tuple(t.shape)} {t.dtype} {t.device} does not match {(N, H + 4, W + 4, 64)} uint8 on {device}")


def f32_to_split2d(x_nhwc: torch.Tensor, out: Optional[torch.Tensor] = None) -> torch.Tensor:
    x = _dev(x_nhwc, "x")
    N, Hh, W, C = x.shape
    if C != 16:
        raise AssertionError(f"the 2-D split-padded format holds 16 channels, got {tuple(x.shape)}")
    if out is None:
        out = split2d_buffer(N, Hh, W, x.device)
    _check_split2d(out, N, Hh, W, x.device)
    _call("mvsgi_f32_to_split2d", x.data_ptr(), out.data_ptr(), N, Hh, W, _stream_ptr(x))
    return out


def split2d_to_f32(x_split: torch.Tensor) -> torch.Tensor:
    N, Hp, Wp, _ = x_split.shape
    _check_split2d(x_split, N, Hp - 4, Wp - 4, x_split.device)
    y = torch.empty((N, Hp - 4, Wp - 4, 16), device=x_split.device, dtype=torch.float32)
    _call("mvsgi_split2d_to_f32", x_split.data_ptr(), y.data_ptr(), N, Hp - 4, Wp - 4, _stream_ptr(x_split))
    return y


def pack_resblock2d_split_weights(w_oihw: torch.Tensor, scale: torch.Tensor) -> torch.Tensor:
    lib = _lib.load()
    w = _dev(w_oihw, "w")
    scale = _dev(scale, "scale")
    if tuple(w.shape) != (16, 16, 3, 3) or scale.numel() != 16:
        raise AssertionError(f"resblock2d_split is the 16 -> 16 channel 3x3 block, got weights {tuple(w.shape)}")
    wp = torch.empty(lib.mvsgi_resblock2d_split_packed_weight_bytes(), device=w.device, dtype=torch.uint8)
    _call("mvsgi_resblock2d_split_pack_weights", w.data_ptr(), scale.data_ptr(), wp.data_ptr(), _stream_ptr(w))
    return wp


def resblock2d_split(x_split, wp1, shift1, wp2, shift2, neg_slope=0.01, out_split=None) -> torch.Tensor:
    N, Hp, Wp, _ = x_split.shape
    Hh, W = Hp - 4, Wp - 4
    _check_split2d(x_split, N, Hh, W, x_split.device)
    if shift1.numel() != 16 or shift2.numel() != 16:
        raise AssertionError("resblock2d_split is the 16-channel block")
    if out_split is not None:
        _check_split2d(out_split, N, Hh, W, x_split.device)
        y = out_split
    else:
        y = torch.empty((N, Hh, W, 16), device=x_split.device, dtype=torch.float32)
    _call("mvsgi_resblock2d_split", x_split.data_ptr(), wp1.data_ptr(), shift1.data_ptr(), wp2.data_ptr(), shift2.data_ptr(), y.data_ptr(),
          int(out_split is not None), N, Hh, W, float(neg_slope), _stream_ptr(x_split))
    return y


def conv2d_s2_split(x_split, w_packed, shift, out_split, neg_slope=0.01) -> torch.Tensor:
    N, Hp, Wp, _ = x_split.shape
    Hh, W = Hp - 4, Wp - 4
    _check_split2d(x_split, N, Hh, W, x_split.device)
    _check_split2d(out_split, N, (Hh - 1) // 2 + 1, (W - 1) // 2 + 1, x_split.device)
    if shift.numel() != 16:
        raise AssertionError("conv2d_s2_split is the 16-channel layer")
    _call("mvsgi_conv2d_s2_split", x_split.data_ptr(), w_packed.data_ptr(), shift.data_ptr(), out_split.data_ptr(), N, Hh, W, float(neg_slope),
          _stream_ptr(x_split))
    return out_split


def resblock2d(x_nhwc, wp1, scale1, shift1, wp2, scale2, shift2, neg_slope=0.01) -> torch.Tensor:
    x = _dev(x_nhwc, "x")
    N, Hh, W, C = x.shape
    if C != 16 or scale1.numel() != 16 or scale2.numel() != 16:
        raise AssertionError(f"resblock2d is the 16-channel block, got x {tuple(x.shape)}")
    y = torch.empty_like(x)
    _call("mvsgi_resblock2d_f32", x.data_ptr(), wp1.data_ptr(), scale1.data_ptr(), shift1.data_ptr(), wp2.data_ptr(), scale2.data_ptr(),
          shift2.data_ptr(), y.data_ptr(), N, Hh, W, float(neg_slope), _stream_ptr(x))
    return y
```

Baseline: 6488.

## Write fp32 records from Winograd up2 and split them inside the head conv

The Winograd upsampling conv can now store plain fp32 activations instead of fp16 hi/lo split pairs, and a new head-conv variant reads those fp32 records and splits them into fp16 hi/lo in registers using permlane swaps before the MFMAs. This is enabled by default for the fp16 path when Winograd pays. The goal is to drop the split arithmetic and the scattered paired stores from the producer's epilogue and move the split into the consumer, where it can overlap with loads. The trade-off is extra VALU and permlane work in the head kernel, which is pinned to 3 waves per EU, and a buffer-format tag that other readers must check.

```diff
diff --git a/include/mvsgi.h b/include/mvsgi.h
--- a/include/mvsgi.h
+++ b/include/mvsgi.h
@@ -208,6 +208,10 @@
 int mvsgi_conv3d_head_split_pack_weights_f16(const float* w_oidhw, void* w_packed, int Cin, mvsgi_stream_t stream);
 int mvsgi_conv3d_head_split_f16(const void* x_split, const void* w_packed, float scale, float shift, float* y, int B, int Cin,
                             int D, int H, int W, float neg_slope, mvsgi_stream_t stream);
+int mvsgi_conv3d_up2_poly_rec32(const void* x_split, const void* plan_dev, const float* scale, const float* shift, void* y_rec32,
+                                int B, int D, int H, int W, float neg_slope, mvsgi_stream_t stream);
+int mvsgi_conv3d_head_rec32_f16(const void* x_rec32, const void* w_packed, float scale, float shift, float* y, int B, int Cin,
+                                int D, int H, int W, float neg_slope, mvsgi_stream_t stream);
 size_t mvsgi_conv3d_up2_poly_plan_bytes(int D, int H, int W);
 int mvsgi_conv3d_up2_poly_plan(const float* w_oidhw_host, void* plan_host, int D, int H, int W);
 int mvsgi_conv3d_up2_poly_f32(const void* x_split, const void* plan_dev, const float* scale, const float* shift, float* y,
diff --git a/mvs_gi_amd/_lib.py b/mvs_gi_amd/_lib.py
--- a/mvs_gi_amd/_lib.py
+++ b/mvs_gi_amd/_lib.py
@@ -97,6 +97,8 @@
     "mvsgi_conv3d_head_split": (c_int, [_P, _P, c_float, c_float, _P] + [c_int] * 5 + [c_float, _P]),
     "mvsgi_conv3d_head_split_pack_weights_f16": (c_int, [_P, _P, c_int, _P]),
     "mvsgi_conv3d_head_split_f16": (c_int, [_P, _P, c_float, c_float, _P] + [c_int] * 5 + [c_float, _P]),
+    "mvsgi_conv3d_head_rec32_f16": (c_int, [_P, _P, c_float, c_float, _P] + [c_int] * 5 + [c_float, _P]),
+    "mvsgi_conv3d_up2_poly_rec32": (c_int, [_P] * 5 + [c_int] * 4 + [c_float, _P]),
     "mvsgi_conv3d_up2_poly_plan_bytes": (c_size_t, [c_int] * 3),
     "mvsgi_conv3d_up2_poly_plan": (c_int, [_P, _P] + [c_int] * 3),
     "mvsgi_conv3d_up2_poly_f32": (c_int, [_P] * 5 + [c_int] * 4 + [c_float, _P]),
diff --git a/mvs_gi_amd/csrc/common.hpp b/mvs_gi_amd/csrc/common.hpp
--- a/mvs_gi_amd/csrc/common.hpp
+++ b/mvs_gi_amd/csrc/common.hpp
@@ -98,6 +98,6 @@
 void wino_up2_pack_role(const float* w32_oidhw, unsigned short* wp, float* unscale32);
 bool wino_up2_applies(int D, int H, int W);
 int wino_up2_launch(const void* x_split, const void* w_roles, const float* unw, const float* scale16, const float* shift16, void* y_split,
-                    int B, int D, int H, int W, float neg_slope, hipStream_t st);
+                    int B, int D, int H, int W, float neg_slope, bool out_f32, hipStream_t st);
 
 }
diff --git a/mvs_gi_amd/csrc/conv3d_headsplit.hip b/mvs_gi_amd/csrc/conv3d_headsplit.hip
--- a/mvs_gi_amd/csrc/conv3d_headsplit.hip
+++ b/mvs_gi_amd/csrc/conv3d_headsplit.hip
@@ -7,6 +7,8 @@
 typedef __bf16 bf16x8 __attribute__((ext_vector_type(8)));
 typedef _Float16 f16x8 __attribute__((ext_vector_type(8)));
 typedef unsigned short u16x8 __attribute__((ext_vector_type(8)));
+
+#include "split_fmt.hpp"
 
 struct HeadArgs {
     const unsigned char* x;
@@ -16,6 +18,7 @@
     float neg_slope;
     int B, Cin, D, H, W;
     int tiles_h, tiles_w;
+    unsigned* sat;
 };
 
 __device__ __forceinline__ int hs_xcd_remap(int bid, int n) {
@@ -49,8 +52,9 @@
     wp[((cs * 2 + tt) * 2 + 1) * 64 + lane] = __builtin_bit_cast(bf16x8, a2);
 }
 
-template <bool F16>
-__global__ __launch_bounds__(256) void conv3d_head_split_kernel(HeadArgs a, int dchunk, int nd) {
+template <bool F16, bool X32 = false>
+__global__ __launch_bounds__(256) __attribute__((amdgpu_waves_per_eu(X32 ? 3 : 1, X32 ? 3 : 8))) void conv3d_head_split_kernel(HeadArgs a, int dchunk, int nd) {
+    static_assert(F16 || !X32, "fp32 records are split into fp16 pairs");
     constexpr int TH = 8, TW = 32, ITH = TH + 2, ITW = TW + 2, PV = ITH * ITW;
     constexpr int NT = (PV + 15) / 16;
     constexpr int TPW = (NT + 3) / 4;
@@ -112,33 +116,65 @@
     int p = p0, cs = 0;
     float pend = 0.f;
     long long pend_vox = -1;
+    [[maybe_unused]] float satm = 0.f;
     for (int u = 0; u < U; ++u) {
         int ncs = cs + 1, np = p;
         if (ncs == nchunks) { ncs = 0; np = p + 1; }
-        bf16x8 cx[TPW], cw[2][2];
-#pragma unroll
-        for (int k = 0; k < TPW; ++k) cx[k] = __builtin_bit_cast(bf16x8, xr[k]);
+        bf16x8 cw[2][2];
 #pragma unroll
         for (int tt = 0; tt < 2; ++tt) { cw[tt][0] = wa[tt][0]; cw[tt][1] = wa[tt][1]; }
         if (pend_vox >= 0) {
             a.y[pend_vox] = pend;
             pend_vox = -1;
         }
-        {
-            const int fp = u + 1 < U ? np : p, fcs = u + 1 < U ? ncs : cs;
+        const int fp = u + 1 < U ? np : p, fcs = u + 1 < U ? ncs : cs;
+        if constexpr (X32) {
+            const __amdgpu_buffer_rsrc_t d_ = __builtin_amdgcn_make_buffer_rsrc(
+                const_cast<unsigned char*>(xb) + (long long)(fp + 1) * plane_bytes, 0, (int)plane_bytes, 0x00020000);
+#pragma unroll
+            for (int tt = 0; tt < 2; ++tt) {
+                wa[tt][0] = a.wp[((fcs * 2 + tt) * 2) * 64 + lane];
+                wa[tt][1] = a.wp[((fcs * 2 + tt) * 2 + 1) * 64 + lane];
+            }
+#pragma unroll
+            for (int k = 0; k < TPW; ++k) {
+                if (wave + 4 * k < NT) {
+                    sf_u32x2 h, l;
+                    sf_split4<true>(__builtin_bit_cast(sf_f32x4, xr[k]), h, l, satm);
+                    xr[k] = __builtin_amdgcn_raw_buffer_load_b128(d_, goff[k] + (unsigned)(fcs * 64), 0, 0);
+                    u32x4 op;
+#pragma unroll
+                    for (int i = 0; i < 2; ++i) {
+                        const auto s32 = __builtin_amdgcn_permlane32_swap(h[i], l[i], false, false);
+                        const auto s16 = __builtin_amdgcn_permlane16_swap(s32[0], s32[1], false, false);
+                        op[i] = s16[0];
+                        op[2 + i] = s16[1];
+                    }
+                    const f16x8 cxk = __builtin_bit_cast(f16x8, op);
+#pragma unroll
+                    for (int tt = 0; tt < 2; ++tt) {
+                        acc[k][tt] = __builtin_amdgcn_mfma_f32_16x16x32_f16(__builtin_bit_cast(f16x8, cw[tt][1]), cxk, acc[k][tt], 0, 0, 0);
+                        acc[k][tt] = __builtin_amdgcn_mfma_f32_16x16x32_f16(__builtin_bit_cast(f16x8, cw[tt][0]), cxk, acc[k][tt], 0, 0, 0);
+                    }
+                }
+            }
+        } else {
+            bf16x8 cx[TPW];
+#pragma unroll
+            for (int k = 0; k < TPW; ++k) cx[k] = __builtin_bit_cast(bf16x8, xr[k]);
             HS_FETCH(fp, fcs)
-        }
-#pragma unroll
-        for (int k = 0; k < TPW; ++k) {
-            if (wave + 4 * k < NT) {
-#pragma unroll
-                for (int tt = 0; tt < 2; ++tt) {
-                    if constexpr (F16) {
-                        acc[k][tt] = __builtin_amdgcn_mfma_f32_16x16x32_f16(__builtin_bit_cast(f16x8, cw[tt][1]), __builtin_bit_cast(f16x8, cx[k]), acc[k][tt], 0, 0, 0);
-                        acc[k][tt] = __builtin_amdgcn_mfma_f32_16x16x32_f16(__builtin_bit_cast(f16x8, cw[tt][0]), __builtin_bit_cast(f16x8, cx[k]), acc[k][tt], 0, 0, 0);
-                    } else {
-                        acc[k][tt] = __builtin_amdgcn_mfma_f32_16x16x32_bf16(cw[tt][1], cx[k], acc[k][tt], 0, 0, 0);
-                        acc[k][tt] = __builtin_amdgcn_mfma_f32_16x16x32_bf16(cw[tt][0], cx[k], acc[k][tt], 0, 0, 0);
+#pragma unroll
+            for (int k = 0; k < TPW; ++k) {
+                if (wave + 4 * k < NT) {
+#pragma unroll
+                    for (int tt = 0; tt < 2; ++tt) {
+                        if constexpr (F16) {
+                            acc[k][tt] = __builtin_amdgcn_mfma_f32_16x16x32_f16(__builtin_bit_cast(f16x8, cw[tt][1]), __builtin_bit_cast(f16x8, cx[k]), acc[k][tt], 0, 0, 0);
+                            acc[k][tt] = __builtin_amdgcn_mfma_f32_16x16x32_f16(__builtin_bit_cast(f16x8, cw[tt][0]), __builtin_bit_cast(f16x8, cx[k]), acc[k][tt], 0, 0, 0);
+                        } else {
+                            acc[k][tt] = __builtin_amdgcn_mfma_f32_16x16x32_bf16(cw[tt][1], cx[k], acc[k][tt], 0, 0, 0);
+                            acc[k][tt] = __builtin_amdgcn_mfma_f32_16x16x32_bf16(cw[tt][0], cx[k], acc[k][tt], 0, 0, 0);
+                        }
                     }
                 }
             }
@@ -187,6 +223,7 @@
         const float r = run[0] * a.scale + a.shift;
         a.y[vox] = r > 0.f ? r : r * a.neg_slope;
     }
+    if constexpr (X32) sf_sat_report(a.sat, kSatSplit, satm, kF16Max);
 #undef HS_FETCH
 }
 
@@ -207,7 +244,7 @@
 }
 
 int head_launch(const void* x_split, const void* w_packed, float scale, float shift, float* y, int B, int Cin, int D, int H, int W,
-                float neg_slope, bool f16, mvsgi_stream_t stream, const char* who) {
+                float neg_slope, bool f16, bool rec32, mvsgi_stream_t stream, const char* who) {
     MVSGI_REQUIRE(x_split && w_packed && y, "%s: null pointer", who);
     MVSGI_REQUIRE(B > 0 && D > 0 && H > 0 && W > 0 && Cin > 0 && Cin % 16 == 0, "%s: bad dims (Cin %% 16 == 0)", who);
     MVSGI_REQUIRE((long long)(H + 2) * (W + 2) * Cin * 4 < (1ll << 31), "%s: plane too large for 32-bit offsets", who);
@@ -227,7 +264,11 @@
     const long long nt = windows * nd;
     MVSGI_REQUIRE(nt < (1ll << 31), "%s: too many tiles", who);
     constexpr size_t lds_bytes = (size_t)27 * 360 * sizeof(float);
-    if (f16)
+    if (rec32) {
+        MVSGI_SAT_WORDS(sat_words_);
+        a.sat = sat_words_;
+        hipLaunchKernelGGL((conv3d_head_split_kernel<true, true>), dim3((unsigned)nt), dim3(256), lds_bytes, mvsgi::as_stream(stream), a, dchunk, (int)nd);
+    } else if (f16)
         hipLaunchKernelGGL(conv3d_head_split_kernel<true>, dim3((unsigned)nt), dim3(256), lds_bytes, mvsgi::as_stream(stream), a, dchunk, (int)nd);
     else
         hipLaunchKernelGGL(conv3d_head_split_kernel<false>, dim3((unsigned)nt), dim3(256), lds_bytes, mvsgi::as_stream(stream), a, dchunk, (int)nd);
@@ -244,9 +285,13 @@
 
 extern "C" int mvsgi_conv3d_head_split(const void* x_split, const void* w_packed, float scale, float shift, float* y, int B, int Cin,
                                        int D, int H, int W, float neg_slope, mvsgi_stream_t stream) {
-    return head_launch(x_split, w_packed, scale, shift, y, B, Cin, D, H, W, neg_slope, false, stream, "mvsgi_conv3d_head_split");
+    return head_launch(x_split, w_packed, scale, shift, y, B, Cin, D, H, W, neg_slope, false, false, stream, "mvsgi_conv3d_head_split");
 }
 extern "C" int mvsgi_conv3d_head_split_f16(const void* x_split, const void* w_packed, float scale, float shift, float* y, int B, int Cin,
                                            int D, int H, int W, float neg_slope, mvsgi_stream_t stream) {
-    return head_launch(x_split, w_packed, scale, shift, y, B, Cin, D, H, W, neg_slope, true, stream, "mvsgi_conv3d_head_split_f16");
-}
+    return head_launch(x_split, w_packed, scale, shift, y, B, Cin, D, H, W, neg_slope, true, false, stream, "mvsgi_conv3d_head_split_f16");
+}
+extern "C" int mvsgi_conv3d_head_rec32_f16(const void* x_rec32, const void* w_packed, float scale, float shift, float* y, int B, int Cin,
+                                           int D, int H, int W, float neg_slope, mvsgi_stream_t stream) {
+    return head_launch(x_rec32, w_packed, scale, shift, y, B, Cin, D, H, W, neg_slope, true, true, stream, "mvsgi_conv3d_head_rec32_f16");
+}
diff --git a/mvs_gi_amd/csrc/conv3d_up2poly.hip b/mvs_gi_amd/csrc/conv3d_up2poly.hip
--- a/mvs_gi_amd/csrc/conv3d_up2poly.hip
+++ b/mvs_gi_amd/csrc/conv3d_up2poly.hip
@@ -415,7 +415,7 @@
 namespace {
 
 int poly_launch(const void* x_split, const void* plan_dev, const float* scale, const float* shift, void* y, int ob, int B, int D, int H,
-                int W, float neg_slope, int fmt, hipStream_t st, int form = 0) {
+                int W, float neg_slope, int fmt, hipStream_t st, int form = 0, bool rec32 = false) {
     MVSGI_REQUIRE(x_split && plan_dev && scale && shift && y, "mvsgi_conv3d_up2_poly: null pointer");
     MVSGI_REQUIRE(fmt == 0 || fmt == MVSGI_SPLIT_F16, "mvsgi_conv3d_up2_poly: fmt %d not in {0, MVSGI_SPLIT_F16}", fmt);
     MVSGI_REQUIRE(B > 0 && D > 0 && H > 0 && W > 0, "mvsgi_conv3d_up2_poly: bad dims");
@@ -480,7 +480,7 @@
                   "D == 8, H %% 2 == 0 and W %% 32 == 0 (got D, H, W = %d, %d, %d)", D, H, W);
     if (form == 2)
         return mvsgi::wino_up2_launch(x_split, P + h.off_wino, reinterpret_cast<const float*>(P + h.off_wino_unscale), scale, shift, y,
-                                      B, D, H, W, neg_slope, st);
+                                      B, D, H, W, neg_slope, rec32, st);
     if (fmt && ob && form == 0 && h.off_wino) {
         const long long units = (long long)B * (H / 2) * (W / 32);
         long long nwalk = cus / 16;
@@ -489,7 +489,7 @@
         const long long rounds = mvsgi::cdiv(mvsgi::cdiv(units, 8), nwalk);
         if (10 * units >= 7 * rounds * 8 * nwalk)
             return mvsgi::wino_up2_launch(x_split, P + h.off_wino, reinterpret_cast<const float*>(P + h.off_wino_unscale), scale, shift, y,
-                                          B, D, H, W, neg_slope, st);
+                                          B, D, H, W, neg_slope, false, st);
     }
     return mvsgi::rs32_up2_launch(x_split, P + h.off_main, scale, shift, y, ob, B, D, H, W, neg_slope, fmt != 0, st);
 }
@@ -512,6 +512,11 @@
                   y_is_split);
     return poly_launch(x_split, plan_dev, scale, shift, y, y_is_split ? 1 : 0, B, D, H, W, neg_slope, fmt, mvsgi::as_stream(stream),
                        y_is_split == 3 ? 1 : (y_is_split == 5 ? 2 : 0));
+}
+
+extern "C" int mvsgi_conv3d_up2_poly_rec32(const void* x_split, const void* plan_dev, const float* scale, const float* shift, void* y_rec32,
+                                           int B, int D, int H, int W, float neg_slope, mvsgi_stream_t stream) {
+    return poly_launch(x_split, plan_dev, scale, shift, y_rec32, 1, B, D, H, W, neg_slope, MVSGI_SPLIT_F16, mvsgi::as_stream(stream), 2, true);
 }
 
 extern "C" int mvsgi_conv3d_up2_poly_wino_pays(int B, int D, int H, int W) {
diff --git a/mvs_gi_amd/csrc/conv3d_wino_up2.hip b/mvs_gi_amd/csrc/conv3d_wino_up2.hip
--- a/mvs_gi_amd/csrc/conv3d_wino_up2.hip
+++ b/mvs_gi_amd/csrc/conv3d_wino_up2.hip
@@ -55,6 +55,7 @@
     lo = sf_cvt_pk<true>(mix_sub_lo(v0, hi), mix_sub_hi(v1, hi));
 }
 
+template <bool OF32>
 __global__ __launch_bounds__(256, 1) void conv3d_wino_up2_kernel(WinoUp2Args a) {
     using namespace wu;
     extern __shared__ __attribute__((aligned(16))) unsigned char lds[];
@@ -106,7 +107,7 @@
                            *reinterpret_cast<const f32x4*>(a.unw + (ph * 2 + 1) * 16 + kg * 4) * esc_};
     __builtin_amdgcn_sched_barrier(0);
 
-    const int lane_out = (2 * n) * 128 + (kg >> 1) * 16 + (kg & 1) * 8;
+    const int lane_out = OF32 ? (2 * n) * 128 + kg * 16 : (2 * n) * 128 + (kg >> 1) * 16 + (kg & 1) * 8;
     const int rd0 = ((kg & 1) * SUB + (i0 * 2 * HALF + n) * PITCH + (kg >> 1) * 2) * 16;
     const int rd1 = ((kg & 1) * SUB + (i1 * 2 * HALF + n) * PITCH + (kg >> 1) * 2) * 16;
     constexpr int RD2 = 16;
@@ -257,12 +258,16 @@
         _Pragma("unroll") for (int e_ = 0; e_ < 4; ++e_)                                                    \
             t_[e_] = __builtin_fmaf(t_[e_], ema_[c_][e_], __builtin_fmaf(rf_[c_][e_], esc_[e_], esh_[e_])); \
         _Pragma("unroll") for (int e_ = 0; e_ < 4; ++e_) t_[e_] = __builtin_fmaxf(t_[e_], t_[e_] * a.neg_slope); \
-        unsigned h0_, l0_, h1_, l1_;                                                                        \
-        split_pair_ovfl(t_[0], t_[1], h0_, l0_, satm);                                                      \
-        split_pair_ovfl(t_[2], t_[3], h1_, l1_, satm);                                                      \
         unsigned char* q_ = yb + (long long)((O) + 1) * oplane_bytes + lane_out + c_ * 64;                  \
-        *reinterpret_cast<u32x2*>(q_) = u32x2{h0_, h1_};                                                    \
-        *reinterpret_cast<u32x2*>(q_ + 32) = u32x2{l0_, l1_};                                               \
+        if constexpr (OF32) {                                                                               \
+            *reinterpret_cast<f32x4*>(q_) = t_;                                                             \
+        } else {                                                                                            \
+            unsigned h0_, l0_, h1_, l1_;                                                                    \
+            split_pair_ovfl(t_[0], t_[1], h0_, l0_, satm);                                                  \
+            split_pair_ovfl(t_[2], t_[3], h1_, l1_, satm);                                                  \
+            *reinterpret_cast<u32x2*>(q_) = u32x2{h0_, h1_};                                                \
+            *reinterpret_cast<u32x2*>(q_ + 32) = u32x2{l0_, l1_};                                           \
+        }                                                                                                   \
     }
 #define KU_SLOT(M, S, SI, SM, SF, VB)                                                                       \
     {                                                                                                       \
@@ -320,7 +325,8 @@
     {                                                                                                       \
         unsigned char* rim_ = lds + RB + rprev * RES_LDS;                                                   \
         KU_OUT_WRITE(SF, (DEPTH - 1) & 1)                                                                   \
-        asm volatile("s_waitcnt vmcnt(4) lgkmcnt(0)" ::: "memory");                                         \
+        if constexpr (OF32) asm volatile("s_waitcnt vmcnt(2) lgkmcnt(0)" ::: "memory");                     \
+        else asm volatile("s_waitcnt vmcnt(4) lgkmcnt(0)" ::: "memory");                                    \
         __builtin_amdgcn_s_barrier();                                                                       \
         KU_EPI_READS((DEPTH - 1) & 1)                                                                       \
         KU_EPILOGUE(DEPTH - 1)                                                                              \
@@ -415,8 +421,9 @@
            (long long)(2 * D + 2) * (2 * H + 2) * (2 * W + 2) * 64 < (1ll << 31);
 }
 
-int wino_up2_launch(const void* x_split, const void* w_roles, const float* unw, const float* scale16, const float* shift16, void* y_split,
-                    int B, int D, int H, int W, float neg_slope, hipStream_t st) {
+template <bool OF32>
+static int wino_up2_launch_t(const void* x_split, const void* w_roles, const float* unw, const float* scale16, const float* shift16,
+                             void* y_split, int B, int D, int H, int W, float neg_slope, hipStream_t st) {
     MVSGI_REQUIRE(wino_up2_applies(D, H, W), "mvsgi_conv3d_up2_poly(winograd): needs D == 8, H %% 2 == 0, W %% 32 == 0 (got %d, %d, %d)", D, H, W);
     WinoUp2Args a;
     memset(&a, 0, sizeof(a));
@@ -437,13 +444,19 @@
     a.sat = sat_words_;
     static PersistentGeom geo_cache[kMaxDevices] = {};
     PersistentGeom geo;
-    if (persistent_geometry(conv3d_wino_up2_kernel, 256, wu::LDS_BYTES, 1, geo_cache, "conv3d(winograd up2)", geo)) return 1;
+    if (persistent_geometry(conv3d_wino_up2_kernel<OF32>, 256, wu::LDS_BYTES, 1, geo_cache, "conv3d(winograd up2)", geo)) return 1;
     long long nwalk = geo.cus / 16;
     const long long most = cdiv(units, 8);
     if (nwalk > most) nwalk = most;
     if (nwalk < 1) nwalk = 1;
-    hipLaunchKernelGGL(conv3d_wino_up2_kernel, dim3((unsigned)(16 * nwalk)), dim3(256), wu::LDS_BYTES, st, a);
+    hipLaunchKernelGGL(conv3d_wino_up2_kernel<OF32>, dim3((unsigned)(16 * nwalk)), dim3(256), wu::LDS_BYTES, st, a);
     return check_launch("mvsgi_conv3d_up2_poly(winograd main)");
 }
 
-}
+int wino_up2_launch(const void* x_split, const void* w_roles, const float* unw, const float* scale16, const float* shift16, void* y_split,
+                    int B, int D, int H, int W, float neg_slope, bool out_f32, hipStream_t st) {
+    return out_f32 ? wino_up2_launch_t<true>(x_split, w_roles, unw, scale16, shift16, y_split, B, D, H, W, neg_slope, st)
+                   : wino_up2_launch_t<false>(x_split, w_roles, unw, scale16, shift16, y_split, B, D, H, W, neg_slope, st);
+}
+
+}
diff --git a/mvs_gi_amd/dropin/cost_volume_regulator.py b/mvs_gi_amd/dropin/cost_volume_regulator.py
--- a/mvs_gi_amd/dropin/cost_volume_regulator.py
+++ b/mvs_gi_amd/dropin/cost_volume_regulator.py
@@ -139,6 +139,7 @@
 _USE_POLY = os.environ.get("MVSGI_POLY", "1") != "0"
 _HEAD_SPLIT = os.environ.get("MVSGI_HEAD_SPLIT", "1") != "0"
 _POLY_MIN_UNITS = 1600
+_TAIL_F32 = os.environ.get("MVSGI_TAIL_F32", "1") != "0"
 
 
 def _poly_tail(self, x: Tensor, skip: Tensor):
@@ -159,6 +160,7 @@
     if _HEAD_SPLIT and Lh.head_split_ok() and Lh.cin == 16:
         hi = cm._owned_split_buffer(self, "_mvsgi_poly_bufs", (B, 4 * Dl, 4 * Hl, 4 * Wl, "hi", x.device),
                                     lambda: H.SplitAct(B, 4 * Dl, 4 * Hl, 4 * Wl, 16, x.device))
+        hi.rec = "f32" if (_TAIL_F32 and xs.fmt == "f16" and H.conv3d_up2_poly_wino_pays(B, 2 * Dl, 2 * Hl, 2 * Wl)) else "pairs"
         return Lh.run_head_split(Lo.run_up2_poly_split(xs, hi))
     return Lh.run(Lo.run_up2_poly(xs))
 
diff --git a/mvs_gi_amd/hip_ops.py b/mvs_gi_amd/hip_ops.py
--- a/mvs_gi_amd/hip_ops.py
+++ b/mvs_gi_amd/hip_ops.py
@@ -437,6 +437,13 @@
                           wino: bool = False) -> "SplitAct":
     if x.C != 32 or scale.numel() != 16 or out.shape != (x.B, 2 * x.D, 2 * x.H, 2 * x.W, 16):
         raise AssertionError(f"conv3d_up2_poly_split: input {x.shape}, output {out.shape}")
+    if out.rec == "f32":
+        if x.fmt != "f16" or direct or not POLY_WINO:
+            raise AssertionError(f"conv3d_up2_poly_split: fp32 records need the fp16 split's Winograd form (input holds {x.fmt} pieces, direct={direct})")
+        _call("mvsgi_conv3d_up2_poly_rec32", x.buf.data_ptr(), plan.data_ptr(), scale.data_ptr(), shift.data_ptr(), out.buf.data_ptr(),
+              x.B, x.D, x.H, x.W, float(neg_slope), _stream_ptr(x.buf))
+        out.fmt = x.fmt
+        return out
     _call("mvsgi_conv3d_up2_poly_fmt", x.buf.data_ptr(), plan.data_ptr(), scale.data_ptr(), shift.data_ptr(), out.buf.data_ptr(),
           5 if wino else (3 if (direct or not POLY_WINO) else 1), x.B, x.D, x.H, x.W, float(neg_slope), _fmt_code(x.fmt), _stream_ptr(x.buf))
     out.fmt = x.fmt
@@ -469,10 +476,13 @@
 def conv3d_head_split(x: "SplitAct", w_packed, scale: float, shift: float, neg_slope=1.0, out=None, f16: bool = False) -> torch.Tensor:
     if x.fmt != ("f16" if f16 else "bf16"):
         raise AssertionError(f"conv3d_head_split(f16={f16}) on a split-padded buffer holding {x.fmt} pieces")
+    if x.rec == "f32" and not f16:
+        raise AssertionError("conv3d_head_split: fp32 records are read in the fp16 split only")
     y = out if out is not None else torch.empty((x.B, x.D, x.H, x.W, 1), device=x.buf.device, dtype=torch.float32)
     if tuple(y.shape) != (x.B, x.D, x.H, x.W, 1) or not y.is_contiguous():
         raise AssertionError(f"head output {tuple(y.shape)} does not match {(x.B, x.D, x.H, x.W, 1)}")
-    _call("mvsgi_conv3d_head_split_f16" if f16 else "mvsgi_conv3d_head_split", x.buf.data_ptr(), w_packed.data_ptr(), float(scale),
+    _call("mvsgi_conv3d_head_rec32_f16" if x.rec == "f32" else ("mvsgi_conv3d_head_split_f16" if f16 else "mvsgi_conv3d_head_split"),
+          x.buf.data_ptr(), w_packed.data_ptr(), float(scale),
           float(shift), y.data_ptr(), x.B, x.C, x.D, x.H, x.W, float(neg_slope), _stream_ptr(x.buf))
     return y
 
@@ -494,11 +504,12 @@
 
 
 class SplitAct:
-    __slots__ = ("buf", "B", "D", "H", "W", "C", "fmt")
+    __slots__ = ("buf", "B", "D", "H", "W", "C", "fmt", "rec")
 
     def __init__(self, B, D, H, W, C, device, buf=None):
         self.B, self.D, self.H, self.W, self.C = int(B), int(D), int(H), int(W), int(C)
         self.fmt = "bf16"
+        self.rec = "pairs"
         if buf is None:
             buf = torch.zeros((self.B, self.D + 2, self.H + 2, self.W + 2, self.C), device=device, dtype=torch.int32)
         self.buf = buf
@@ -524,6 +535,8 @@
 
 
 def act_from_split(x: SplitAct, out: Optional[torch.Tensor] = None) -> torch.Tensor:
+    if x.rec != "pairs":
+        raise AssertionError("act_from_split reads (hi | lo) pairs; this buffer holds fp32 records")
     y = out if out is not None else torch.empty(x.shape, device=x.buf.device, dtype=torch.float32)
     _call("mvsgi_act_split_to_f32_fmt", x.buf.data_ptr(), y.data_ptr(), x.B, x.C, x.D, x.H, x.W, _fmt_code(x.fmt), _stream_ptr(x.buf))
     return y
```

After: 6563 (median of 6 runs). +1.1%, better.
